# eryxcoop/acvm-backend-plonky2

Measured on AMD Instinct MI355X. Metric: prove latency (ms) + proofs/sec at 2^20 LDE rows, 1 GPU(s): value = proofs/sec, witness resident in HBM, 4 proof(s) in flight per GPU; latency_ms_single_proof = lone resident proof; *_host_witness = p2gpu_prove from host RAM (PCIe inside the call), higher is better.
Workload: dtype u64; 1 GPU; synth(d=17,sha): 131072 gates -> 2^20 LDE rows, 234 wires / 80 routed, KeccakGoldilocksConfig, rate 8, cap 2^4, 28 queries, 16 PoW bits (BASELINE configs[2] shape); degree_bits=17, lde_rows=1048576, mix=sha, public_inputs=0, in_flight_per_gpu=4, proof_bytes=170972

## Files before the change

acvm-backend-plonky2_amd/__init__.py:

```python
from .prover import (
    CircuitData,
    WitnessPlan,
    build_blob,
    VerifierCircuitData,
    ProofWithPublicInputs,
    P2GpuError,
    device_info,
    peer_access,
    init,
    host_array,
    host_free,
    ifft_batch,
    lde_batch,
    commit_values,
    hash_rows,
    field_selftest,
    lib_path,
    load_library,
)
from .synth import make_circuit, synth_lib_path
from . import parallel
from . import translate
from . import acir
```

acvm-backend-plonky2_amd/csrc/gen_keccak_fixed.py:

```python
#!/usr/bin/env python3
import sys

from gen_keccak_sched import RC, Op, ref_keccak_f, round_ops, schedule

NTEMP = 36


def build(base):
    a = [(f"a{i}l", f"a{i}h") for i in range(25)]
    live = [v for p in a for v in p]
    ops = []
    c = []
    for x in range(5):
        halves = []
        for h in range(2):
            p = f"cin{x}{'lh'[h]}p"
            q = f"cin{x}{'lh'[h]}"
            ops.append(Op("X3", p, (a[x][h], a[x + 5][h], a[x + 10][h]), 0x96, len(ops)))
            ops.append(Op("X3", q, (p, a[x + 15][h], a[x + 20][h]), 0x96, len(ops)))
            halves.append(q)
        c.append(tuple(halves))
    cur_a, cur_c = a, c
    for r in range(24):
        rops, cur_a, cur_c = round_ops(r, cur_a, cur_c)
        ops.extend(rops)
    needed = {v for p in cur_a for v in p}
    keep = []
    for o in reversed(ops):
        if o.dst in needed:
            keep.append(o)
            needed.update(o.srcs)
    ops = list(reversed(keep))
    return live, g_schedule(ops, live), cur_a


def g_schedule(ops, live_in, gap=1):
    pos = {v: -gap for v in live_in}
    remaining = list(ops)
    out = []
    slot = 0
    pattern = "BBA"
    while remaining:
        t = len(out)
        avail = [o for o in remaining if all(s in pos and pos[s] + gap <= t for s in o.srcs)]
        if not avail:
            avail = [o for o in remaining if all(s in pos for s in o.srcs)][:1]
        want_a = pattern[slot % 3] == "A"
        pick = None
        for o in avail:
            if (o.kind == "ROT") == want_a:
                pick = o
                break
        if pick is None:
            pick = avail[0]
        else:
            slot += 1
        out.append(pick)
        pos[pick.dst] = t
        remaining.remove(pick)
    return out


def allocate(live, ops, final_a, base):
    alias = {}
    for o in ops:
        if o.kind == "IOTA" and ((RC[int(o.dst[1:].split("_")[0])] >> (32 * o.imm)) & 0xFFFFFFFF) == 0:
            alias[o.dst] = alias.get(o.srcs[0], o.srcs[0])
    if alias:
        ops = [Op(o.kind, o.dst, tuple(alias.get(s_, s_) for s_ in o.srcs), o.imm, o.order) for o in ops if o.dst not in alias]
        final_a = [tuple(alias.get(v, v) for v in p) for p in final_a]
    last_use = {}
    for t, o in enumerate(ops):
        for s in o.srcs:
            last_use[s] = t
    finals = [v for p in final_a for v in p]
    for v in finals:
        last_use[v] = len(ops) + 1
    consumers = {}
    for t, o in enumerate(ops):
        for s in o.srcs:
            consumers.setdefault(s, []).append(o)
    reg = {v: base + i for i, v in enumerate(live)}
    free = list(range(base + 50, base + 50 + NTEMP))
    out = []
    conflicts = 0
    for t, o in enumerate(ops):
        srcs = [reg[s] for s in o.srcs]
        if o.kind in ("X3", "CHI") and len({r % 4 for r in srcs}) == 1:
            conflicts += 1
        for s in set(o.srcs):
            if last_use[s] == t:
                free.append(reg[s])
        avoid_hard, avoid_soft = set(), set()
        for cns in consumers.get(o.dst, []):
            if cns.kind not in ("X3", "CHI"):
                continue
            others = [s for s in cns.srcs if s != o.dst]
            banks = [reg[s] % 4 for s in others if s in reg]
            if len(others) == 2 and len(banks) == 2 and banks[0] == banks[1]:
                avoid_hard.add(banks[0])
            else:
                avoid_soft.update(banks)
        best = None
        for r_ in free:
            b = r_ % 4
            score = (b in avoid_hard) * 100 + (b in avoid_soft) * 1
            if best is None or score < best[0]:
                best = (score, r_)
        if best is None:
            raise SystemExit(f"out of registers at op {t} (NTEMP = {NTEMP})")
        free.remove(best[1])
        reg[o.dst] = best[1]
        out.append((o, best[1], srcs))
    moves = []
    want = {base + i: reg[v] for i, v in enumerate(finals)}
    pending = {d: s for d, s in want.items() if d != s}
    tmp = None
    spare = [r_ for r_ in range(base + 50, base + 50 + NTEMP) if r_ not in set(want.values())]
    while pending:
        progressed = False
        for d, s in list(pending.items()):
            if d not in pending.values():
                moves.append((d, s))
                del pending[d]
                progressed = True
        if not progressed:
            d, s = next(iter(pending.items()))
            tmp = spare[0]
            moves.append((tmp, d))
            for k in pending:
                if pending[k] == d:
                    pending[k] = tmp
    return out, moves, conflicts


def simulate(alloc, moves, st, base):
    M = 0xFFFFFFFF
    regs = {}
    for i in range(25):
        regs[base + 2 * i] = st[i] & M
        regs[base + 2 * i + 1] = st[i] >> 32
    for o, d, srcs in alloc:
        s = [regs[r] for r in srcs]
        if o.kind == "X3":
            v = s[0] ^ s[1] ^ s[2]
        elif o.kind == "CHI":
            v = s[0] ^ (~s[1] & s[2] & M)
        elif o.kind == "ROT":
            v = (((s[0] << 32) | s[1]) >> o.imm) & M
        else:
            rnd = int(o.dst[1:].split("_")[0])
            v = s[0] ^ ((RC[rnd] >> (32 * o.imm)) & M)
        regs[d] = v & M
    for d, s in moves:
        regs[d] = regs[s]
    return [regs[base + 2 * i] | (regs[base + 2 * i + 1] << 32) for i in range(25)]


def main():
    base = 36
    args = [x for x in sys.argv[1:] if not x.startswith("--")]
    if args:
        base = int(args[0])
    live, ops, final_a = build(base)
    alloc, moves, conflicts = allocate(live, ops, final_a, base)
    if "--check" in sys.argv:
        import random
        rng = random.Random(2)
        for _ in range(3):
            st = [rng.getrandbits(64) for _ in range(25)]
            assert simulate(alloc, moves, st, base) == ref_keccak_f(st)
        kinds = "".join("A" if o.kind == "ROT" else "B" for o, _, _ in alloc)
        print(f"ok: {len(alloc)} instructions + {len(moves)} moves, {conflicts} three-source instructions with all sources in one bank;",
              kinds[:60], "...", file=sys.stderr)
        return
    w = sys.stdout.write
    top = base + 50 + NTEMP
    w("// GENERATED by gen_keccak_fixed.py -- do not edit.  Keccak-f[1600], 24 rounds unrolled, explicit VGPRs (see the generator).\n")
    w(f"#define P2_KF_BASE {base}\n#define P2_KF_TOP {top}  /* first register above the block's */\n")
    w("#define P2_KECCAK_FIXED_PERMUTE() P2_KECCAK_FIXED_PERMUTE_PH(1)\n")
    w("#define P2_KECCAK_FIXED_PERMUTE_PH(PH) asm volatile(\".p2align 6\\n .rept \" #PH \"\\n s_nop 0\\n .endr\\n\" \\\n")
    for o, d, srcs in alloc:
        if o.kind in ("X3", "CHI"):
            w(f'  "v_bitop3_b32 v{d}, v{srcs[0]}, v{srcs[1]}, v{srcs[2]} bitop3:{hex(o.imm)}\\n" \\\n')
        elif o.kind == "ROT":
            w(f'  "v_alignbit_b32 v{d}, v{srcs[0]}, v{srcs[1]}, {o.imm}\\n" \\\n')
        else:
            rnd = int(o.dst[1:].split("_")[0])
            k = (RC[rnd] >> (32 * o.imm)) & 0xFFFFFFFF
            if k <= 64:
                w(f'  "v_xor_b32_e64 v{d}, {k}, v{srcs[0]}\\n" \\\n')
            else:
                w(f'  "v_xor_b32 v{d}, {hex(k)}, v{srcs[0]}\\n" \\\n')
    for d, s in moves:
        w(f'  "v_mov_b32 v{d}, v{s}\\n" \\\n')
    w(f'  ::: "v{top - 1}")\n')


if __name__ == "__main__":
    main()
```

acvm-backend-plonky2_amd/csrc/handle.hip:

```cpp
#include "prover_internal.hpp"
#include <functional>

using namespace p2;

namespace {

void release_for_destroy(p2gpu_circuit *c) {
  for (p2gpu_circuit *m : c->group) {
    m->peer = nullptr;
    release_for_destroy(m);
    delete m;
  }
  c->group.clear();
  if (c->peer && c->shard_rank == 0) {
    for (auto e : c->peer->recv_free) if (e) (void)hipEventDestroy(e);
    for (auto e : c->peer->sent) if (e) (void)hipEventDestroy(e);
    delete c->peer;
  }
  c->peer = nullptr;
  (void)hipSetDevice(c->device);
  if (c->stream) (void)hipStreamSynchronize(c->stream);
  if (c->rccl_comm) (void)rccl().CommDestroy((ncclComm_t)c->rccl_comm);
  c->rccl_comm = nullptr;
  circuit_release(c);
}
struct ReleaseHook {
  ReleaseHook() { p2::g_circuit_release = release_for_destroy; }
} g_release_hook;

struct Scratch {
  std::vector<void *> ptrs;
  hipStream_t st = nullptr;
  ~Scratch() {
    for (void *p : ptrs) (void)hipFree(p);
    if (st) (void)hipStreamDestroy(st);
  }
  template <class T> T *alloc(size_t n) {
    void *p = nullptr;
    if (hipMalloc(&p, (n ? n : 1) * sizeof(T)) != hipSuccess) return nullptr;
    ptrs.push_back(p);
    return (T *)p;
  }
};

}

namespace p2 {

int g_device = -1;
std::vector<int> g_peer_access;
std::vector<int> g_devices;

void circuit_release(p2gpu_circuit *c) {
  c->tw_fwd.release(); c->tw_inv.release(); c->scale.release(); c->inv_scale.release(); c->d_kis.release();
  c->d_sigmas.release(); c->fri_scale.release(); c->d_gates.release(); c->qconst.release(); c->l0_lde.release();
  c->d_row_gate.release(); c->d_gconsts.release(); c->d_prc.release(); c->d_prc_hash.release();
  c->hsum.release(); c->htmp_a.release(); c->htmp_b.release();
  c->cs.release(); c->wires.release(); c->zp.release(); c->quot.release();
  c->wires_vals.release(); c->zp_vals.release(); c->cp.release(); c->scan_tmp.release();
  c->apow.release(); c->qvals.release(); c->qtmp.release(); c->pw.release(); c->partial.release();
  c->ext_apow.release(); c->f01.release(); c->f01v.release(); c->fv.release();
  for (auto &b : c->fri_coef) b.release();
  for (auto &b : c->fri_vals) b.release();
  for (auto &b : c->fri_trees) b.release();
  c->hash_state.release();
  c->wire_nz.release();
  c->wire_nzlist.release();
  c->wire_clean.release();
  c->wire_scalar.release(); c->sparse_coeffs.release(); c->sparse_lde.release(); c->sparse_partial.release();
  c->pin.release();
  if (c->sync_event) (void)hipEventDestroy(c->sync_event);
  c->sync_event = nullptr;
  if (c->tail_stage) (void)hipHostFree(c->tail_stage);
  c->tail_stage = nullptr;
  c->pow_result.release(); c->gather_ptrs.release(); c->gather_out.release(); c->xchg_recv.release();
  ntt_plan_destroy(c->plan_inv);
  ntt_plan_destroy(c->plan_fwd);
  for (auto *p : c->fri_plans)
    if (p != c->plan_fwd) ntt_plan_destroy(p);
  c->plan_inv = c->plan_fwd = nullptr;
  c->fri_plans.clear();
  for (auto e : c->event_pool) (void)hipEventDestroy(e);
  for (auto e : c->copy_events) (void)hipEventDestroy(e);
  if (c->copy_stream) (void)hipStreamDestroy(c->copy_stream);
  if (c->stream) (void)hipStreamDestroy(c->stream);
}

int ensure_device() {
  if (g_device >= 0) return 0;
  int cnt = 0;
  hipError_t e = hipGetDeviceCount(&cnt);
  if (e != hipSuccess || cnt == 0) {
    set_err("no HIP device available (%s); libp2gpu has no CPU fallback", e == hipSuccess ? "count=0" : hipGetErrorString(e));
    return P2GPU_E_DEVICE;
  }
  int dev = 0;
  (void)hipGetDevice(&dev);
  g_device = dev;
  g_devices.assign(1, dev);
  g_peer_access.assign(1, -1);
  return 0;
}

}


namespace {

#define CK(e, what)                                       \
  do {                                                    \
    const hipError_t e_ = (e);                            \
    if (e_ != hipSuccess) {                               \
      set_err("%s: %s", what, hipGetErrorString(e_));     \
      return P2GPU_E_DEVICE;                              \
    }                                                     \
  } while (0)

void schedule_gates(p2gpu_circuit *c) {
  c->nterms = c->K + c->K * c->nchunks + c->max_gate_constraints;
  auto cost = [](const GateDesc &g) { return g.kind == G_POSEIDON ? 0u : 4u * g.num_constraints + 8u; };
  const uint32_t perm_cost = (uint32_t)env_uint("P2GPU_PERM_COST", 8u * c->R + 100u);
  uint32_t total = 0;
  for (auto &g : c->gates) total += cost(g);
  c->gate_groups = env_uint("P2GPU_GATE_GROUPS", total > 2 * perm_cost ? 4u : 1u) == 4 ? 4u : 1u;
  uint32_t load[4] = {perm_cost, 0, 0, 0};
  std::vector<uint32_t> order(c->gates.size());
  for (size_t i = 0; i < order.size(); i++) order[i] = (uint32_t)i;
  std::sort(order.begin(), order.end(), [&](uint32_t x, uint32_t y) { return cost(c->gates[x]) > cost(c->gates[y]); });
  for (uint32_t gi : order) {
    uint32_t best = 0;
    for (uint32_t q = 1; q < 4; q++)
      if (load[q] < load[best]) best = q;
    c->gates[gi].pad = c->gate_groups == 4 ? best : 0;
    load[best] += cost(c->gates[gi]);
  }
  uint64_t half_constraints = 0;
  if (env_flag("P2GPU_HALF_GATES", true) && c->d >= 6 && c->rate_bits == 3)
    for (auto &g : c->gates)
      if (g.kind != G_POSEIDON && g.num_constraints >= 48 && gate_degree(g.kind, g.p) <= 4 && c->half_slots < 64) {
        g.pad |= (++c->half_slots) << 16;
        half_constraints += g.num_constraints;
      }
  c->half_auto = (half_constraints << c->d) >= ((uint64_t)12 << 20);
  if (c->half_slots) {
    auto cost_main = [&](const GateDesc &g) { return gate_half_slot(g) ? 8u : cost(g); };
    uint32_t rest = 0;
    for (auto &g : c->gates) rest += cost_main(g);
    c->gate_groups_half = env_uint("P2GPU_GATE_GROUPS_HALF", rest > 2 * perm_cost ? 4u : 1u) == 4 ? 4u : 1u;
    uint32_t lm[4] = {perm_cost, 0, 0, 0}, ls[4] = {0, 0, 0, 0};
    c->sums_groups = env_uint("P2GPU_SUMS_GROUPS", c->half_slots >= 2 ? 4u : 1u) == 4 ? 4u : 1u;
    for (uint32_t gi : order) {
      GateDesc &g = c->gates[gi];
      uint32_t bm = 0, bs = 0;
      for (uint32_t q = 1; q < 4; q++) {
        if (lm[q] < lm[bm]) bm = q;
        if (ls[q] < ls[bs]) bs = q;
      }
      if (c->gate_groups_half == 4) g.pad |= bm << 4;
      lm[bm] += cost_main(g);
      if (gate_half_slot(g)) {
        if (c->sums_groups == 4) g.pad |= bs << 8;
        ls[bs] += cost(g);
      }
    }
  }
}

int make_streams(p2gpu_circuit *c) {
  if (poseidon_upload_constants()) { set_err("uploading Poseidon constants failed"); return P2GPU_E_DEVICE; }
  CK(hipStreamCreateWithFlags(&c->stream, hipStreamNonBlocking), "hipStreamCreate");
  CK(hipStreamCreateWithFlags(&c->copy_stream, hipStreamNonBlocking), "hipStreamCreate");
  return P2GPU_OK;
}

int make_root_tables(p2gpu_circuit *c) {
  hipStream_t st = c->stream;
  const size_t n = c->n;
  const uint32_t d = c->d, K = c->K, C = c->C;
  const size_t half = n >= 2 ? n / 2 : 1;
  CK(c->tw_fwd.alloc(half), "alloc tw");
  CK(c->tw_inv.alloc(half), "alloc tw");
  CK(c->scale.alloc((size_t)C * n), "alloc scale");
  CK(c->inv_scale.alloc((size_t)C * n), "alloc scale");
  CK(c->fri_scale.alloc((size_t)C * n), "alloc scale");
  CK(c->d_kis.alloc(c->R), "alloc kis");
  CK(c->d_sigmas.alloc((size_t)c->R * n), "alloc sigmas");
  CK(c->d_gates.alloc(c->num_gates ? c->num_gates : 1), "alloc gates");
  gl_t wn = gl_root(d), wN = gl_root(d + c->rate_bits);
  c->plan_inv = ntt_plan_create(st, d, NttDir::ToCoeffs);
  c->plan_fwd = ntt_plan_create(st, d, NttDir::ToValues);
  if (!c->plan_inv || !c->plan_fwd) { set_err("ntt plan allocation failed"); return P2GPU_E_DEVICE; }
  fill_powers(st, c->tw_fwd.p, wn, (uint32_t)half);
  fill_powers(st, c->tw_inv.p, gl_inv(wn), (uint32_t)half);
  fill_coset_scale(st, c->scale.p, GL_GEN, wN, d, C, 1);
  fill_coset_scale(st, c->inv_scale.p, gl_inv(GL_GEN), gl_inv(wN), d, C, 1);
  if (c->half_slots) {
    const size_t per = (size_t)4 * c->half_slots * K * n;
    CK(c->hsum.alloc(2 * per), "alloc gate sums");
    CK(c->htmp_a.alloc(per), "alloc gate sums");
    CK(c->htmp_b.alloc(per), "alloc gate sums");
    const gl_t w8 = gl_root(3), quarter = gl_inv(4);
    for (int mo = 0; mo < 4; mo++)
      for (int m = 0; m < 4; m++) {
        const gl_t base = gl_pow(w8, (uint64_t)((2 * mo + 1 - 2 * m + 16) % 8));
        gl_t acc = 0, pw = 1;
        for (int j = 0; j < 4; j++) {
          acc = gl_add(acc, pw);
          pw = gl_mul(pw, base);
        }
        c->half_cross[4 * mo + m] = gl_mul(acc, quarter);
      }
  }
  CK(c->qconst.alloc(24), "alloc qconst");
  {
    gl_t qc[24];
    memset(qc, 0, sizeof qc);
    gl_t wC = gl_root(c->rate_bits), gn = gl_pow(GL_GEN, n);
    for (uint32_t r = 0; r < C; r++) {
      qc[r] = gl_mul(GL_GEN, gl_pow(wN, r));
      qc[8 + r] = gl_sub(gl_mul(gn, gl_pow(wC, r)), 1);
      qc[16 + r] = gl_inv(qc[8 + r]);
    }
    CK(hipMemcpy(c->qconst.p, qc, sizeof qc, hipMemcpyHostToDevice), "copy qconst");
    CK(c->l0_lde.alloc((size_t)C * n), "alloc L0 table");
    fill_l0_table(st, c->qconst.p, c->tw_fwd.p, 0, d, C, gl_inv((gl_t)n), c->l0_lde.p);
  }
  return P2GPU_OK;
}

int tables_from_blob(p2gpu_circuit *c, const gl_t *constants, const gl_t *sigmas) {
  const size_t n = c->n;
  const uint32_t ngc = c->NC - c->num_selectors;
  CK(hipMemcpyAsync(c->d_sigmas.p, sigmas, 8 * (size_t)c->R * n, hipMemcpyHostToDevice, c->stream), "copy sigmas");
  std::vector<uint8_t> rg(n, 0);
  for (size_t row = 0; row < n; row++) {
    uint32_t gi = 0;
    for (uint32_t s = 0; s < c->num_selectors; s++) {
      gl_t v = constants[(size_t)s * n + row];
      if (c->num_selectors == 1 || v != 0xFFFFFFFFULL) gi = (uint32_t)v;
    }
    if (gi >= c->num_gates) { set_err("selector column holds an unknown gate index"); return P2GPU_E_BLOB; }
    rg[row] = (uint8_t)gi;
    if (c->sparse_row == UINT32_MAX && c->gates[gi].kind == G_PUBLIC_INPUT) c->sparse_row = (uint32_t)row;
  }
  c->sparse_rows = SparseRows();
  if (c->sparse_row != UINT32_MAX) {
    c->sparse_rows.row[c->sparse_rows.count++] = c->sparse_row;
    for (size_t row = 0; row < n && c->sparse_rows.count < MAX_SPARSE_ROWS; row++)
      if (c->gates[rg[row]].kind == G_POSEIDON) c->sparse_rows.row[c->sparse_rows.count++] = (uint32_t)row;
  }
  CK(hipMemcpy(c->d_row_gate.p, rg.data(), n, hipMemcpyHostToDevice), "copy row_gate");
  if (ngc)
    CK(hipMemcpy(c->d_gconsts.p, constants + (size_t)c->num_selectors * n, 8 * (size_t)ngc * n, hipMemcpyHostToDevice), "copy gconsts");
  return P2GPU_OK;
}

int alloc_proof_buffers(p2gpu_circuit *c) {
  hipStream_t st = c->stream;
  const size_t n = c->n;
  const uint32_t d = c->d, K = c->K, C = c->C;
  const uint32_t ncs = c->NC + c->R, nzp = K * (1 + c->PP), nq = K * c->QF;
  const uint32_t nall = ncs + c->W + nzp + nq;
  if (batch_alloc(c, c->cs, ncs) || batch_alloc(c, c->wires, c->W) || batch_alloc(c, c->zp, nzp) || batch_alloc(c, c->quot, nq)) return P2GPU_E_DEVICE;
  CK(c->wires_vals.alloc((size_t)c->W * n), "alloc wires");
  CK(c->wire_nz.alloc(c->W), "alloc wire flags");
  CK(c->wire_nzlist.alloc(c->W + 1), "alloc wire flags");
  CK(c->wire_clean.alloc(c->W), "alloc wire flags");
  CK(hipMemsetAsync(c->wire_clean.p, 0, sizeof(uint32_t) * c->W, c->stream), "clear wire flags");
  CK(c->wire_scalar.alloc((size_t)MAX_SPARSE_ROWS * c->W), "alloc wire flags");
  if (c->sparse_row != UINT32_MAX) {
    const uint32_t nr = c->sparse_rows.count;
    CK(c->sparse_coeffs.alloc((size_t)nr * n), "alloc sparse basis");
    CK(c->sparse_lde.alloc((size_t)nr * C * n), "alloc sparse basis");
    CK(c->sparse_partial.alloc(16 * 2 + 2), "alloc sparse basis");
    const gl_t one = 1;
    CK(hipMemsetAsync(c->sparse_coeffs.p, 0, 8 * (size_t)nr * n, st), "sparse basis");
    for (uint32_t s = 0; s < nr; s++)
      CK(hipMemcpyAsync(c->sparse_coeffs.p + (size_t)s * n + c->sparse_rows.row[s], &one, 8, hipMemcpyHostToDevice, st), "sparse basis");
    CK(hipStreamSynchronize(st), "sparse basis");
    ntt_batch(st, c->plan_inv, c->sparse_coeffs.p, c->sparse_coeffs.p, nr, 1, nullptr, gl_inv((gl_t)n), false);
    for (uint32_t s = 0; s < nr; s++)
      ntt_batch(st, c->plan_fwd, c->sparse_coeffs.p + (size_t)s * n, c->sparse_lde.p + (size_t)s * C * n, 1, C, c->scale.p, 1, false);
  }
  CK(c->zp_vals.alloc((size_t)nzp * n), "alloc zp");
  CK(c->cp.alloc((size_t)K * (c->nchunks + 1) * n), "alloc cp");
  CK(c->scan_tmp.alloc((size_t)K * (n + (n + 255) / 256 + 8)), "alloc scan");
  CK(c->apow.alloc((size_t)2 * c->nterms), "alloc apow");
  CK(c->qvals.alloc((size_t)K * C * n), "alloc qvals");
  CK(c->qtmp.alloc((size_t)K * C * n), "alloc qtmp");
  CK(c->pw.alloc((size_t)4 * n), "alloc pw");
  CK(c->partial.alloc(((size_t)(nall + K) + 8) * 16 * 2), "alloc partial");
  CK(c->ext_apow.alloc((size_t)2 * nall), "alloc ext_apow");
  CK(c->f01.alloc((size_t)4 * n), "alloc f01");
  CK(c->f01v.alloc((size_t)4 * n), "alloc f01v");
  CK(c->fv.alloc((size_t)2 * n), "alloc fv");
  c->fri_coef.resize(c->n_steps + 1);
  c->fri_vals.resize(c->n_steps + 1);
  c->fri_trees.resize(c->n_steps);
  size_t gather_words = 0;
  {
    uint32_t ds = d;
    const size_t cap_per = ((size_t)1 << c->cap_h) >> c->rate_bits;
    for (uint32_t s = 0; s <= c->n_steps; s++) {
      c->fri_plans.push_back(s == 0 ? c->plan_fwd : ntt_plan_create(st, ds, NttDir::ToValues));
      if (!c->fri_plans.back()) { set_err("ntt plan allocation failed"); return P2GPU_E_DEVICE; }
      CK(c->fri_coef[s].alloc((size_t)2 << ds), "alloc fri coef");
      if (s < c->n_steps) {
        CK(c->fri_vals[s].alloc((size_t)2 * C << ds), "alloc fri vals");
        uint32_t ab = c->arity[s];
        if (ab < 1 || ab > 4 || ds < ab || (((size_t)1 << ds) >> ab) < cap_per) { set_err("unsupported FRI reduction arity"); return P2GPU_E_BLOB; }
        if (tree_alloc(c->fri_trees[s], C, ((size_t)1 << ds) >> ab, cap_per)) return P2GPU_E_DEVICE;
        gather_words += (2u << ab) + 4 * (size_t)(ds + c->rate_bits);
        ds -= ab;
      }
    }
  }
  gather_words += nall + 4 * 4 * (size_t)(d + c->rate_bits);
  c->gather_cap = gather_words * c->num_queries + 64;
  CK(c->gather_ptrs.alloc(c->gather_cap), "alloc gather");
  CK(c->gather_out.alloc(c->gather_cap), "alloc gather");
  CK(c->pow_result.alloc(1), "alloc pow");
  {
    size_t n_final = n;
    for (uint32_t s = 0; s < c->n_steps; s++) n_final >>= c->arity[s];
    const size_t caps = (size_t)2 * (4 + c->n_steps) * (sizeof(dig_t) << c->cap_h);
    CK(c->pin.alloc(16 * c->gather_cap + 32 * n_final + 16 * (size_t)(nall + K) * 16 + 16 * (size_t)nall + 16 * (size_t)c->nterms +
                    20 * (size_t)c->W + caps + ((size_t)1 << 18)),
       "alloc pinned staging");
  }
  return P2GPU_OK;
}

struct TableSource {
  const gl_t *constants = nullptr, *sigmas = nullptr;
  const BuildInputs *build = nullptr;
};

int commit_constants_sigmas(p2gpu_circuit *c, const TableSource &src) {
  hipStream_t st = c->stream;
  const size_t n = c->n;
  const uint32_t ncs = c->NC + c->R;
  gl_t *stage = c->cs.lde.p;
  if (src.build) {
    build_selector_columns(st, c, stage);
    if (c->NC > c->num_selectors)
      CK(hipMemcpyAsync(stage + (size_t)c->num_selectors * n, c->d_gconsts.p, 8 * (size_t)(c->NC - c->num_selectors) * n, hipMemcpyDeviceToDevice, st),
         "copy constants");
  } else {
    CK(hipMemcpyAsync(stage, src.constants, 8 * (size_t)c->NC * n, hipMemcpyHostToDevice, st), "copy constants");
  }
  CK(hipMemcpyAsync(stage + (size_t)c->NC * n, c->d_sigmas.p, 8 * (size_t)c->R * n, hipMemcpyDeviceToDevice, st), "copy sigmas");
  ntt_batch(st, c->plan_inv, stage, c->cs.coeffs.p, ncs, 1, nullptr, gl_inv((gl_t)n), false);
  return batch_commit_from_coeffs(c, c->cs);
}

int check_cap_and_digest(p2gpu_circuit *c, const uint8_t *cap_in) {
  if (cap_in) {
    for (size_t i = 0; i < c->cs.cap.size(); i++)
      if (memcmp(cap_in + 32 * i, c->cs.cap[i].w, c->hasher ? 32 : 25)) { set_err("constants_sigmas cap mismatch"); return P2GPU_E_CAP_MISMATCH; }
  }
  if (!(c->flags & 1)) {
    std::vector<gl_t> parts;
    for (auto &dg : c->cs.cap) {
      gl_t e[4];
      digest_elems(dg, e);
      parts.insert(parts.end(), e, e + 4);
    }
    std::vector<gl_t> pad(8, 0);
    pad[0] = 1;
    pad[7] = 1;
    dig_t ds = host_hash_no_pad(pad);
    gl_t e[4];
    digest_elems(ds, e);
    parts.insert(parts.end(), e, e + 4);
    parts.push_back(c->d);
    c->circuit_digest = host_hash_no_pad(parts);
  }
  return P2GPU_OK;
}

int circuit_finish(p2gpu_circuit *c, const TableSource &src, const uint8_t *cap_in) {
  schedule_gates(c);
  CK(hipSetDevice(c->device), "hipSetDevice");
  const CreateTrace tr{c, now_ms()};
  if (int rc = make_streams(c)) return rc;
  tr.mark("streams + poseidon constants");
  if (int rc = make_root_tables(c)) return rc;
  tr.mark("root tables + ntt plans");
  const uint32_t ngc = c->NC - c->num_selectors;
  CK(hipMemcpyAsync(c->d_kis.p, c->k_is.data(), 8 * (size_t)c->R, hipMemcpyHostToDevice, c->stream), "copy kis");
  if (c->num_gates)
    CK(hipMemcpyAsync(c->d_gates.p, c->gates.data(), sizeof(GateDesc) * c->num_gates, hipMemcpyHostToDevice, c->stream), "copy gates");
  CK(c->d_row_gate.alloc(c->n), "alloc row_gate");
  CK(c->d_gconsts.alloc((size_t)(ngc ? ngc : 1) * c->n), "alloc gconsts");
  CK(c->d_prc.alloc(360), "alloc prc");
  if (int rc = src.build ? build_device_tables(c, *src.build, tr) : tables_from_blob(c, src.constants, src.sigmas)) return rc;
  CK(hipMemcpy(c->d_prc.p, c->poseidon_rc, sizeof c->poseidon_rc, hipMemcpyHostToDevice), "copy prc");
  gl_t hrc[360];
  poseidon_device_constants(c->poseidon_rc, hrc);
  CK(c->d_prc_hash.alloc(360), "alloc prc (hash form)");
  CK(hipMemcpy(c->d_prc_hash.p, hrc, sizeof hrc, hipMemcpyHostToDevice), "copy prc (hash form)");
  tr.mark("sigma/constant uploads, row->gate");
  if (int rc = alloc_proof_buffers(c)) return rc;
  tr.mark("batch + work buffer allocation");
  if (int rc = commit_constants_sigmas(c, src)) return rc;
  if (int rc = check_cap_and_digest(c, cap_in)) return rc;
  CK(hipStreamSynchronize(c->stream), "sync");
  tr.mark("constants_sigmas commitment");
  return P2GPU_OK;
}
#undef CK

int circuit_create_one(const uint8_t *blob, size_t len, int device, p2gpu_circuit **out_c) try {
  HalfBuilt c(new p2gpu_circuit());
  size_t off = 0;
  const uint8_t *cap_in = nullptr;
  c->device = device;
  if (int rc = circuit_parse(blob, len, c.get(), &off, &cap_in)) return rc;
  c->blob_prefix.assign(blob, blob + off);
  if (len < off + 8 * ((size_t)c->NC * c->n + (size_t)c->R * c->n)) { set_err("blob truncated (tables)"); return P2GPU_E_BLOB; }
  TableSource src;
  src.constants = (const gl_t *)(blob + off);
  src.sigmas = src.constants + (size_t)c->NC * c->n;
  if (int rc = circuit_finish(c.get(), src, cap_in)) return rc;
  *out_c = c.release();
  return P2GPU_OK;
} P2GPU_CATCH

struct BuildCall {
  const p2gpu_build_params *bp;
  const p2gpu_gate_decl *gates;
  uint32_t num_gates;
  BuildInputs in;
  std::vector<uint8_t> prefix;
};
int build_call_prepare(BuildCall &b, const p2gpu_build_params *bp, const p2gpu_gate_decl *gates, uint32_t num_gates, const uint32_t *row_gate,
                       const uint64_t *row_constants, const uint32_t *copies, size_t num_copies, uint32_t hasher, p2gpu_circuit **out_c) {
  if (out_c) *out_c = nullptr;
  if (!bp || !gates || !row_gate || !out_c || (num_copies && !copies)) return P2GPU_E_ARG;
  if (hasher > 1) { set_err("unsupported hasher (0 = KeccakHash<25>, 1 = PoseidonHash)"); return P2GPU_E_ARG; }
  BuildPlan pl;
  if (int rc = build_plan(bp, gates, num_gates, row_constants != nullptr, pl)) return rc;
  b.prefix.resize(pl.prefix_len);
  if (int rc = build_prefix(pl, bp, gates, hasher, b.prefix.data())) return rc;
  b.bp = bp; b.gates = gates; b.num_gates = num_gates;
  b.in = BuildInputs{row_gate, row_constants, copies, num_copies};
  return P2GPU_OK;
}
int circuit_build_one(const BuildCall &b, int device, p2gpu_circuit **out_c) try {
  HalfBuilt c(new p2gpu_circuit());
  c->device = device;
  size_t off = 0;
  const uint8_t *cap_in = nullptr;
  if (int rc = circuit_parse(b.prefix.data(), b.prefix.size(), c.get(), &off, &cap_in))
    return rc == P2GPU_E_BLOB ? P2GPU_E_ARG : rc;
  c->blob_prefix = b.prefix;
  TableSource src;
  src.build = &b.in;
  if (int rc = circuit_finish(c.get(), src, nullptr)) return rc;
  *out_c = c.release();
  return P2GPU_OK;
} P2GPU_CATCH
}

extern "C" {

int p2gpu_init(const int *device_ids, int n_devices) {
  int cnt = 0;
  hipError_t e = hipGetDeviceCount(&cnt);
  if (e != hipSuccess || cnt == 0) {
    set_err("no HIP device available (%s); libp2gpu has no CPU fallback", e == hipSuccess ? "count=0" : hipGetErrorString(e));
    return P2GPU_E_DEVICE;
  }
  if (n_devices > 8) {
    set_err("p2gpu_init: %d device ids (at most 8: one per LDE coset)", n_devices);
    return P2GPU_E_ARG;
  }
  std::vector<int> devs;
  for (int i = 0; i < (device_ids ? n_devices : 0); i++) devs.push_back(device_ids[i]);
  if (devs.empty()) devs.push_back(0);
  for (int dev : devs)
    if (dev < 0 || dev >= cnt) {
      set_err("device id %d out of range (%d devices)", dev, cnt);
      return P2GPU_E_ARG;
    }
  std::vector<int> peer(devs.size() * devs.size(), -1);
  for (size_t a = 0; a < devs.size(); a++)
    for (size_t b = 0; b < devs.size(); b++)
      if (devs[a] != devs[b]) {
        (void)hipSetDevice(devs[a]);
        const hipError_t pe = hipDeviceEnablePeerAccess(devs[b], 0);
        (void)hipGetLastError();
        peer[a * devs.size() + b] = (pe == hipSuccess || pe == hipErrorPeerAccessAlreadyEnabled) ? 1 : 0;
      }
  HIP_TRY(hipSetDevice(devs[0]));
  g_device = devs[0];
  g_devices = devs;
  g_peer_access = peer;
  return P2GPU_OK;
}

int p2gpu_peer_access(int *matrix_out, int cap) {
  if (int rc = ensure_device()) return rc;
  const int n = (int)g_devices.size();
  if (matrix_out) {
    if (cap < n * n) { set_err("p2gpu_peer_access: room for %d entries, %d needed", cap, n * n); return P2GPU_E_BUFFER; }
    for (int i = 0; i < n * n; i++) matrix_out[i] = i < (int)g_peer_access.size() ? g_peer_access[i] : -1;
  }
  return n;
}

void *p2gpu_host_alloc(size_t bytes) {
  if (ensure_device()) return nullptr;
  void *p = nullptr;
  hipError_t e = hipHostMalloc(&p, bytes ? bytes : 1, hipHostMallocPortable);
  if (e != hipSuccess) {
    (void)hipGetLastError();
    set_err("p2gpu_host_alloc: %zu bytes of page-locked memory: %s", bytes, hipGetErrorString(e));
    return nullptr;
  }
  return p;
}
void p2gpu_host_free(void *p) {
  if (p) (void)hipHostFree(p);
}

int p2gpu_device_info(char *name_out, size_t name_cap, int *cu_count, size_t *hbm_bytes) {
  if (int rc = ensure_device()) return rc;
  hipDeviceProp_t prop;
  HIP_TRY(hipGetDeviceProperties(&prop, g_device));
  if (name_out && name_cap) snprintf(name_out, name_cap, "%s (%s)", prop.name, prop.gcnArchName);
  if (cu_count) *cu_count = prop.multiProcessorCount;
  if (hbm_bytes) *hbm_bytes = prop.totalGlobalMem;
  return P2GPU_OK;
}


static int shard_layout(p2gpu_circuit *c, int rank, int world);
static int shard_args_ok(p2gpu_circuit *c, int rank, int world);


int p2gpu_circuit_create_on(const uint8_t *blob, size_t len, int device_id, p2gpu_circuit **out_c) try {
  if (!blob || !out_c) return P2GPU_E_ARG;
  if (int rc = ensure_device()) return rc;
  if (std::find(g_devices.begin(), g_devices.end(), device_id) == g_devices.end()) {
    set_err("p2gpu_circuit_create_on: device %d is not in the list given to p2gpu_init", device_id);
    return P2GPU_E_ARG;
  }
  const int rc = circuit_create_one(blob, len, device_id, out_c);
  (void)hipSetDevice(g_device);
  return rc;
} P2GPU_CATCH

static int circuit_make(const std::function<int(int, p2gpu_circuit **)> &one, p2gpu_circuit **out_c) {
  if (g_devices.size() <= 1) return one(g_device, out_c);
  const int n = (int)g_devices.size();
  std::vector<p2gpu_circuit *> hs(n, nullptr);
  std::vector<int> rcs(n, 0);
  std::vector<std::string> errs(n);
  {
    std::vector<std::thread> th;
    for (int q = 0; q < n; q++)
      th.emplace_back([&, q] {
        rcs[q] = one(g_devices[q], &hs[q]);
        if (rcs[q]) errs[q] = p2gpu_last_error();
      });
    for (auto &t : th) t.join();
  }
  (void)hipSetDevice(g_device);
  auto drop = [&](int rc, const std::string &msg) {
    for (auto *h : hs)
      if (h) {
        h->peer = nullptr;
        p2gpu_circuit_destroy(h);
      }
    set_err("%s", msg.c_str());
    return rc;
  };
  for (int q = 0; q < n; q++)
    if (rcs[q]) return drop(rcs[q], errs[q]);
  for (int q = 0; q < n; q++) {
    if (int rc = shard_args_ok(hs[q], q, n)) return drop(rc, p2gpu_last_error());
    if (int rc = shard_layout(hs[q], q, n)) return drop(rc, p2gpu_last_error());
  }
  PeerGroup *pg = new PeerGroup();
  pg->n = n;
  pg->cs = hs;
  pg->recv_free.assign(n, nullptr);
  pg->sent.assign(n, nullptr);
  pg->proof_scratch.resize(n);
  pg->send_ptr.resize(n);
  pg->recv_ptr.resize(n);
  for (int q = 0; q < n; q++) {
    (void)hipSetDevice(hs[q]->device);
    if (hipEventCreateWithFlags(&pg->recv_free[q], hipEventDisableTiming) != hipSuccess ||
        hipEventCreateWithFlags(&pg->sent[q], hipEventDisableTiming) != hipSuccess) {
      for (int k = 0; k <= q; k++) {
        (void)hipSetDevice(hs[k]->device);
        if (pg->recv_free[k]) (void)hipEventDestroy(pg->recv_free[k]);
        if (pg->sent[k]) (void)hipEventDestroy(pg->sent[k]);
        hs[k]->peer = nullptr;
      }
      (void)hipSetDevice(g_device);
      delete pg;
      return drop(P2GPU_E_DEVICE, "hipEventCreate failed");
    }
    hs[q]->peer = pg;
  }
  (void)hipSetDevice(g_device);
  for (int q = 1; q < n; q++) hs[0]->group.push_back(hs[q]);
  *out_c = hs[0];
  return P2GPU_OK;
}

int p2gpu_circuit_create(const uint8_t *blob, size_t len, p2gpu_circuit **out_c) try {
  if (!blob || !out_c) return P2GPU_E_ARG;
  if (int rc = ensure_device()) return rc;
  return circuit_make([&](int device, p2gpu_circuit **h) { return circuit_create_one(blob, len, device, h); }, out_c);
} P2GPU_CATCH


int p2gpu_circuit_build_on(const p2gpu_build_params *bp, const p2gpu_gate_decl *gates, uint32_t num_gates, const uint32_t *row_gate,
                           const uint64_t *row_constants, const uint32_t *copies, size_t num_copies, uint32_t hasher, int device_id,
                           p2gpu_circuit **out_c) try {
  BuildCall b;
  if (int rc = build_call_prepare(b, bp, gates, num_gates, row_gate, row_constants, copies, num_copies, hasher, out_c)) return rc;
  if (int rc = ensure_device()) return rc;
  if (std::find(g_devices.begin(), g_devices.end(), device_id) == g_devices.end()) {
    set_err("p2gpu_circuit_build_on: device %d is not in the list given to p2gpu_init", device_id);
    return P2GPU_E_ARG;
  }
  const int rc = circuit_build_one(b, device_id, out_c);
  (void)hipSetDevice(g_device);
  return rc;
} P2GPU_CATCH

int p2gpu_circuit_build(const p2gpu_build_params *bp, const p2gpu_gate_decl *gates, uint32_t num_gates, const uint32_t *row_gate,
                        const uint64_t *row_constants, const uint32_t *copies, size_t num_copies, uint32_t hasher, p2gpu_circuit **out_c) try {
  BuildCall b;
  if (int rc = build_call_prepare(b, bp, gates, num_gates, row_gate, row_constants, copies, num_copies, hasher, out_c)) return rc;
  if (int rc = ensure_device()) return rc;
  return circuit_make([&](int device, p2gpu_circuit **h) { return circuit_build_one(b, device, h); }, out_c);
} P2GPU_CATCH

int p2gpu_circuit_export_blob(const p2gpu_circuit *cc, uint8_t *out, size_t *len) try {
  if (!cc || !len) return P2GPU_E_ARG;
  if (int rc = prover_handle(cc)) return rc;
  p2gpu_circuit *c = const_cast<p2gpu_circuit *>(cc);
  const size_t n = c->n, nsel = c->num_selectors, ngc = c->NC - c->num_selectors;
  const size_t need = c->blob_prefix.size() + 8 * ((size_t)c->NC + c->R) * n;
  if (!out || *len < need) {
    const bool probe = out == nullptr;
    *len = need;
    if (probe) return P2GPU_OK;
    set_err("blob buffer too small: need %zu bytes", need);
    return P2GPU_E_BUFFER;
  }
  HIP_TRY(hipSetDevice(c->device));
  Scratch S;
  gl_t *sel = S.alloc<gl_t>(nsel * n);
  if (!sel) { set_err("hipMalloc failed"); (void)hipSetDevice(g_device); return P2GPU_E_DEVICE; }
  build_selector_columns(c->stream, c, sel);
  memcpy(out, c->blob_prefix.data(), c->blob_prefix.size());
  uint8_t *q = out + c->blob_prefix.size();
  hipError_t e = hipMemcpyAsync(q, sel, 8 * nsel * n, hipMemcpyDeviceToHost, c->stream);
  if (e == hipSuccess && ngc) e = hipMemcpyAsync(q + 8 * nsel * n, c->d_gconsts.p, 8 * ngc * n, hipMemcpyDeviceToHost, c->stream);
  if (e == hipSuccess) e = hipMemcpyAsync(q + 8 * (size_t)c->NC * n, c->d_sigmas.p, 8 * (size_t)c->R * n, hipMemcpyDeviceToHost, c->stream);
  const hipError_t e2 = hipStreamSynchronize(c->stream);
  (void)hipSetDevice(g_device);
  HIP_TRY(e);
  HIP_TRY(e2);
  *len = need;
  return P2GPU_OK;
} P2GPU_CATCH




int p2gpu_circuit_set(p2gpu_circuit *c, const char *key, uint64_t value) try {
  if (!c || !key) return P2GPU_E_ARG;
  if (int rc = prover_handle(c)) return rc;
  for (p2gpu_circuit *m : c->group)
    if (int rc = p2gpu_circuit_set(m, key, value)) return rc;
  HIP_TRY(hipSetDevice(c->device));
  std::string k(key);
  if (k == "pow_hint") c->pow_hint = value;
  else if (k == "self_check") c->self_check = (int)value;
  else if (k == "shard_exercise") c->shard_exercise = (int)value;
  else if (k == "shard_intt") c->shard_intt = (int)value;
  else if (k == "shard_reduce") c->shard_reduce = (int)value;
  else if (k == "shard_zs") c->shard_zs = (int)value;
  else if (k == "half_gates") c->half_gates = (int)value;
  else if (k == "blocking_sync") c->blocking_sync = (int)value;
  else if (k == "virtual_columns") {
    c->virtual_columns = (int)value;
    if (c->wire_clean.p) HIP_TRY(hipMemsetAsync(c->wire_clean.p, 0, sizeof(uint32_t) * c->W, c->stream));
  }
  else if (k == "zero_columns") {
    c->zero_columns = (int)value;
    c->structured_off = false;
    if (c->wire_clean.p) HIP_TRY(hipMemsetAsync(c->wire_clean.p, 0, sizeof(uint32_t) * c->W, c->stream));
  }
  else if (k == "profile") {
    flush_kstats(c);
    c->profile = (int)value;
    c->kstats.clear();
  } else {
    set_err("unknown knob %s", key);
    return P2GPU_E_ARG;
  }
  return P2GPU_OK;
} P2GPU_CATCH

static int shard_layout(p2gpu_circuit *c, int rank, int world) {
  HIP_TRY(hipSetDevice(c->device));
  if (c->stream) HIP_TRY(hipStreamSynchronize(c->stream));
  if (c->rccl_comm) {
    (void)rccl().CommDestroy((ncclComm_t)c->rccl_comm);
    c->rccl_comm = nullptr;
  }
  c->shard_rank = rank;
  c->shard_world = world;
  c->shard_fn = nullptr;
  c->shard_ctx = nullptr;
  const uint32_t ncl = c->C / (uint32_t)world;
  const size_t cap_per = ((size_t)1 << c->cap_h) >> c->rate_bits;
  CosetMap cm;
  cm.first = (uint32_t)rank;
  cm.stride = (uint32_t)world;
  Batch *bs[3] = {&c->wires, &c->zp, &c->quot};
  for (Batch *b : bs) {
    b->ncl = ncl;
    b->cm = cm;
    tree_layout(*b, ncl, c->n, cap_per);
  }
  if (c->n_steps > 0) {
    Batch &t0 = c->fri_trees[0];
    t0.ncl = ncl;
    t0.cm = cm;
    tree_layout(t0, ncl, c->n >> c->arity[0], cap_per);
  }
  if (c->wire_clean.p) HIP_TRY(hipMemsetAsync(c->wire_clean.p, 0, sizeof(uint32_t) * c->W, c->stream));
  c->xchg_recv.release();
  HIP_TRY(c->xchg_recv.alloc(std::max({(size_t)world * c->gather_cap, (size_t)c->K * c->C * c->n, (size_t)2 * world * c->n}) + 64));
  return P2GPU_OK;
}
static int shard_args_ok(p2gpu_circuit *c, int rank, int world) {
  if (!c || world < 1 || rank < 0 || rank >= world || (c->C % (uint32_t)world) != 0) {
    set_err("bad shard configuration: rank %d of %d (cosets %u)", rank, world, c ? c->C : 0u);
    return P2GPU_E_ARG;
  }
  if (int rc = prover_handle(c)) return rc;
  return P2GPU_OK;
}

static int not_a_group(const p2gpu_circuit *c) {
  if (c && c->peer) { set_err("this handle is a device group of one process (p2gpu_init with several ids): its sharding is fixed"); return P2GPU_E_ARG; }
  return P2GPU_OK;
}
int p2gpu_circuit_set_shard(p2gpu_circuit *c, int rank, int world, p2gpu_allgather_fn fn, void *ctx) try {
  if (int rc = not_a_group(c)) return rc;
  if (int rc = shard_args_ok(c, rank, world)) return rc;
  if (world > 1 && !fn) { set_err("a host all-gather callback is needed for world > 1 (or use p2gpu_circuit_set_shard_rccl)"); return P2GPU_E_ARG; }
  if (int rc = shard_layout(c, rank, world)) return rc;
  c->shard_fn = fn;
  c->shard_ctx = ctx;
  return P2GPU_OK;
} P2GPU_CATCH

int p2gpu_shard_unique_id(uint8_t id_out[128]) try {
  if (!id_out) return P2GPU_E_ARG;
  if (int rc = ensure_device()) return rc;
  if (!rccl().ok) { set_err("librccl.so.1 could not be loaded"); return P2GPU_E_DEVICE; }
  ncclUniqueId id;
  static_assert(sizeof id == 128, "ncclUniqueId is 128 bytes");
  RCCL_TRY(rccl().GetUniqueId(&id));
  memcpy(id_out, &id, sizeof id);
  return P2GPU_OK;
} P2GPU_CATCH

int p2gpu_circuit_set_shard_rccl(p2gpu_circuit *c, int rank, int world, const uint8_t id_in[128]) try {
  if (int rc = not_a_group(c)) return rc;
  if (int rc = shard_args_ok(c, rank, world)) return rc;
  if (!id_in) return P2GPU_E_ARG;
  if (!rccl().ok) { set_err("librccl.so.1 could not be loaded"); return P2GPU_E_DEVICE; }
  if (int rc = shard_layout(c, rank, world)) return rc;
  ncclUniqueId id;
  memcpy(&id, id_in, sizeof id);
  ncclComm_t comm = nullptr;
  RCCL_TRY(rccl().CommInitRank(&comm, world, id, rank));
  c->rccl_comm = (void *)comm;
  return P2GPU_OK;
} P2GPU_CATCH

int p2gpu_kernel_stats(p2gpu_circuit *c, char *names, double *ms, double *bytes, uint64_t *launches, int cap) try {
  if (!c) return P2GPU_E_ARG;
  if (int rc = prover_handle(c)) return rc;
  (void)hipSetDevice(c->device);
  (void)hipStreamSynchronize(c->stream);
  flush_kstats(c);
  int i = 0;
  for (auto &kv : c->kstats) {
    if (i >= cap) break;
    snprintf(names + 64 * i, 64, "%s", kv.first.c_str());
    ms[i] = kv.second.ms;
    bytes[i] = kv.second.bytes;
    launches[i] = kv.second.launches;
    i++;
  }
  return i;
} P2GPU_CATCH

int p2gpu_ifft_batch(const uint64_t *vals, size_t ncols, unsigned d, uint64_t *coeffs_out) try {
  if (int rc = ensure_device()) return rc;
  if (!vals || !coeffs_out || d > 24) return P2GPU_E_ARG;
  Scratch S;
  HIP_TRY(hipStreamCreate(&S.st));
  size_t n = (size_t)1 << d, half = n >= 2 ? n / 2 : 1;
  gl_t *a = S.alloc<gl_t>(ncols * n), *b = S.alloc<gl_t>(ncols * n), *tw = S.alloc<gl_t>(half);
  if (!a || !b || !tw) { set_err("hipMalloc failed"); return P2GPU_E_DEVICE; }
  HIP_TRY(hipMemcpyAsync(a, vals, 8 * ncols * n, hipMemcpyHostToDevice, S.st));
  NttPlan *plan = ntt_plan_create(S.st, d, NttDir::ToCoeffs);
  if (!plan) { set_err("hipMalloc failed"); return P2GPU_E_DEVICE; }
  ntt_batch(S.st, plan, a, b, (uint32_t)ncols, 1, nullptr, gl_inv((gl_t)n), false);
  bitrev_cols(S.st, b, a, d, (uint32_t)ncols);
  hipError_t e1 = hipMemcpyAsync(coeffs_out, a, 8 * ncols * n, hipMemcpyDeviceToHost, S.st);
  hipError_t e2 = hipStreamSynchronize(S.st);
  ntt_plan_destroy(plan);
  HIP_TRY(e1);
  HIP_TRY(e2);
  return P2GPU_OK;
} P2GPU_CATCH

int p2gpu_lde_batch(const uint64_t *coeffs, size_t ncols, unsigned d, unsigned rate_bits, uint64_t *lde_out) try {
  if (int rc = ensure_device()) return rc;
  if (!coeffs || !lde_out || d > 24 || rate_bits > 3) return P2GPU_E_ARG;
  Scratch S;
  HIP_TRY(hipStreamCreate(&S.st));
  size_t n = (size_t)1 << d, half = n >= 2 ? n / 2 : 1;
  uint32_t C = 1u << rate_bits;
  gl_t *a = S.alloc<gl_t>(ncols * n), *b = S.alloc<gl_t>(ncols * n), *tw = S.alloc<gl_t>(half);
  gl_t *scale = S.alloc<gl_t>(C * n), *lde = S.alloc<gl_t>(C * ncols * n);
  if (!a || !b || !tw || !scale || !lde) { set_err("hipMalloc failed"); return P2GPU_E_DEVICE; }
  HIP_TRY(hipMemcpyAsync(a, coeffs, 8 * ncols * n, hipMemcpyHostToDevice, S.st));
  bitrev_cols(S.st, a, b, d, (uint32_t)ncols);
  NttPlan *plan = ntt_plan_create(S.st, d, NttDir::ToValues);
  if (!plan) { set_err("hipMalloc failed"); return P2GPU_E_DEVICE; }
  fill_coset_scale(S.st, scale, GL_GEN, gl_root(d + rate_bits), d, C, 1);
  ntt_batch(S.st, plan, b, lde, (uint32_t)ncols, C, scale, 1, false);
  std::vector<gl_t> tmp(C * ncols * n);
  hipError_t e1 = hipMemcpyAsync(tmp.data(), lde, 8 * tmp.size(), hipMemcpyDeviceToHost, S.st);
  hipError_t e2 = hipStreamSynchronize(S.st);
  ntt_plan_destroy(plan);
  HIP_TRY(e1);
  HIP_TRY(e2);
  for (uint32_t r = 0; r < C; r++)
    for (size_t col = 0; col < ncols; col++)
      for (size_t k = 0; k < n; k++) lde_out[col * C * n + C * k + r] = tmp[((size_t)r * ncols + col) * n + k];
  return P2GPU_OK;
} P2GPU_CATCH

static int field_selftest_words(const uint64_t *a, const uint64_t *b, size_t n, uint64_t *bad_out, size_t words);
int p2gpu_field_selftest(const uint64_t *a, const uint64_t *b, size_t n, uint64_t bad_out[8]) { return field_selftest_words(a, b, n, bad_out, 8); }
int p2gpu_field_selftest16(const uint64_t *a, const uint64_t *b, size_t n, uint64_t bad_out[16]) { return field_selftest_words(a, b, n, bad_out, 16); }
static int field_selftest_words(const uint64_t *a, const uint64_t *b, size_t n, uint64_t *bad_out, size_t words) try {
  if (int rc = ensure_device()) return rc;
  if (!a || !b || !bad_out || n == 0 || n > ((size_t)1 << 28)) return P2GPU_E_ARG;
  Scratch S;
  HIP_TRY(hipStreamCreate(&S.st));
  uint64_t *da = S.alloc<uint64_t>(n), *db = S.alloc<uint64_t>(n);
  unsigned long long *bad = S.alloc<unsigned long long>(16);
  if (!da || !db || !bad) { set_err("hipMalloc failed"); return P2GPU_E_DEVICE; }
  HIP_TRY(hipMemcpyAsync(da, a, 8 * n, hipMemcpyHostToDevice, S.st));
  HIP_TRY(hipMemcpyAsync(db, b, 8 * n, hipMemcpyHostToDevice, S.st));
  HIP_TRY(hipMemsetAsync(bad, 0, 128, S.st));
  field_selftest(S.st, da, db, (uint32_t)n, bad);
  HIP_TRY(hipMemcpyAsync(bad_out, bad, 8 * words, hipMemcpyDeviceToHost, S.st));
  HIP_TRY(hipStreamSynchronize(S.st));
  return P2GPU_OK;
} P2GPU_CATCH

int p2gpu_hash_rows(const uint64_t *rows, size_t n_rows, size_t row_len, uint8_t *digests_out) try {
  if (int rc = ensure_device()) return rc;
  if (!rows || !digests_out) return P2GPU_E_ARG;
  Scratch S;
  HIP_TRY(hipStreamCreate(&S.st));
  gl_t *a = S.alloc<gl_t>(n_rows * row_len);
  dig_t *dg = S.alloc<dig_t>(n_rows);
  if (!a || !dg) { set_err("hipMalloc failed"); return P2GPU_E_DEVICE; }
  HIP_TRY(hipMemcpyAsync(a, rows, 8 * n_rows * row_len, hipMemcpyHostToDevice, S.st));
  hash_rows(S.st, a, n_rows, (uint32_t)row_len, dg);
  std::vector<dig_t> h(n_rows);
  HIP_TRY(hipMemcpyAsync(h.data(), dg, sizeof(dig_t) * n_rows, hipMemcpyDeviceToHost, S.st));
  HIP_TRY(hipStreamSynchronize(S.st));
  for (size_t i = 0; i < n_rows; i++) memcpy(digests_out + 25 * i, h[i].w, 25);
  return P2GPU_OK;
} P2GPU_CATCH

int p2gpu_commit_values(const uint64_t *vals, size_t ncols, unsigned d, unsigned rate_bits, unsigned cap_h,
                        uint8_t *cap_out) try {
  if (int rc = ensure_device()) return rc;
  if (!vals || !cap_out || d > 24 || rate_bits > 3 || cap_h < rate_bits || cap_h > rate_bits + d) return P2GPU_E_ARG;
  HalfBuilt own(new p2gpu_circuit());
  p2gpu_circuit *c = own.get();
  c->d = d; c->rate_bits = rate_bits; c->cap_h = cap_h; c->n = (size_t)1 << d; c->N = c->n << rate_bits;
  c->C = 1u << rate_bits; c->device = g_device; c->n_steps = 0;
  int rc = P2GPU_OK;
  size_t n = c->n, half = n >= 2 ? n / 2 : 1;
  do {
    if (hipStreamCreate(&c->stream) != hipSuccess || c->tw_fwd.alloc(half) != hipSuccess ||
        c->tw_inv.alloc(half) != hipSuccess || c->scale.alloc((size_t)c->C * n) != hipSuccess ||
        c->wires_vals.alloc(ncols * n) != hipSuccess || c->pin.alloc(((size_t)1 << 16) + 2 * (sizeof(dig_t) << cap_h)) != hipSuccess) {
      set_err("hipMalloc failed");
      rc = P2GPU_E_DEVICE;
      break;
    }
    if ((rc = batch_alloc(c, c->wires, (uint32_t)ncols))) break;
    c->plan_inv = ntt_plan_create(c->stream, d, NttDir::ToCoeffs);
    c->plan_fwd = ntt_plan_create(c->stream, d, NttDir::ToValues);
    if (!c->plan_inv || !c->plan_fwd) {
      set_err("hipMalloc failed");
      rc = P2GPU_E_DEVICE;
      break;
    }
    fill_coset_scale(c->stream, c->scale.p, GL_GEN, gl_root(d + rate_bits), d, c->C, 1);
    if (hipMemcpyAsync(c->wires_vals.p, vals, 8 * ncols * n, hipMemcpyHostToDevice, c->stream) != hipSuccess) {
      set_err("copy failed");
      rc = P2GPU_E_DEVICE;
      break;
    }
    if ((rc = batch_commit_from_values(c, c->wires, c->wires_vals.p))) break;
    for (size_t i = 0; i < c->wires.cap.size(); i++) memcpy(cap_out + 25 * i, c->wires.cap[i].w, 25);
  } while (0);
  return rc;
} P2GPU_CATCH

}
```

acvm-backend-plonky2_amd/csrc/internal.hpp:

```cpp
#pragma once
#include <hip/hip_runtime.h>
#include <cstdlib>
#include <vector>
#include "gl.hpp"
#include "keccak.hpp"
#include "gates.hpp"

namespace p2 {

constexpr int MAX_GATES = 64;
constexpr uint32_t MAX_GATE_CONSTRAINTS = 4096;
constexpr uint32_t MAX_ARITY_BITS = 4;
constexpr int MAX_CHALLENGES = 2;
constexpr int MAX_ROUTED = 128;

inline bool env_flag(const char *name, bool dflt) {
  const char *e = getenv(name);
  return e && *e ? *e != '0' : dflt;
}
inline uint64_t env_uint(const char *name, uint64_t dflt) {
  const char *e = getenv(name);
  return e ? strtoull(e, nullptr, 10) : dflt;
}

struct Prof {
  virtual void begin(const char *kernel, double algorithmic_bytes) = 0;
  virtual void end() = 0;
  virtual ~Prof() {}
};
extern thread_local Prof *g_prof;
struct ProfScope {
  ProfScope(const char *k, double bytes) { if (g_prof) g_prof->begin(k, bytes); }
  ~ProfScope() { if (g_prof) g_prof->end(); }
};

constexpr uint32_t MAX_SPARSE_ROWS = 4;
struct SparseRows {
  uint32_t row[MAX_SPARSE_ROWS] = {UINT32_MAX, UINT32_MAX, UINT32_MAX, UINT32_MAX};
  uint32_t count = 0;
};
struct ColHints {
  const uint32_t *cls = nullptr;
  const uint32_t *clean = nullptr;
  const gl_t *val = nullptr;
  const gl_t *basis = nullptr;
  bool basis_per_coset = false;
  uint32_t nrows = 1, val_stride = 0;
  size_t basis_stride = 0;
  uint32_t virt_first = UINT32_MAX;
  uint32_t dense_hint = 0;
  bool fill_only = false;
};
void column_clean_update(hipStream_t st, const uint32_t *cls, uint32_t cols, uint32_t *clean, bool after);
void column_flags(hipStream_t st, const gl_t *vals, uint32_t cols, uint32_t d, const SparseRows &rows, uint32_t *flags,
                  gl_t *scalar, uint32_t sstride);

constexpr int NTT_MAX_ROUNDS = 6;
enum class NttDir { ToCoeffs, ToValues };
struct NttPass {
  uint32_t s, a, tb, nrounds;
  uint32_t r[NTT_MAX_ROUNDS], tw_off[NTT_MAX_ROUNDS];
  bool direct = false;
  uint32_t rm = 0, rl = 0, fold_r = 0, fold_s0 = 0;
  uint32_t ftw_off = 0;
};
struct NttPlan {
  uint32_t d = 0;
  NttDir dir = NttDir::ToCoeffs;
  std::vector<NttPass> passes;
  gl_t *ptw = nullptr;
  size_t table_len = 0;
};
struct CosetMap {
  uint32_t first = 0, stride = 1;
};
NttPlan *ntt_plan_create(hipStream_t st, uint32_t d, NttDir dir);
void ntt_plan_destroy(NttPlan *p);
void ntt_batch(hipStream_t st, const NttPlan *plan, const gl_t *src, gl_t *dst, uint32_t cols, uint32_t cosets,
               const gl_t *scale, gl_t post, bool src_per_coset, CosetMap cm = CosetMap(), uint32_t stride_cols = 0,
               const ColHints *hints = nullptr);

void fill_powers(hipStream_t st, gl_t *out, gl_t root, uint32_t count);
void fill_coset_scale(hipStream_t st, gl_t *out, gl_t shift, gl_t wN, uint32_t d, uint32_t cosets, gl_t mult);

void bitrev_cols(hipStream_t st, const gl_t *in, gl_t *out, uint32_t d, uint32_t cols);
void field_selftest(hipStream_t st, const uint64_t *a, const uint64_t *b, uint32_t n, unsigned long long *bad);

struct VirtCols {
  const uint32_t *cls = nullptr;
  const gl_t *val = nullptr;
  const gl_t *basis = nullptr;
  uint32_t first = UINT32_MAX;
  uint32_t coset_first = 0, coset_stride = 1;
};
uint32_t hash_lde_leaves(hipStream_t st, const gl_t *lde, uint32_t cols, uint32_t d, uint32_t cosets, dig_t *dig, const gl_t *prc = nullptr,
                         const VirtCols *virt = nullptr, dig_t *lvl1 = nullptr, dig_t *lvl2 = nullptr);
void hash_lde_absorb(hipStream_t st, const gl_t *lde, uint32_t cols, uint32_t d, uint32_t cosets, uint32_t blk0,
                     uint32_t nblk, bool first, bool last, uint64_t *state, dig_t *dig, const VirtCols *virt = nullptr);
void hash_rows(hipStream_t st, const gl_t *rows, size_t n_rows, uint32_t row_len, dig_t *dig);
void hash_fri_leaves(hipStream_t st, const gl_t *vals, uint32_t lg_npc, uint32_t cosets, uint32_t arity_bits,
                     dig_t *dig, const gl_t *prc = nullptr);
bool tree_levels(hipStream_t st, dig_t *lvl, uint32_t cosets, uint32_t m, uint32_t cap_per, const gl_t *prc = nullptr,
                 dig_t *host_mirror = nullptr);

struct ZsArgs {
  const gl_t *wires;
  const gl_t *sigmas;
  const gl_t *k_is;
  const gl_t *sub_tw;
  uint32_t tw_shift;
  uint32_t d, R, QF, nchunks, K;
  gl_t betas[MAX_CHALLENGES], gammas[MAX_CHALLENGES];
  gl_t *cp;
  uint32_t sb;
  uint32_t row0, rows;
  gl_t *zp;
};
void zs_partial_products(hipStream_t st, const ZsArgs &a, gl_t *scan_tmp);
void zs_chunks(hipStream_t st, const ZsArgs &a);
void zs_scan_finish(hipStream_t st, const ZsArgs &a, gl_t *scan_tmp);

struct QuotArgs {
  const gl_t *cs_lde;
  const gl_t *wires_lde;
  const gl_t *zp_lde;
  const gl_t *k_is;
  const gl_t *tw;
  const gl_t *apow;
  const GateDesc *gates;
  const GateDesc *host_gates;
  gl_t *out;
  uint32_t tw_shift, d, rate_bits, W, R, NC, num_selectors, K, QF, nchunks, PP, num_gates, nterms, has_poseidon;
  uint32_t gate_groups;
  uint32_t gate_groups_half;
  uint32_t use_half;
  uint32_t nsk;
  gl_t *hsum;
  uint32_t coset_first, coset_stride, ncosets;
  gl_t betas[MAX_CHALLENGES], gammas[MAX_CHALLENGES];
  gl_t pi_hash[4];
  const gl_t *qconst;
  gl_t n_inv;
  const gl_t *l0;
};
void quotient_eval(hipStream_t st, const QuotArgs &a);
void gate_sums_eval(hipStream_t st, const QuotArgs &a, uint32_t groups);
void gate_sums_cross(hipStream_t st, const gl_t *in, const gl_t *inv_scale, gl_t *out, uint32_t d, uint32_t cols, const gl_t F[16]);
void fill_l0_table(hipStream_t st, const gl_t *qconst, const gl_t *tw, uint32_t tw_shift, uint32_t d, uint32_t cosets, gl_t n_inv, gl_t *out);
int poseidon_upload_constants();
void quotient_chunks(hipStream_t st, const gl_t *in, const gl_t *inv_scale, gl_t *out, uint32_t d, uint32_t K,
                     uint32_t rate_bits, gl_t w_inv, gl_t gn_inv, gl_t rate_inv, uint32_t world = 1);

void fill_witness(hipStream_t st, gl_t *wires, const uint8_t *row_gate, const GateDesc *gates, const gl_t *gconsts,
                  const gl_t *prc, uint32_t d, uint32_t ngc, uint32_t num_wires);

void ext_powers_bitrev2(hipStream_t st, ext_t base0, ext_t base1, uint32_t d, gl_t *out0, gl_t *out1);
void eval_columns(hipStream_t st, const gl_t *coeffs, uint32_t cols, uint32_t d, const gl_t *pw, uint32_t parts,
                  gl_t *partial , const ColHints *hints = nullptr, const gl_t *basis_partial = nullptr);
struct EvalSegs {
  struct Seg {
    const gl_t *coeffs;
    const gl_t *pw;
    gl_t *partial;
    uint32_t cols;
  } seg[6];
  uint32_t count = 0, hinted = UINT32_MAX;
  const uint32_t *cls = nullptr;
  const gl_t *val = nullptr, *basis_partial = nullptr;
};
void eval_columns_multi(hipStream_t st, const EvalSegs &S, uint32_t d, uint32_t parts, uint32_t col0 = 0, uint32_t ncols = UINT32_MAX);
void reduce_columns(hipStream_t st, const gl_t *coeffs, uint32_t cols, uint32_t d, const gl_t *apow ,
                    uint32_t j0, gl_t *acc, bool accumulate, const uint32_t *nzlist = nullptr, const gl_t *basis = nullptr,
                    const gl_t *fold = nullptr);
void compact_nonzero(hipStream_t st, const uint32_t *flags, uint32_t cols, uint32_t *list);
void sum_parts(hipStream_t st, const gl_t *parts, uint32_t nparts, size_t len, gl_t *out);
void class1_fold(hipStream_t st, const ColHints &h, uint32_t cols, const gl_t *apow, uint32_t j0, gl_t *fold);
void fri_quotient_values(hipStream_t st, const gl_t *F0, const gl_t *F1, uint32_t d, const gl_t *tw, uint32_t tw_shift,
                         ext_t zeta, ext_t gzeta, ext_t f0z, ext_t f1z, ext_t aK, gl_t *out );
void fri_fold(hipStream_t st, const gl_t *in , uint32_t d, uint32_t arity_bits, ext_t beta, gl_t *out);
void pow_search(hipStream_t st, const gl_t state[12], uint32_t pos, uint32_t pow_bits, uint64_t base, uint64_t count,
                unsigned long long *result, const gl_t *prc = nullptr);
void gather_u64(hipStream_t st, const uint64_t *addr, uint32_t count, gl_t *out);

}
```

acvm-backend-plonky2_amd/csrc/keccak.hpp:

```cpp
#pragma once
#include "gl.hpp"

namespace p2 {

struct alignas(32) dig_t {
  uint64_t w[4];
};

P2_HD uint64_t rotl64(uint64_t x, int n) { return (x << n) | (x >> (64 - n)); }

#if defined(__HIP_DEVICE_COMPILE__)
__device__ __forceinline__ uint64_t kx3(uint64_t a, uint64_t b, uint64_t c) {
  uint32_t lo = __builtin_amdgcn_bitop3_b32((uint32_t)a, (uint32_t)b, (uint32_t)c, 0x96);
  uint32_t hi = __builtin_amdgcn_bitop3_b32((uint32_t)(a >> 32), (uint32_t)(b >> 32), (uint32_t)(c >> 32), 0x96);
  return ((uint64_t)hi << 32) | lo;
}
__device__ __forceinline__ uint64_t kchi(uint64_t a, uint64_t b, uint64_t c) {
  uint32_t lo = __builtin_amdgcn_bitop3_b32((uint32_t)a, (uint32_t)b, (uint32_t)c, 0xD2);
  uint32_t hi = __builtin_amdgcn_bitop3_b32((uint32_t)(a >> 32), (uint32_t)(b >> 32), (uint32_t)(c >> 32), 0xD2);
  return ((uint64_t)hi << 32) | lo;
}
template <int N>
__device__ __forceinline__ uint64_t krot(uint64_t x) {
  const uint32_t lo = (uint32_t)x, hi = (uint32_t)(x >> 32);
  if constexpr (N == 0) {
    return x;
  } else if constexpr (N == 32) {
    return ((uint64_t)lo << 32) | hi;
  } else if constexpr (N < 32) {
    uint32_t nh = __builtin_amdgcn_alignbit(hi, lo, 32 - N), nl = __builtin_amdgcn_alignbit(lo, hi, 32 - N);
    return ((uint64_t)nh << 32) | nl;
  } else {
    uint32_t nh = __builtin_amdgcn_alignbit(lo, hi, 64 - N), nl = __builtin_amdgcn_alignbit(hi, lo, 64 - N);
    return ((uint64_t)nh << 32) | nl;
  }
}
#define P2_KX3(a, b, c) kx3(a, b, c)
#define P2_KCHI(a, b, c) kchi(a, b, c)
#define P2_KROT(x, n) krot<n>(x)
#else
#define P2_KX3(a, b, c) ((a) ^ (b) ^ (c))
#define P2_KCHI(a, b, c) ((a) ^ (~(b) & (c)))
#define P2_KROT(x, n) rotl64(x, n)
#endif

#define P2_KECCAK_ROUND(RC)                                                                                            \
  {                                                                                                                    \
    uint64_t c0 = P2_KX3(P2_KX3(a00, a05, a10), a15, a20), c1 = P2_KX3(P2_KX3(a01, a06, a11), a16, a21),               \
             c2 = P2_KX3(P2_KX3(a02, a07, a12), a17, a22), c3 = P2_KX3(P2_KX3(a03, a08, a13), a18, a23),               \
             c4 = P2_KX3(P2_KX3(a04, a09, a14), a19, a24);                                                             \
    uint64_t r0 = P2_KROT(c0, 1), r1 = P2_KROT(c1, 1), r2 = P2_KROT(c2, 1), r3 = P2_KROT(c3, 1), r4 = P2_KROT(c4, 1);  \
                                                                        \
    a00 = P2_KX3(a00, c4, r1); a05 = P2_KX3(a05, c4, r1); a10 = P2_KX3(a10, c4, r1); a15 = P2_KX3(a15, c4, r1);        \
    a20 = P2_KX3(a20, c4, r1);                                                                                         \
    a01 = P2_KX3(a01, c0, r2); a06 = P2_KX3(a06, c0, r2); a11 = P2_KX3(a11, c0, r2); a16 = P2_KX3(a16, c0, r2);        \
    a21 = P2_KX3(a21, c0, r2);                                                                                         \
    a02 = P2_KX3(a02, c1, r3); a07 = P2_KX3(a07, c1, r3); a12 = P2_KX3(a12, c1, r3); a17 = P2_KX3(a17, c1, r3);        \
    a22 = P2_KX3(a22, c1, r3);                                                                                         \
    a03 = P2_KX3(a03, c2, r4); a08 = P2_KX3(a08, c2, r4); a13 = P2_KX3(a13, c2, r4); a18 = P2_KX3(a18, c2, r4);        \
    a23 = P2_KX3(a23, c2, r4);                                                                                         \
    a04 = P2_KX3(a04, c3, r0); a09 = P2_KX3(a09, c3, r0); a14 = P2_KX3(a14, c3, r0); a19 = P2_KX3(a19, c3, r0);        \
    a24 = P2_KX3(a24, c3, r0);                                                                                         \
                                                                             \
    uint64_t b00 = a00, b10 = P2_KROT(a01, 1), b20 = P2_KROT(a02, 62), b05 = P2_KROT(a03, 28), b15 = P2_KROT(a04, 27); \
    uint64_t b16 = P2_KROT(a05, 36), b01 = P2_KROT(a06, 44), b11 = P2_KROT(a07, 6), b21 = P2_KROT(a08, 55),            \
             b06 = P2_KROT(a09, 20);                                                                                   \
    uint64_t b07 = P2_KROT(a10, 3), b17 = P2_KROT(a11, 10), b02 = P2_KROT(a12, 43), b12 = P2_KROT(a13, 25),            \
             b22 = P2_KROT(a14, 39);                                                                                   \
    uint64_t b23 = P2_KROT(a15, 41), b08 = P2_KROT(a16, 45), b18 = P2_KROT(a17, 15), b03 = P2_KROT(a18, 21),           \
             b13 = P2_KROT(a19, 8);                                                                                    \
    uint64_t b14 = P2_KROT(a20, 18), b24 = P2_KROT(a21, 2), b09 = P2_KROT(a22, 61), b19 = P2_KROT(a23, 56),            \
             b04 = P2_KROT(a24, 14);                                                                                   \
                                                                                                              \
    a00 = P2_KCHI(b00, b01, b02); a01 = P2_KCHI(b01, b02, b03); a02 = P2_KCHI(b02, b03, b04);                          \
    a03 = P2_KCHI(b03, b04, b00); a04 = P2_KCHI(b04, b00, b01);                                                        \
    a05 = P2_KCHI(b05, b06, b07); a06 = P2_KCHI(b06, b07, b08); a07 = P2_KCHI(b07, b08, b09);                          \
    a08 = P2_KCHI(b08, b09, b05); a09 = P2_KCHI(b09, b05, b06);                                                        \
    a10 = P2_KCHI(b10, b11, b12); a11 = P2_KCHI(b11, b12, b13); a12 = P2_KCHI(b12, b13, b14);                          \
    a13 = P2_KCHI(b13, b14, b10); a14 = P2_KCHI(b14, b10, b11);                                                        \
    a15 = P2_KCHI(b15, b16, b17); a16 = P2_KCHI(b16, b17, b18); a17 = P2_KCHI(b17, b18, b19);                          \
    a18 = P2_KCHI(b18, b19, b15); a19 = P2_KCHI(b19, b15, b16);                                                        \
    a20 = P2_KCHI(b20, b21, b22); a21 = P2_KCHI(b21, b22, b23); a22 = P2_KCHI(b22, b23, b24);                          \
    a23 = P2_KCHI(b23, b24, b20); a24 = P2_KCHI(b24, b20, b21);                                                        \
    a00 ^= (RC);                                                                                                       \
  }

#if defined(__HIP_DEVICE_COMPILE__)
#include "keccak_fixed.inc"
#define P2_KF_SET(i, lo, hi)                                                                                     \
  asm volatile("v_mov_b32 v%c2, %0\n v_mov_b32 v%c3, %1" ::"v"(lo), "v"(hi), "n"(P2_KF_BASE + 2 * (i)), "n"(P2_KF_BASE + 2 * (i) + 1))
#define P2_KF_XOR(i, lo, hi)                                                                                     \
  asm volatile("v_xor_b32 v%c2, v%c2, %0\n v_xor_b32 v%c3, v%c3, %1" ::"v"(lo), "v"(hi), "n"(P2_KF_BASE + 2 * (i)), "n"(P2_KF_BASE + 2 * (i) + 1))
#define P2_KF_GET(i, lo, hi)                                                                                     \
  asm volatile("v_mov_b32 %0, v%c2\n v_mov_b32 %1, v%c3" : "=v"(lo), "=v"(hi) : "n"(P2_KF_BASE + 2 * (i)), "n"(P2_KF_BASE + 2 * (i) + 1))
#define P2_KF_KERNEL_ATTR __attribute__((amdgpu_num_vgpr(P2_KF_BASE / 2)))
#else
#define P2_KF_KERNEL_ATTR
#define P2_KF_SET(i, lo, hi) ((void)(lo), (void)(hi))
#define P2_KF_XOR(i, lo, hi) ((void)(lo), (void)(hi))
#define P2_KF_GET(i, lo, hi) ((lo) = 0, (hi) = 0)
#define P2_KECCAK_FIXED_PERMUTE() ((void)0)
#define P2_KECCAK_FIXED_PERMUTE_PH(PH) ((void)0)
#endif

P2_HD void keccak_f1600(uint64_t st[25]) {
  const uint64_t RC[24] = {
      0x0000000000000001ULL, 0x0000000000008082ULL, 0x800000000000808aULL, 0x8000000080008000ULL,
      0x000000000000808bULL, 0x0000000080000001ULL, 0x8000000080008081ULL, 0x8000000000008009ULL,
      0x000000000000008aULL, 0x0000000000000088ULL, 0x0000000080008009ULL, 0x000000008000000aULL,
      0x000000008000808bULL, 0x800000000000008bULL, 0x8000000000008089ULL, 0x8000000000008003ULL,
      0x8000000000008002ULL, 0x8000000000000080ULL, 0x000000000000800aULL, 0x800000008000000aULL,
      0x8000000080008081ULL, 0x8000000000008080ULL, 0x0000000080000001ULL, 0x8000000080008008ULL};
  uint64_t a00 = st[0], a01 = st[1], a02 = st[2], a03 = st[3], a04 = st[4], a05 = st[5], a06 = st[6], a07 = st[7],
           a08 = st[8], a09 = st[9], a10 = st[10], a11 = st[11], a12 = st[12], a13 = st[13], a14 = st[14],
           a15 = st[15], a16 = st[16], a17 = st[17], a18 = st[18], a19 = st[19], a20 = st[20], a21 = st[21],
           a22 = st[22], a23 = st[23], a24 = st[24];
#if defined(__HIP_DEVICE_COMPILE__)
#pragma unroll 2
#endif
  for (int r = 0; r < 24; r++) P2_KECCAK_ROUND(RC[r])
  st[0] = a00; st[1] = a01; st[2] = a02; st[3] = a03; st[4] = a04; st[5] = a05; st[6] = a06; st[7] = a07;
  st[8] = a08; st[9] = a09; st[10] = a10; st[11] = a11; st[12] = a12; st[13] = a13; st[14] = a14; st[15] = a15;
  st[16] = a16; st[17] = a17; st[18] = a18; st[19] = a19; st[20] = a20; st[21] = a21; st[22] = a22; st[23] = a23;
  st[24] = a24;
}

P2_HD void keccak256_words(const uint64_t *in, size_t nwords, uint64_t out[4]) {
  uint64_t st[25];
  for (int i = 0; i < 25; i++) st[i] = 0;
  size_t off = 0;
  while (nwords - off >= 17) {
    for (int i = 0; i < 17; i++) st[i] ^= in[off + i];
    keccak_f1600(st);
    off += 17;
  }
  size_t rem = nwords - off;
  for (size_t i = 0; i < rem; i++) st[i] ^= in[off + i];
  st[rem] ^= 0x01ULL;
  st[16] ^= 0x8000000000000000ULL;
  keccak_f1600(st);
  for (int i = 0; i < 4; i++) out[i] = st[i];
}

P2_HD dig_t dig_from_state(const uint64_t st[4]) {
  dig_t d;
  d.w[0] = st[0];
  d.w[1] = st[1];
  d.w[2] = st[2];
  d.w[3] = st[3] & 0xFFULL;
  return d;
}

P2_HD dig_t keccak_two_to_one(const dig_t &l, const dig_t &r) {
  uint64_t st[25];
  for (int i = 0; i < 25; i++) st[i] = 0;
  st[0] = l.w[0];
  st[1] = l.w[1];
  st[2] = l.w[2];
  st[3] = (l.w[3] & 0xFFULL) | (r.w[0] << 8);
  st[4] = (r.w[0] >> 56) | (r.w[1] << 8);
  st[5] = (r.w[1] >> 56) | (r.w[2] << 8);
  st[6] = (r.w[2] >> 56) | ((r.w[3] & 0xFFULL) << 8) | (0x01ULL << 16);
  st[16] = 0x8000000000000000ULL;
  keccak_f1600(st);
  return dig_from_state(st);
}

struct KeccakCoopLane {
  uint32_t col[4];
  uint32_t rm, rp;
  uint32_t b0, b1, b2;
  uint32_t s, swap;
  uint32_t m0;
};
P2_HD KeccakCoopLane keccak_coop_lane(uint32_t lane) {
  const int rot[25] = {0, 1, 62, 28, 27, 36, 44, 6, 55, 20, 3, 10, 43, 25, 39, 41, 45, 15, 21, 8, 18, 2, 61, 56, 14};
  const uint32_t base = lane & 32u, L0 = lane & 31u, L = L0 < 25 ? L0 : 0;
  const int x = L % 5, y = L / 5;
  KeccakCoopLane c;
  for (int i = 0; i < 4; i++) c.col[i] = (base + (L + 5 * (i + 1)) % 25) * 4;
  c.rm = (base + (x + 4) % 5 + 5 * y) * 4;
  c.rp = (base + (x + 1) % 5 + 5 * y) * 4;
  auto src = [&](int X, int Y) { return (uint32_t)((((Y - 3 * X) % 5 + 5) % 5) * 3 % 5 + 5 * X); };
  c.b0 = (base + src(x, y)) * 4;
  c.b1 = (base + src((x + 1) % 5, y)) * 4;
  c.b2 = (base + src((x + 2) % 5, y)) * 4;
  const int r = rot[L];
  c.swap = (r == 0 || r >= 32) ? 1u : 0u;
  c.s = (uint32_t)(32 - (r & 31)) & 31u;
  c.m0 = L0 == 0 ? 0xFFFFFFFFu : 0u;
  return c;
}
__device__ __forceinline__ void keccak_f1600_coop(uint32_t &lo, uint32_t &hi, const KeccakCoopLane &c) {
#if defined(__HIP_DEVICE_COMPILE__)
  constexpr uint64_t RC[24] = {
      0x0000000000000001ULL, 0x0000000000008082ULL, 0x800000000000808aULL, 0x8000000080008000ULL,
      0x000000000000808bULL, 0x0000000080000001ULL, 0x8000000080008081ULL, 0x8000000000008009ULL,
      0x000000000000008aULL, 0x0000000000000088ULL, 0x0000000080008009ULL, 0x000000008000000aULL,
      0x000000008000808bULL, 0x800000000000008bULL, 0x8000000000008089ULL, 0x8000000000008003ULL,
      0x8000000000008002ULL, 0x8000000000000080ULL, 0x000000000000800aULL, 0x800000008000000aULL,
      0x8000000080008081ULL, 0x8000000000008080ULL, 0x0000000080000001ULL, 0x8000000080008008ULL};
  auto bp = [](uint32_t addr, uint32_t v) { return (uint32_t)__builtin_amdgcn_ds_bpermute((int)addr, (int)v); };
  auto x3 = [](uint32_t a, uint32_t b, uint32_t d) { return __builtin_amdgcn_bitop3_b32(a, b, d, 0x96); };
#pragma unroll
  for (int r = 0; r < 24; r++) {
    const uint32_t t0 = bp(c.col[0], lo), t1 = bp(c.col[1], lo), t2 = bp(c.col[2], lo), t3 = bp(c.col[3], lo);
    const uint32_t u0 = bp(c.col[0], hi), u1 = bp(c.col[1], hi), u2 = bp(c.col[2], hi), u3 = bp(c.col[3], hi);
    const uint32_t cl = x3(x3(lo, t0, t1), t2, t3), ch = x3(x3(hi, u0, u1), u2, u3);
    const uint32_t ml = bp(c.rm, cl), mh = bp(c.rm, ch), pl = bp(c.rp, cl), ph = bp(c.rp, ch);
    lo = x3(lo, ml, __builtin_amdgcn_alignbit(pl, ph, 31));
    hi = x3(hi, mh, __builtin_amdgcn_alignbit(ph, pl, 31));
    const uint32_t L_ = c.swap ? hi : lo, H_ = c.swap ? lo : hi;
    const uint32_t rl = __builtin_amdgcn_alignbit(L_, H_, c.s), rh = __builtin_amdgcn_alignbit(H_, L_, c.s);
    const uint32_t a0 = bp(c.b0, rl), a1 = bp(c.b1, rl), a2 = bp(c.b2, rl);
    const uint32_t h0 = bp(c.b0, rh), h1 = bp(c.b1, rh), h2 = bp(c.b2, rh);
    lo = __builtin_amdgcn_bitop3_b32(a0, a1, a2, 0xD2) ^ ((uint32_t)RC[r] & c.m0);
    hi = __builtin_amdgcn_bitop3_b32(h0, h1, h2, 0xD2) ^ ((uint32_t)(RC[r] >> 32) & c.m0);
  }
#else
  (void)lo, (void)hi, (void)c;
#endif
}

P2_HD void dig_to_elems(const dig_t &d, gl_t out[4]) {
  const uint64_t M56 = 0x00FFFFFFFFFFFFFFULL;
  out[0] = d.w[0] & M56;
  out[1] = ((d.w[0] >> 56) | (d.w[1] << 8)) & M56;
  out[2] = ((d.w[1] >> 48) | (d.w[2] << 16)) & M56;
  out[3] = ((d.w[2] >> 40) | ((d.w[3] & 0xFF) << 24)) & 0xFFFFFFFFULL;
}

template <int NEED = 12>
P2_HD void keccak_permutation12(gl_t st[12]) {
  uint64_t h[4];
  keccak256_words(st, 12, h);
  int got = 0;
  for (;;) {
    for (int i = 0; i < 4 && got < NEED; i++)
      if (h[i] < GL_P) st[got++] = h[i];
    if (got >= NEED) break;
    uint64_t h2[4];
    keccak256_words(h, 4, h2);
    for (int i = 0; i < 4; i++) h[i] = h2[i];
  }
}

}
```

acvm-backend-plonky2_amd/csrc/kf_check.py:

```python
#!/usr/bin/env python3
import os
import re
import subprocess
import sys
import tempfile

here = os.path.dirname(os.path.abspath(__file__))
inc = open(os.path.join(here, "keccak_fixed.inc")).read()
base = int(re.search(r"#define P2_KF_BASE (\d+)", inc).group(1))
top = int(re.search(r"#define P2_KF_TOP (\d+)", inc).group(1))
hipcc = sys.argv[1] if len(sys.argv) > 1 else "hipcc"
arch = sys.argv[2] if len(sys.argv) > 2 else "gfx950"
flags = [f for f in sys.argv[3:] if f not in ("-fPIC", "-c") and not f.startswith("--offload-arch")] or ["-O3", "-std=c++17", "-Wno-pass-failed", "-Wno-inline-asm"]
with tempfile.NamedTemporaryFile(suffix=".s") as f:
    subprocess.run([hipcc] + flags + [f"--offload-arch={arch}", "--cuda-device-only", "-S", os.path.join(here, "merkle.hip"), "-o", f.name],
                   check=True, capture_output=True)
    lines = [l.strip() for l in open(f.name)]
bad = 0
names = [l[:-1].split(":")[0] for l in lines if re.match(r"^_Z\w*kf_kernel\w*:", l)]
assert names, "no *_kf_kernel found"
for name in names:
    i = [k for k, l in enumerate(lines) if l.startswith(name + ":")][0]
    ends = [k for k in range(i, len(lines)) if re.match(r"^\.Lfunc_end\d+:", lines[k]) or lines[k].startswith(".size\t" + name + ",") or lines[k].startswith(".size " + name + ",")]
    assert ends, f"no end marker for {name}"
    inasm, mx, endpgm, barriers = False, 0, 0, 0
    for l in lines[i:ends[0]]:
        if l.startswith("s_endpgm"):
            endpgm += 1
        if l.startswith("s_barrier"):
            barriers += 1
        if "ASMSTART" in l:
            inasm = True
        elif "ASMEND" in l:
            inasm = False
        elif not inasm and l and not l.startswith((";", ".")) and not l.endswith(":"):
            regs = [int(x) for x in re.findall(r"\bv(\d+)\b", l)] + [int(b) for _, b in re.findall(r"v\[(\d+):(\d+)\]", l)]
            if regs:
                mx = max(mx, max(regs))
    scratch = [int(m.group(1)) for l in lines if (m := re.match(r"\.set " + re.escape(name) + r"\.private_seg_size, (\d+)", l))]
    nfree = None
    k0 = [k for k, l in enumerate(lines) if l.startswith(".amdhsa_kernel " + name)]
    if k0:
        for l in lines[k0[0]:k0[0] + 80]:
            m = re.match(r"\.amdhsa_next_free_vgpr\s+(\S+)", l)
            if m:
                try:
                    nfree = int(m.group(1))
                except ValueError:
                    sym = [int(mm.group(1)) for ll in lines if (mm := re.match(r"\.set " + re.escape(name) + r"\.num_vgpr, (\d+)", ll))]
                    nfree = sym[0] if sym else None
                break
    want_barriers = 2 if re.search(r"hash_lde_leaves_kf_kernelILb[01]ELi2E", name) else None
    ok = mx < base and (not scratch or scratch[0] == 0) and endpgm >= 1 and nfree is not None and nfree >= top and \
        (want_barriers is None or barriers == want_barriers)
    print(f"{name[:60]:60s} compiler registers up to v{mx} (state v{base}..v{top - 1}), scratch {scratch[0] if scratch else '?'} B, "
          f"next_free_vgpr {nfree}, s_endpgm x{endpgm}, s_barrier x{barriers}: {'ok' if ok else 'VIOLATION'}")
    bad += not ok
sys.exit(1 if bad else 0)
```

acvm-backend-plonky2_amd/csrc/merkle.hip:

```cpp
#include "internal.hpp"
#include "treeplan.hpp"

namespace p2 {

__device__ __forceinline__ dig_t poseidon_digest(const gl_t *st) {
  dig_t d;
  d.w[0] = st[0]; d.w[1] = st[1]; d.w[2] = st[2]; d.w[3] = st[3];
  return d;
}
template <class F>
__device__ __forceinline__ dig_t poseidon_sponge(uint32_t nwords, F get, const gl_t *prc) {
  gl_t st[12];
#pragma unroll
  for (int i = 0; i < 12; i++) st[i] = 0;
  for (uint32_t off = 0; off < nwords; off += 8) {
#pragma unroll
    for (int w = 0; w < 8; w++)
      if (off + w < nwords) st[w] = get(off + w);
    poseidon_permute_dev(st, prc);
  }
  return poseidon_digest(st);
}
__device__ __forceinline__ dig_t poseidon_two_to_one(const dig_t &l, const dig_t &r, const gl_t *prc) {
  gl_t st[12] = {l.w[0], l.w[1], l.w[2], l.w[3], r.w[0], r.w[1], r.w[2], r.w[3], 0, 0, 0, 0};
  poseidon_permute_dev(st, prc);
  return poseidon_digest(st);
}

template <bool PREFETCH = true, class F>
__device__ __forceinline__ dig_t sponge_hash(uint32_t nwords, F get) {
  uint64_t st[25];
#pragma unroll
  for (int i = 0; i < 25; i++) st[i] = 0;
  uint32_t off = 0;
  if constexpr (PREFETCH) {
    uint64_t nxt[17];
    const bool first_full = nwords >= 17;
    if (first_full) {
#pragma unroll
      for (int w = 0; w < 17; w++) nxt[w] = get(w);
    }
    while (nwords - off >= 17) {
#pragma unroll
      for (int w = 0; w < 17; w++) st[w] ^= nxt[w];
      off += 17;
      if (nwords - off >= 17) {
#pragma unroll
        for (int w = 0; w < 17; w++) nxt[w] = get(off + w);
      }
      keccak_f1600(st);
    }
  } else {
    while (nwords - off >= 17) {
#pragma unroll
      for (int w = 0; w < 17; w++) st[w] ^= get(off + w);
      off += 17;
      keccak_f1600(st);
    }
  }
  const uint32_t rem = nwords - off;
#pragma unroll
  for (int w = 0; w < 17; w++) {
    if ((uint32_t)w < rem) st[w] ^= get(off + w);
    if ((uint32_t)w == rem) st[w] ^= 0x01ULL;
  }
  st[16] ^= 0x8000000000000000ULL;
  keccak_f1600(st);
  return dig_from_state(st);
}

template <int H = 0, bool PREFETCH = true, class F>
__device__ __forceinline__ dig_t hash_or_noop(uint32_t nwords, F get, const gl_t *prc = nullptr) {
  constexpr uint32_t COPIED = H == 1 ? 4 : 3;
  if (H == 1 ? nwords <= 4 : nwords * 8 <= 25) {
    dig_t d;
#pragma unroll
    for (uint32_t j = 0; j < 4; j++) d.w[j] = j < COPIED && j < nwords ? get(j) : 0;
    return d;
  }
  if constexpr (H == 1) return poseidon_sponge(nwords, get, prc);
  else return sponge_hash<PREFETCH>(nwords, get);
}

__device__ __forceinline__ gl_t virt_get(const VirtCols &v, uint32_t i, gl_t Lk, const gl_t *base, size_t n) {
  if (i >= v.first) {
    const uint32_t cl = ld_uniform(v.cls + i);
    if (cl < 2u) return cl == 1u ? gl_mul(ld_uniform(v.val + i), Lk) : (gl_t)0;
  }
  return base[(size_t)i * n];
}
template <bool V>
struct LeafRow {
  const size_t &n;
  const gl_t *base;
  const VirtCols &v;
  gl_t Lk = 0;
  __device__ __forceinline__ LeafRow(const gl_t *lde, uint32_t cols, const size_t &n_, uint32_t c, size_t k, const VirtCols &v_)
      : n(n_), base(lde + (size_t)c * cols * n + k), v(v_) {
    if constexpr (V) Lk = v.basis ? v.basis[(size_t)(v.coset_first + c * v.coset_stride) * n + k] : (gl_t)0;
  }
  __device__ __forceinline__ gl_t operator()(uint32_t i) const {
    if constexpr (V) return virt_get(v, i, Lk, base, n);
    else return base[(size_t)i * n];
  }
};
template <int H, bool V>
__global__ __launch_bounds__(256, V ? 4 : 1) void hash_lde_leaves_kernel(const gl_t *__restrict__ lde, uint32_t cols, uint32_t d,
                                                              dig_t *__restrict__ dig, const gl_t *__restrict__ prc, const VirtCols v) {
  const size_t n = (size_t)1 << d;
  const size_t k = (size_t)blockIdx.x * blockDim.x + threadIdx.x;
  const uint32_t c = blockIdx.y;
  if (k >= n) return;
  const LeafRow<V> row(lde, cols, n, c, k, v);
  dig[(size_t)c * n + k] = hash_or_noop<H, !V>(cols, row, prc);
}

__device__ __forceinline__ void kf_zero() {
  static_for<0, 25>([&](auto ic) { P2_KF_SET(decltype(ic)::value, 0u, 0u); });
}
template <int W0, int W1, class F>
__device__ __forceinline__ void kf_absorb_group(uint32_t off, F get) {
  uint64_t x[W1 - W0];
#pragma unroll
  for (int w = W0; w < W1; w++) x[w - W0] = get(off + w);
  static_for<W0, W1>([&](auto wc) {
    constexpr int w = decltype(wc)::value;
    const uint64_t xw = x[w - W0];
    const uint32_t lo = (uint32_t)xw, hi = (uint32_t)(xw >> 32);
    P2_KF_XOR(w, lo, hi);
  });
}
template <bool SPLIT, class F>
__device__ __forceinline__ void kf_absorb(uint32_t off, uint32_t rem, F get) {
  if (rem >= 17) {
    if constexpr (SPLIT) {
      kf_absorb_group<0, 6>(off, get);
      kf_absorb_group<6, 12>(off, get);
      kf_absorb_group<12, 17>(off, get);
    } else {
      kf_absorb_group<0, 17>(off, get);
    }
  } else {
    static_for<0, 17>([&](auto wc) {
      constexpr int w = decltype(wc)::value;
      if ((uint32_t)w <= rem) {
        const uint64_t xw = (uint32_t)w < rem ? get(off + w) : (uint64_t)1;
        const uint32_t lo = (uint32_t)xw, hi = (uint32_t)(xw >> 32);
        P2_KF_XOR(w, lo, hi);
      }
    });
    P2_KF_XOR(16, 0u, 0x80000000u);
  }
}
__device__ __forceinline__ dig_t kf_digest() {
  uint32_t l0, h0, l1, h1, l2, h2, l3, h3;
  P2_KF_GET(0, l0, h0);
  P2_KF_GET(1, l1, h1);
  P2_KF_GET(2, l2, h2);
  P2_KF_GET(3, l3, h3);
  dig_t dg;
  dg.w[0] = ((uint64_t)h0 << 32) | l0;
  dg.w[1] = ((uint64_t)h1 << 32) | l1;
  dg.w[2] = ((uint64_t)h2 << 32) | l2;
  dg.w[3] = l3 & 0xFFu;
  (void)h3;
  return dg;
}
__device__ __forceinline__ void kf_set_two_to_one(const dig_t &l, const dig_t &r) {
  uint64_t w[7];
  w[0] = l.w[0];
  w[1] = l.w[1];
  w[2] = l.w[2];
  w[3] = (l.w[3] & 0xFFULL) | (r.w[0] << 8);
  w[4] = (r.w[0] >> 56) | (r.w[1] << 8);
  w[5] = (r.w[1] >> 56) | (r.w[2] << 8);
  w[6] = (r.w[2] >> 56) | ((r.w[3] & 0xFFULL) << 8) | (0x01ULL << 16);
  static_for<0, 7>([&](auto ic) {
    constexpr int i = decltype(ic)::value;
    const uint64_t x = w[i];
    const uint32_t lo = (uint32_t)x, hi = (uint32_t)(x >> 32);
    P2_KF_SET(i, lo, hi);
  });
  static_for<7, 25>([&](auto ic) {
    constexpr int i = decltype(ic)::value;
    P2_KF_SET(i, 0u, (i == 16 ? 0x80000000u : 0u));
  });
}
template <bool V, int LV>
__global__ __launch_bounds__(256) P2_KF_KERNEL_ATTR void hash_lde_leaves_kf_kernel(const gl_t *__restrict__ lde, uint32_t cols, uint32_t d,
                                                                                   dig_t *__restrict__ dig, dig_t *__restrict__ lvl1,
                                                                                   dig_t *__restrict__ lvl2, const VirtCols v) {
  __shared__ dig_t xch1[LV ? 2 : 1][64], xch2[64];
  const size_t n = (size_t)1 << d;
  const uint32_t g = threadIdx.x >> 6, t = threadIdx.x & 63u;
  const size_t k = LV ? (size_t)blockIdx.x * 64 + t + (size_t)g * (n >> 2) : (size_t)blockIdx.x * blockDim.x + threadIdx.x;
  const uint32_t c = blockIdx.y;
  if (!LV && k >= n) return;
  const LeafRow<V> row(lde, cols, n, c, k, v);
  kf_zero();
  uint64_t x[V ? 1 : 17];
  auto load_block = [&](uint32_t off) {
    if constexpr (!V) {
      const uint32_t rem = cols - off;
#pragma unroll
      for (int w = 0; w < 17; w++) x[w] = (uint32_t)w < rem ? row(off + w) : ((uint32_t)w == rem ? (uint64_t)1 : (uint64_t)0);
    }
  };
  load_block(0);
  uint32_t off = 0, stage = 0;
  for (;;) {
    bool complete = true;
    off = __builtin_amdgcn_readfirstlane(off);
    if (stage == 0) {
      const uint32_t rem = cols - off;
      complete = rem < 17;
      if constexpr (!V) {
        static_for<0, 17>([&](auto wc) {
          constexpr int w = decltype(wc)::value;
          const uint64_t xw = x[w];
          const uint32_t lo = (uint32_t)xw, hi = (uint32_t)(xw >> 32);
          P2_KF_XOR(w, lo, hi);
        });
        if (complete) P2_KF_XOR(16, 0u, 0x80000000u);
        off += 17;
        if (!complete) load_block(off);
      } else {
        kf_absorb<true>(off, rem, row);
        off += 17;
      }
    }
    P2_KECCAK_FIXED_PERMUTE();
    if (!complete) continue;
    const dig_t dg = kf_digest();
    if (stage == 0) dig[(size_t)c * n + k] = dg;
    else if (stage == 1) lvl1[(size_t)c * (n >> 1) + k] = dg;
    else lvl2[(size_t)c * (n >> 2) + k] = dg;
    if (stage == (uint32_t)LV) break;
    dig_t r;
    if (stage == 0) {
      if (g >= 2) xch1[g & 1][t] = dg;
      __syncthreads();
      if (g >= 2) break;
      r = xch1[g & 1][t];
    } else {
      if (g == 1) xch2[t] = dg;
      __syncthreads();
      if (g == 1) break;
      r = xch2[t];
    }
    kf_set_two_to_one(dg, r);
    if constexpr (!V) {
#pragma unroll
      for (int w = 0; w < 17; w++) x[w] = 0;
    }
    stage++;
  }
}
template <int PH>
__device__ __forceinline__ dig_t kf_two_to_one(const dig_t &l, const dig_t &r) {
  kf_set_two_to_one(l, r);
  if constexpr (PH == 0) P2_KECCAK_FIXED_PERMUTE_PH(0);
  else P2_KECCAK_FIXED_PERMUTE_PH(1);
  return kf_digest();
}
template <int PH>
__global__ __launch_bounds__(256) P2_KF_KERNEL_ATTR void merkle_level_kf_kernel(const dig_t *__restrict__ in, dig_t *__restrict__ out, uint32_t m) {
  const uint32_t half = m >> 1;
  const uint32_t k = blockIdx.x * blockDim.x + threadIdx.x;
  const uint32_t c = blockIdx.y;
  if (k >= half) return;
  const dig_t l = in[(size_t)c * m + k], r = in[(size_t)c * m + k + half];
  out[(size_t)c * half + k] = kf_two_to_one<PH>(l, r);
}
__global__ __launch_bounds__(256) P2_KF_KERNEL_ATTR void merkle_levels_kf_kernel(dig_t *lvl, uint32_t cosets, uint32_t m, uint32_t levels) {
  __shared__ dig_t nodes[4][64];
  const uint32_t mf = m >> levels, bpc = mf >> 6;
  const uint32_t c = blockIdx.x / bpc, t = threadIdx.x & 63u, g = threadIdx.x >> 6;
  const uint32_t k = (blockIdx.x % bpc) * 64 + t;
  uint32_t cnt = 1u << levels;
#pragma unroll 1
  for (uint32_t lv = 0; lv < levels; lv++) {
    const uint32_t half = cnt >> 1;
    if (g < half) {
      dig_t l, r;
      if (lv == 0) {
        const dig_t *in = lvl + (size_t)c * m;
        l = in[k + (size_t)g * mf];
        r = in[k + (size_t)(g + half) * mf];
      } else {
        l = nodes[g][t];
        r = nodes[g + half][t];
      }
      const dig_t o = kf_two_to_one<0>(l, r);
      lvl[(size_t)cosets * m + (size_t)c * (m >> 1) + k + (size_t)g * mf] = o;
      nodes[g][t] = o;
    }
    __syncthreads();
    lvl += (size_t)cosets * m;
    m >>= 1;
    cnt = half;
  }
}
__global__ __launch_bounds__(256) void merkle_coop_kernel(dig_t *lvl, uint32_t cosets, uint32_t m, uint32_t levels, dig_t *mirror,
                                                          uint32_t cap_per) {
  __shared__ uint64_t nodes[16][4];
  const uint32_t mf = m >> levels;
  const uint32_t c = blockIdx.x / mf, k0 = blockIdx.x % mf;
  const uint32_t lane = threadIdx.x & 63u, L = lane & 31u, slot = (threadIdx.x >> 6) * 2 + (lane >> 5);
  const KeccakCoopLane cl = keccak_coop_lane(lane);
  uint32_t cnt = 1u << levels;
  for (uint32_t lv = 0; lv < levels; lv++) {
    const uint32_t half = cnt >> 1;
    if (slot < half) {
      uint64_t p = 0, q = 0;
      if (L < 7) {
        if (lv == 0) {
          const dig_t *in = lvl + (size_t)c * m;
          const dig_t *l = in + k0 + (size_t)slot * mf, *r = in + k0 + (size_t)(slot + half) * mf;
          p = L < 4 ? l->w[L] : r->w[L - 4];
          if (L >= 3) q = r->w[L - 3];
        } else {
          p = L < 4 ? nodes[slot][L] : nodes[slot + half][L - 4];
          if (L >= 3) q = nodes[slot + half][L - 3];
        }
      }
      uint64_t w = L < 3 ? p : (L == 3 ? (p & 0xFFULL) : (p >> 56));
      if (L >= 3 && L < 7) w |= (L == 6 ? ((q & 0xFFULL) << 8) | (1ULL << 16) : (q << 8));
      if (L >= 7) w = L == 16 ? 0x8000000000000000ULL : 0ULL;
      uint32_t lo = (uint32_t)w, hi = (uint32_t)(w >> 32);
      keccak_f1600_coop(lo, hi, cl);
      if (L < 4) {
        const uint64_t o = L == 3 ? (uint64_t)(lo & 0xFFu) : (((uint64_t)hi << 32) | lo);
        lvl[(size_t)cosets * m + (size_t)c * (m >> 1) + k0 + (size_t)slot * mf].w[L] = o;
        if (mirror != nullptr && (m >> 1) == cap_per) mirror[(size_t)c * cap_per + k0 + (size_t)slot * mf].w[L] = o;
        nodes[slot][L] = o;
      }
    }
    __syncthreads();
    lvl += (size_t)cosets * m;
    m >>= 1;
    cnt = half;
  }
}

template <bool V>
__global__ __launch_bounds__(256) P2_KF_KERNEL_ATTR void hash_lde_absorb_kf_kernel(const gl_t *__restrict__ lde, uint32_t cols, uint32_t d,
                                                                                   uint32_t blk0, uint32_t nblk, int first, int last,
                                                                                   uint64_t *__restrict__ state, dig_t *__restrict__ dig, const VirtCols v) {
  const size_t n = (size_t)1 << d;
  const size_t k = (size_t)blockIdx.x * blockDim.x + threadIdx.x;
  const uint32_t c = blockIdx.y;
  if (k >= n) return;
  const LeafRow<V> row(lde, cols, n, c, k, v);
  uint64_t *sp = state + (size_t)c * 25 * n + k;
  if (first) kf_zero();
  else
    static_for<0, 25>([&](auto ic) {
      constexpr int i = decltype(ic)::value;
      const uint64_t x = sp[(size_t)i * n];
      P2_KF_SET(i, (uint32_t)x, (uint32_t)(x >> 32));
    });
  const uint32_t steps = nblk + (last ? 1u : 0u);
  for (uint32_t b = 0; b < steps; b++) {
    const uint32_t off = 17 * (blk0 + b);
    kf_absorb<true>(off, b < nblk ? 17u : cols - off, row);
    P2_KECCAK_FIXED_PERMUTE();
  }
  if (last) {
    dig[(size_t)c * n + k] = kf_digest();
  } else {
    static_for<0, 25>([&](auto ic) {
      constexpr int i = decltype(ic)::value;
      uint32_t lo, hi;
      P2_KF_GET(i, lo, hi);
      sp[(size_t)i * n] = ((uint64_t)hi << 32) | lo;
    });
  }
}

template <bool V>
__global__ __launch_bounds__(256) void hash_lde_absorb_kernel(const gl_t *__restrict__ lde, uint32_t cols, uint32_t d,
                                                              uint32_t blk0, uint32_t nblk, int first, int last,
                                                              uint64_t *__restrict__ state, dig_t *__restrict__ dig, const VirtCols v) {
  const size_t n = (size_t)1 << d;
  const size_t k = (size_t)blockIdx.x * blockDim.x + threadIdx.x;
  const uint32_t c = blockIdx.y;
  if (k >= n) return;
  const LeafRow<V> row(lde, cols, n, c, k, v);
  uint64_t *sp = state + (size_t)c * 25 * n + k;
  uint64_t st[25];
#pragma unroll
  for (int i = 0; i < 25; i++) st[i] = first ? 0 : sp[(size_t)i * n];
  for (uint32_t b = 0; b < nblk; b++) {
    const uint32_t i0 = 17 * (blk0 + b);
#pragma unroll
    for (int w = 0; w < 17; w++) st[w] ^= row(i0 + w);
    keccak_f1600(st);
  }
  if (last) {
    const uint32_t off = 17 * (blk0 + nblk), rem = cols - off;
#pragma unroll
    for (int w = 0; w < 17; w++) {
      if ((uint32_t)w < rem) st[w] ^= row(off + w);
      if ((uint32_t)w == rem) st[w] ^= 0x01ULL;
    }
    st[16] ^= 0x8000000000000000ULL;
    keccak_f1600(st);
    dig[(size_t)c * n + k] = dig_from_state(st);
  } else {
#pragma unroll
    for (int i = 0; i < 25; i++) sp[(size_t)i * n] = st[i];
  }
}

__global__ __launch_bounds__(256) void hash_rows_kernel(const gl_t *__restrict__ rows, size_t n_rows, uint32_t row_len,
                                                        dig_t *__restrict__ dig) {
  const size_t r = (size_t)blockIdx.x * blockDim.x + threadIdx.x;
  if (r >= n_rows) return;
  const gl_t *base = rows + r * row_len;
  dig[r] = hash_or_noop(row_len, [&](uint32_t i) { return base[i]; });
}

template <int H>
__global__ __launch_bounds__(256) void hash_fri_leaves_kernel(const gl_t *__restrict__ vals, uint32_t lg_npc,
                                                              uint32_t ab, dig_t *__restrict__ dig, const gl_t *__restrict__ prc) {
  const uint32_t npc = 1u << lg_npc, per = npc >> ab;
  const uint32_t kl = blockIdx.x * blockDim.x + threadIdx.x;
  const uint32_t r = blockIdx.y;
  if (kl >= per) return;
  const gl_t *c0 = vals + (size_t)r * 2 * npc, *c1 = c0 + npc;
  dig[(size_t)r * per + kl] = hash_or_noop<H>(2u << ab, [&](uint32_t w) {
    uint32_t t = w >> 1;
    uint32_t k = bitrev32(t, ab) * per + kl;
    return (w & 1) ? c1[k] : c0[k];
  }, prc);
}

__global__ __launch_bounds__(256) void hash_fri_leaves_coop_poseidon_kernel(const gl_t *__restrict__ vals, uint32_t lg_npc, uint32_t ab,
                                                                            uint32_t cosets, dig_t *__restrict__ dig,
                                                                            const gl_t *__restrict__ prc) {
  const uint32_t npc = 1u << lg_npc, per = npc >> ab;
  const uint32_t lane = threadIdx.x & 63u, i = lane & 15u;
  const uint32_t slot = blockIdx.x * 16 + (threadIdx.x >> 6) * 4 + (lane >> 4);
  if (slot >= cosets * per) return;
  const uint32_t r = slot / per, kl = slot % per;
  const gl_t *c0 = vals + (size_t)r * 2 * npc, *c1 = c0 + npc;
  const PoseidonCoopLane cl = poseidon_coop_lane(lane);
  gl_t x = 0;
  for (uint32_t b = 0; b < (2u << ab) / 8; b++) {
    if (i < 8) {
      const uint32_t w = 8 * b + i, k = bitrev32(w >> 1, ab) * per + kl;
      x = (w & 1) ? c1[k] : c0[k];
    }
    x = poseidon_permute_coop(x, prc, cl);
  }
  if (i < 4) dig[(size_t)r * per + kl].w[i] = x;
}

template <int H>
__global__ __launch_bounds__(256) void merkle_level_kernel(const dig_t *__restrict__ in, dig_t *__restrict__ out,
                                                           uint32_t m, const gl_t *__restrict__ prc) {
  const uint32_t half = m >> 1;
  const uint32_t k = blockIdx.x * blockDim.x + threadIdx.x;
  const uint32_t c = blockIdx.y;
  if (k >= half) return;
  const dig_t l = in[(size_t)c * m + k], r = in[(size_t)c * m + k + half];
  static_assert(H == 1, "Keccak levels: merkle_level_kf_kernel");
  out[(size_t)c * half + k] = poseidon_two_to_one(l, r, prc);
}

__global__ __launch_bounds__(256) void merkle_coop_poseidon_kernel(dig_t *lvl, uint32_t cosets, uint32_t m, uint32_t levels,
                                                                   const gl_t *__restrict__ prc) {
  __shared__ uint64_t nodes[32][4];
  const uint32_t mf = m >> levels;
  const uint32_t c = blockIdx.x / mf, k0 = blockIdx.x % mf;
  const uint32_t lane = threadIdx.x & 63u, i = lane & 15u, slot = (threadIdx.x >> 6) * 4 + (lane >> 4);
  const PoseidonCoopLane cl = poseidon_coop_lane(lane);
  uint32_t cnt = 1u << levels;
  for (uint32_t lv = 0; lv < levels; lv++) {
    const uint32_t half = cnt >> 1;
    if (slot < half) {
      gl_t x = 0;
      if (i < 8) {
        const uint32_t j = slot + (i < 4 ? 0u : half), w = i & 3u;
        x = lv == 0 ? lvl[(size_t)c * m + k0 + (size_t)j * mf].w[w] : nodes[j][w];
      }
      x = poseidon_permute_coop(x, prc, cl);
      if (i < 4) {
        lvl[(size_t)cosets * m + (size_t)c * (m >> 1) + k0 + (size_t)slot * mf].w[i] = x;
        nodes[slot][i] = x;
      }
    }
    __syncthreads();
    lvl += (size_t)cosets * m;
    m >>= 1;
    cnt = half;
  }
}

bool tree_levels(hipStream_t st, dig_t *lvl, uint32_t cosets, uint32_t m, uint32_t cap_per, const gl_t *prc, dig_t *host_mirror) {
  const TreePlan plan = tree_plan(prc ? 1 : 0, cosets, m, cap_per);
  for (uint32_t i = 0; i < plan.count; i++) {
    const TreeStep &s = plan.step[i];
    const dim3 grid(s.grid_x, s.grid_y), block(s.block);
    dig_t *out = lvl + (size_t)cosets * s.m;
    ProfScope ps(tree_kernel_name(s.kernel), s.bytes(cosets));
    switch (s.kernel) {
      case TreeKernel::LevelPoseidon: hipLaunchKernelGGL(merkle_level_kernel<1>, grid, block, 0, st, lvl, out, s.m, prc); break;
      case TreeKernel::LevelKfMany: hipLaunchKernelGGL(merkle_level_kf_kernel<1>, grid, block, 0, st, lvl, out, s.m); break;
      case TreeKernel::LevelKfLone: hipLaunchKernelGGL(merkle_level_kf_kernel<0>, grid, block, 0, st, lvl, out, s.m); break;
      case TreeKernel::LevelsKf: hipLaunchKernelGGL(merkle_levels_kf_kernel, grid, block, 0, st, lvl, cosets, s.m, s.levels); break;
      case TreeKernel::CoopKeccak: hipLaunchKernelGGL(merkle_coop_kernel, grid, block, 0, st, lvl, cosets, s.m, s.levels, host_mirror, cap_per); break;
      case TreeKernel::CoopPoseidon: hipLaunchKernelGGL(merkle_coop_poseidon_kernel, grid, block, 0, st, lvl, cosets, s.m, s.levels, prc); break;
    }
    for (uint32_t q = 0; q < s.levels; q++) lvl += (size_t)cosets * (s.m >> q);
  }
  return host_mirror != nullptr && plan.cap_from_coop_keccak();
}

static bool leaf_levels_on() {
  static const bool on = env_flag("P2GPU_LEAF_LEVELS", true);
  return on;
}
static bool has_virtual(const VirtCols *virt, uint32_t cols) { return virt && virt->cls && virt->first < cols; }

struct LeafVariant {
  const char *name;
  void (*plain)(const gl_t *, uint32_t, uint32_t, dig_t *, const gl_t *, VirtCols);
  void (*fixed)(const gl_t *, uint32_t, uint32_t, dig_t *, dig_t *, dig_t *, VirtCols);
  uint32_t levels;
};
#define P2_LEAF_PLAIN(...) LeafVariant{#__VA_ARGS__, __VA_ARGS__, nullptr, 0}
#define P2_LEAF_FIXED(LV, ...) LeafVariant{#__VA_ARGS__, nullptr, __VA_ARGS__, LV}
uint32_t hash_lde_leaves(hipStream_t st, const gl_t *lde, uint32_t cols, uint32_t d, uint32_t cosets, dig_t *dig, const gl_t *prc,
                         const VirtCols *virt, dig_t *lvl1, dig_t *lvl2) {
  size_t n = (size_t)1 << d;
  uint32_t threads = n >= 256 ? 256 : 64;
  const bool kf = !prc && cols * 8 > 25 && n >= 256;
  const bool virt_on = has_virtual(virt, cols);
  const bool lv2 = kf && virt_on && lvl1 != nullptr && lvl2 != nullptr && cols > 3 * 17 && leaf_levels_on();
  const LeafVariant k = prc   ? (virt_on ? P2_LEAF_PLAIN(hash_lde_leaves_kernel<1, true>) : P2_LEAF_PLAIN(hash_lde_leaves_kernel<1, false>))
                        : !kf ? (virt_on ? P2_LEAF_PLAIN(hash_lde_leaves_kernel<0, true>) : P2_LEAF_PLAIN(hash_lde_leaves_kernel<0, false>))
                        : !virt_on ? P2_LEAF_FIXED(0, hash_lde_leaves_kf_kernel<false, 0>)
                        : lv2      ? P2_LEAF_FIXED(2, hash_lde_leaves_kf_kernel<true, 2>)
                                   : P2_LEAF_FIXED(0, hash_lde_leaves_kf_kernel<true, 0>);
  const double node_bytes = k.levels ? 96.0 * cosets * (double)(n / 2 + n / 4) : 0.0;
  const dim3 grid((uint32_t)((n + threads - 1) / threads), cosets);
  const VirtCols vc = virt_on ? *virt : VirtCols();
  ProfScope ps(k.name, (8.0 * cols + 32.0) * cosets * (double)n + node_bytes);
  if (k.fixed) hipLaunchKernelGGL(k.fixed, grid, dim3(threads), 0, st, lde, cols, d, dig, lvl1, lvl2, vc);
  else hipLaunchKernelGGL(k.plain, grid, dim3(threads), 0, st, lde, cols, d, dig, prc, vc);
  return k.levels;
}
#undef P2_LEAF_PLAIN
#undef P2_LEAF_FIXED
void hash_lde_absorb(hipStream_t st, const gl_t *lde, uint32_t cols, uint32_t d, uint32_t cosets, uint32_t blk0,
                     uint32_t nblk, bool first, bool last, uint64_t *state, dig_t *dig, const VirtCols *virt) {
  size_t n = (size_t)1 << d;
  uint32_t threads = n >= 256 ? 256 : 64;
  const bool virt_on = has_virtual(virt, cols), kf = n >= 256;
  ProfScope ps("hash_lde_absorb_kernel", (8.0 * 17 * nblk + (first ? 0 : 200) + (last ? 32 + 8.0 * (cols - 17 * (blk0 + nblk)) : 200)) *
                                             cosets * (double)n);
  hipLaunchKernelGGL(kf ? (virt_on ? hash_lde_absorb_kf_kernel<true> : hash_lde_absorb_kf_kernel<false>)
                        : (virt_on ? hash_lde_absorb_kernel<true> : hash_lde_absorb_kernel<false>),
                     dim3((n + threads - 1) / threads, cosets), dim3(threads), 0, st, lde, cols, d, blk0, nblk, first ? 1 : 0, last ? 1 : 0,
                     state, dig, virt_on ? *virt : VirtCols());
}
void hash_rows(hipStream_t st, const gl_t *rows, size_t n_rows, uint32_t row_len, dig_t *dig) {
  hipLaunchKernelGGL(hash_rows_kernel, dim3((n_rows + 255) / 256), dim3(256), 0, st, rows, n_rows, row_len, dig);
}
void hash_fri_leaves(hipStream_t st, const gl_t *vals, uint32_t lg_npc, uint32_t cosets, uint32_t ab, dig_t *dig, const gl_t *prc) {
  uint32_t per = (1u << lg_npc) >> ab;
  uint32_t threads = per >= 256 ? 256 : 64;
  ProfScope ps(prc ? "hash_fri_leaves_kernel<1>" : "hash_fri_leaves_kernel<0>", (16.0 * (1u << ab) + 32.0) * cosets * (double)per);
  if (prc && (2u << ab) >= 8 && (size_t)cosets * per <= 4096)
    hipLaunchKernelGGL(hash_fri_leaves_coop_poseidon_kernel, dim3((cosets * per + 15) / 16), dim3(256), 0, st, vals, lg_npc, ab, cosets, dig, prc);
  else
    hipLaunchKernelGGL(prc ? hash_fri_leaves_kernel<1> : hash_fri_leaves_kernel<0>, dim3((per + threads - 1) / threads, cosets), dim3(threads), 0,
                       st, vals, lg_npc, ab, dig, prc);
}

}
```

acvm-backend-plonky2_amd/prover.py:

```python
import ctypes
import os

import numpy as np

_HERE = os.path.dirname(os.path.abspath(__file__))
_LIB = None

UINT64_MAX = (1 << 64) - 1


class P2GpuError(RuntimeError):
    def __init__(self, code, msg):
        super().__init__(f"p2gpu error {code}: {msg}")
        self.code = code


class _Timings(ctypes.Structure):
    _fields_ = [
        ("wires_commit_ms", ctypes.c_double),
        ("zs_commit_ms", ctypes.c_double),
        ("quotient_ms", ctypes.c_double),
        ("openings_ms", ctypes.c_double),
        ("fri_ms", ctypes.c_double),
        ("total_ms", ctypes.c_double),
        ("h2d_ms", ctypes.c_double),
        ("pow_witness", ctypes.c_uint64),
    ]


_ALLGATHER_FN = ctypes.CFUNCTYPE(ctypes.c_int, ctypes.c_void_p, ctypes.c_uint64, ctypes.c_uint64, ctypes.c_uint64)


class _DevBytes:

    def __init__(self, ptr, nbytes):
        self.__cuda_array_interface__ = {"shape": (int(nbytes),), "typestr": "|u1", "data": (int(ptr), False),
                                         "version": 2}


def lib_path():
    return os.environ.get("P2GPU_LIBRARY") or os.path.join(_HERE, "libp2gpu.so")


def load_library():
    global _LIB
    if _LIB is not None:
        return _LIB
    path = lib_path()
    if not os.path.exists(path):
        raise P2GpuError(-8, f"{path} is missing: build it with __graft_entry__.build() (hipcc, gfx950)")
    try:
        import torch
    except Exception:
        pass
    lib = ctypes.CDLL(path)
    vp, sz, u8p = ctypes.c_void_p, ctypes.c_size_t, ctypes.c_void_p
    lib.p2gpu_last_error.restype = ctypes.c_char_p
    lib.p2gpu_init.argtypes = [ctypes.POINTER(ctypes.c_int), ctypes.c_int]
    lib.p2gpu_circuit_create.argtypes = [u8p, sz, ctypes.POINTER(vp)]
    lib.p2gpu_circuit_destroy.argtypes = [vp]
    lib.p2gpu_circuit_destroy.restype = None
    lib.p2gpu_circuit_cap.argtypes = [vp, u8p]
    lib.p2gpu_circuit_digest.argtypes = [vp, u8p]
    lib.p2gpu_proof_size_bound.argtypes = [vp]
    lib.p2gpu_proof_size_bound.restype = sz
    lib.p2gpu_circuit_device.argtypes = [vp]
    lib.p2gpu_circuit_hash_bytes.argtypes = [vp]
    lib.p2gpu_prove.argtypes = [vp, vp, vp, ctypes.c_uint32, u8p, ctypes.POINTER(sz), ctypes.POINTER(_Timings)]
    lib.p2gpu_prove_dev.argtypes = lib.p2gpu_prove.argtypes
    lib.p2gpu_prove_routed.argtypes = lib.p2gpu_prove.argtypes
    a = lib.p2gpu_prove.argtypes
    lib.p2gpu_prove_sparse.argtypes = [a[0], a[1], ctypes.c_uint32, ctypes.c_void_p, ctypes.c_uint32] + list(a[2:])
    lib.p2gpu_fill_witness.argtypes = [vp, vp]
    lib.p2gpu_witness_plan_create.argtypes = [vp, vp, sz, ctypes.POINTER(vp)]
    lib.p2gpu_witness_plan_build.argtypes = [vp, vp, sz, ctypes.POINTER(vp)]
    lib.p2gpu_witness_plan_export.argtypes = [vp, vp, vp, vp, vp]
    lib.p2gpu_witness_plan_create_gen.argtypes = [vp, vp, sz, vp, sz, ctypes.POINTER(vp)]
    lib.p2gpu_witness_plan_build_gen.argtypes = [vp, vp, sz, vp, sz, ctypes.POINTER(vp)]
    lib.p2gpu_witness_plan_export_generators.argtypes = [vp, vp, ctypes.POINTER(sz)]
    lib.p2gpu_witness_plan_destroy.argtypes = [vp]
    lib.p2gpu_witness_plan_destroy.restype = None
    lib.p2gpu_witness_plan_info.argtypes = [vp, vp, vp]
    lib.p2gpu_generate_witness.argtypes = [vp, vp, vp]
    lib.p2gpu_generate_witness_batch.argtypes = [vp, vp, sz, vp, vp, vp]
    lib.p2gpu_prove_seeds.argtypes = [vp, vp, vp, ctypes.c_uint32, u8p, ctypes.POINTER(sz), ctypes.POINTER(_Timings)]
    lib.p2gpu_verify.argtypes = [vp, u8p, sz]
    lib.p2gpu_circuit_export_vk.argtypes = [vp, u8p, ctypes.POINTER(sz)]
    lib.p2gpu_circuit_export_vk_plonky2.argtypes = [vp, u8p, ctypes.POINTER(sz)]
    lib.p2gpu_verifier_create_plonky2.argtypes = [u8p, sz, ctypes.c_int, ctypes.POINTER(vp)]
    lib.p2gpu_verifier_create.argtypes = [u8p, sz, ctypes.POINTER(vp)]
    lib.p2gpu_proof_compress.argtypes = [vp, u8p, sz, u8p, ctypes.POINTER(sz)]
    lib.p2gpu_proof_decompress.argtypes = [vp, u8p, sz, u8p, ctypes.POINTER(sz)]
    lib.p2gpu_verify_compressed.argtypes = [vp, u8p, sz]
    lib.p2gpu_circuit_set.argtypes = [vp, ctypes.c_char_p, ctypes.c_uint64]
    lib.p2gpu_circuit_set_shard.argtypes = [vp, ctypes.c_int, ctypes.c_int, _ALLGATHER_FN, vp]
    lib.p2gpu_shard_unique_id.argtypes = [vp]
    lib.p2gpu_circuit_set_shard_rccl.argtypes = [vp, ctypes.c_int, ctypes.c_int, vp]
    lib.p2gpu_kernel_stats.argtypes = [vp, ctypes.c_char_p, vp, vp, vp, ctypes.c_int]
    lib.p2gpu_ifft_batch.argtypes = [vp, sz, ctypes.c_uint, vp]
    lib.p2gpu_lde_batch.argtypes = [vp, sz, ctypes.c_uint, ctypes.c_uint, vp]
    lib.p2gpu_commit_values.argtypes = [vp, sz, ctypes.c_uint, ctypes.c_uint, ctypes.c_uint, u8p]
    lib.p2gpu_hash_rows.argtypes = [vp, sz, sz, u8p]
    lib.p2gpu_field_selftest.argtypes = [vp, vp, sz, vp]
    lib.p2gpu_field_selftest16.argtypes = [vp, vp, sz, vp]
    lib.p2gpu_device_info.argtypes = [ctypes.c_char_p, sz, ctypes.POINTER(ctypes.c_int), ctypes.POINTER(sz)]
    lib.p2gpu_peer_access.argtypes = [ctypes.POINTER(ctypes.c_int), ctypes.c_int]
    lib.p2gpu_circuit_create_on.argtypes = [u8p, sz, ctypes.c_int, ctypes.POINTER(vp)]
    lib.p2gpu_circuit_build.argtypes = [vp, vp, ctypes.c_uint32, vp, vp, vp, sz, ctypes.c_uint32, ctypes.POINTER(vp)]
    lib.p2gpu_circuit_build_on.argtypes = [vp, vp, ctypes.c_uint32, vp, vp, vp, sz, ctypes.c_uint32, ctypes.c_int, ctypes.POINTER(vp)]
    lib.p2gpu_circuit_export_blob.argtypes = [vp, u8p, ctypes.POINTER(sz)]
    lib.p2gpu_peer_access.restype = ctypes.c_int
    lib.p2gpu_host_alloc.argtypes = [sz]
    lib.p2gpu_host_alloc.restype = vp
    lib.p2gpu_host_free.argtypes = [vp]
    lib.p2gpu_host_free.restype = None
    _LIB = lib
    return lib


def _check(rc):
    if rc != 0:
        raise P2GpuError(rc, load_library().p2gpu_last_error().decode(errors="replace"))


def _u64(a):
    a = np.ascontiguousarray(a, dtype=np.uint64)
    return a


def init(devices=(0,)):
    lib = load_library()
    devs = (ctypes.c_int * len(devices))(*[int(d) for d in devices])
    _check(lib.p2gpu_init(devs, len(devices)))


class _HostBlock:

    def __init__(self, nbytes):
        self._lib = load_library()
        self.ptr = self._lib.p2gpu_host_alloc(nbytes)
        if not self.ptr:
            raise P2GpuError(-3, self._lib.p2gpu_last_error().decode(errors="replace"))
        self.buf = (ctypes.c_uint8 * max(1, nbytes)).from_address(self.ptr)

    def __del__(self):
        if getattr(self, "ptr", None):
            self.buf = None
            self._lib.p2gpu_host_free(self.ptr)
            self.ptr = None


def host_array(shape, dtype=np.uint64):
    shape = (shape,) if isinstance(shape, int) else tuple(shape)
    nbytes = int(np.prod(shape, dtype=np.int64)) * np.dtype(dtype).itemsize
    blk = _HostBlock(nbytes)
    arr = np.frombuffer(blk.buf, dtype=dtype, count=nbytes // np.dtype(dtype).itemsize).reshape(shape)
    _HOST_BLOCKS[id(blk)] = blk
    arr.flags.writeable = True
    return arr


_HOST_BLOCKS = {}


def host_free(arr):
    addr = arr.ctypes.data
    for k, blk in list(_HOST_BLOCKS.items()):
        if blk.ptr == addr:
            del _HOST_BLOCKS[k]
            blk.__del__()
            return
    raise P2GpuError(-1, "host_free: not an array from host_array")


def device_info():
    lib = load_library()
    name = ctypes.create_string_buffer(256)
    cu = ctypes.c_int()
    mem = ctypes.c_size_t()
    _check(lib.p2gpu_device_info(name, 256, ctypes.byref(cu), ctypes.byref(mem)))
    return {"name": name.value.decode(), "cu_count": cu.value, "hbm_bytes": mem.value}


def peer_access():
    lib = load_library()
    n = lib.p2gpu_peer_access(None, 0)
    if n < 0:
        _check(n)
    m = (ctypes.c_int * (n * n))()
    _check(min(0, lib.p2gpu_peer_access(m, n * n)))
    return [[int(m[a * n + b]) for b in range(n)] for a in range(n)]


class ProofWithPublicInputs:

    def __init__(self, data, timings=None):
        self._data = bytes(data)
        self.timings = timings or {}

    def to_bytes(self):
        return self._data

    def __len__(self):
        return len(self._data)

    def __eq__(self, other):
        return isinstance(other, ProofWithPublicInputs) and self._data == other._data


class CircuitData:

    def __init__(self, blob, device=None):
        lib = load_library()
        self._lib = lib
        self._blob = np.ascontiguousarray(np.frombuffer(blob, dtype=np.uint8) if not isinstance(blob, np.ndarray) else blob)
        hdr = self._blob[:256].view(np.uint32)
        self.degree_bits = int(hdr[2])
        self.num_wires = int(hdr[3])
        self.num_routed_wires = int(hdr[4])
        self.rate_bits = int(hdr[9])
        self.cap_height = int(hdr[10])
        self.num_public_inputs = int(hdr[24])
        self._h = ctypes.c_void_p()
        if device is None:
            _check(lib.p2gpu_circuit_create(self._blob.ctypes.data, self._blob.nbytes, ctypes.byref(self._h)))
        else:
            _check(lib.p2gpu_circuit_create_on(self._blob.ctypes.data, self._blob.nbytes, int(device), ctypes.byref(self._h)))
        self._bound = lib.p2gpu_proof_size_bound(self._h)

    @classmethod
    def from_blob(cls, blob):
        return cls(blob)

    @classmethod
    def build(cls, degree_bits, gates, row_gate, row_constants, copies, num_public_inputs=0, num_wires=234, num_routed_wires=80,
              num_challenges=2, quotient_degree_factor=8, rate_bits=3, cap_height=4, proof_of_work_bits=16, num_query_rounds=28,
              hasher=0, device=None):
        lib = load_library()
        bp, gd, rg, rc, cp = _build_args(degree_bits, gates, row_gate, row_constants, copies, num_public_inputs, num_wires, num_routed_wires,
                                         num_challenges, quotient_degree_factor, rate_bits, cap_height, proof_of_work_bits, num_query_rounds)
        self = cls.__new__(cls)
        self._lib = lib
        self._blob = None
        self.degree_bits, self.num_wires, self.num_routed_wires = int(degree_bits), int(num_wires), int(num_routed_wires)
        self.rate_bits, self.cap_height, self.num_public_inputs = int(rate_bits), int(cap_height), int(num_public_inputs)
        self._h = ctypes.c_void_p()
        args = [ctypes.byref(bp), gd, len(gates), rg.ctypes.data, rc.ctypes.data if rc.size else None, cp.ctypes.data if cp.size else None,
                len(cp), int(hasher)]
        if device is None:
            _check(lib.p2gpu_circuit_build(*args, ctypes.byref(self._h)))
        else:
            _check(lib.p2gpu_circuit_build_on(*args, int(device), ctypes.byref(self._h)))
        self._bound = lib.p2gpu_proof_size_bound(self._h)
        return self

    def to_blob(self):
        ln = ctypes.c_size_t(0)
        _check(self._lib.p2gpu_circuit_export_blob(self._h, None, ctypes.byref(ln)))
        out = np.zeros(ln.value, dtype=np.uint8)
        _check(self._lib.p2gpu_circuit_export_blob(self._h, out.ctypes.data, ctypes.byref(ln)))
        return out[:ln.value]

    @property
    def degree(self):
        return 1 << self.degree_bits

    def constants_sigmas_cap(self):
        out = np.zeros(self.hash_bytes() << self.cap_height, dtype=np.uint8)
        _check(self._lib.p2gpu_circuit_cap(self._h, out.ctypes.data))
        return out.tobytes()

    def circuit_digest(self):
        out = np.zeros(self.hash_bytes(), dtype=np.uint8)
        _check(self._lib.p2gpu_circuit_digest(self._h, out.ctypes.data))
        return out.tobytes()

    def hash_bytes(self):
        return int(self._lib.p2gpu_circuit_hash_bytes(self._h))

    def device_index(self):
        return int(self._lib.p2gpu_circuit_device(self._h))

    def set(self, key, value):
        _check(self._lib.p2gpu_circuit_set(self._h, key.encode(), ctypes.c_uint64(value)))

    def set_shard(self, rank, world, group=None, transport=None):
        import torch
        import torch.distributed as dist

        backend = dist.get_backend(group) if (world > 1 or (dist.is_available() and dist.is_initialized())) else None
        if transport is None:
            transport = "rccl" if backend == "nccl" else "callback"
        if transport == "rccl":
            idbuf = np.zeros(128, dtype=np.uint8)
            if rank == 0:
                _check(self._lib.p2gpu_shard_unique_id(idbuf.ctypes.data))
            if world > 1:
                if backend == "nccl":
                    t = torch.from_numpy(idbuf).cuda()
                    dist.broadcast(t, src=dist.get_global_rank(group, 0) if group is not None else 0, group=group)
                    idbuf = t.cpu().numpy()
                else:
                    t = torch.from_numpy(idbuf)
                    dist.broadcast(t, src=dist.get_global_rank(group, 0) if group is not None else 0, group=group)
                    idbuf = t.numpy()
            idbuf = np.ascontiguousarray(idbuf)
            _check(self._lib.p2gpu_circuit_set_shard_rccl(self._h, rank, world, idbuf.ctypes.data))
            self._shard_cb = None
            self.shard = (rank, world)
            return
        if world > 1:

            def _allgather(_ctx, send, recv, nbytes):
                try:
                    s = torch.as_tensor(_DevBytes(send, nbytes), device="cuda")
                    r = torch.as_tensor(_DevBytes(recv, nbytes * world), device="cuda")
                    if backend == "nccl":
                        dist.all_gather_into_tensor(r, s, group=group)
                    else:
                        out = torch.empty(nbytes * world, dtype=torch.uint8)
                        dist.all_gather_into_tensor(out, s.cpu(), group=group)
                        r.copy_(out)
                    torch.cuda.synchronize()
                    return 0
                except Exception as e:
                    self._shard_error = e
                    return -1

            self._shard_cb = _ALLGATHER_FN(_allgather)
        else:
            self._shard_cb = _ALLGATHER_FN(0)
        _check(self._lib.p2gpu_circuit_set_shard(self._h, rank, world, self._shard_cb, None))
        self.shard = (rank, world)

    def kernel_stats(self):
        cap = 64
        names = ctypes.create_string_buffer(64 * cap)
        ms = np.zeros(cap, dtype=np.float64)
        by = np.zeros(cap, dtype=np.float64)
        ln = np.zeros(cap, dtype=np.uint64)
        k = self._lib.p2gpu_kernel_stats(self._h, names, ms.ctypes.data, by.ctypes.data, ln.ctypes.data, cap)
        out = {}
        for i in range(max(k, 0)):
            nm = names.raw[64 * i:64 * (i + 1)].split(b"\0", 1)[0].decode()
            out[nm] = {"ms": float(ms[i]), "bytes": float(by[i]), "launches": int(ln[i])}
        return out

    def prove(self, wires, public_inputs=()):
        pis = _u64(np.array(list(public_inputs), dtype=np.uint64))
        out = np.zeros(self._bound, dtype=np.uint8)
        plen = ctypes.c_size_t(out.nbytes)
        tm = _Timings()
        expect = self.num_wires * self.degree
        if hasattr(wires, "data_ptr") and getattr(wires, "is_cuda", False):
            if wires.numel() != expect or wires.element_size() != 8 or not wires.is_contiguous():
                raise P2GpuError(-7, "wires tensor must be contiguous int64/uint64 [num_wires][degree]")
            if wires.device.index != self.device_index():
                raise P2GpuError(-7, f"wires tensor lives on cuda:{wires.device.index}, the circuit on cuda:{self.device_index()}")
            rc = self._lib.p2gpu_prove_dev(self._h, ctypes.c_void_p(wires.data_ptr()), pis.ctypes.data, len(pis),
                                           out.ctypes.data, ctypes.byref(plen), ctypes.byref(tm))
        else:
            w = _u64(wires)
            if w.size != expect:
                raise P2GpuError(-7, f"wires must be [num_wires={self.num_wires}][degree={self.degree}]")
            rc = self._lib.p2gpu_prove(self._h, w.ctypes.data, pis.ctypes.data, len(pis), out.ctypes.data,
                                       ctypes.byref(plen), ctypes.byref(tm))
        _check(rc)
        t = {f: getattr(tm, f) for f, _ in _Timings._fields_}
        return ProofWithPublicInputs(out[:plen.value].tobytes(), t)

    def fill_witness(self, wires_dev):
        if not (hasattr(wires_dev, "data_ptr") and getattr(wires_dev, "is_cuda", False)):
            raise P2GpuError(-7, "fill_witness needs a torch tensor on the GPU")
        if wires_dev.numel() != self.num_wires * self.degree or not wires_dev.is_contiguous():
            raise P2GpuError(-7, "wires tensor must be contiguous [num_wires][degree]")
        _check(self._lib.p2gpu_fill_witness(self._h, ctypes.c_void_p(wires_dev.data_ptr())))
        return wires_dev

    def witness_plan(self, seed_cells, compile="host", generators=None):
        return WitnessPlan(self, seed_cells, compile=compile, generators=generators)

    def prove_routed(self, routed, public_inputs=()):
        pis = _u64(np.array(list(public_inputs), dtype=np.uint64))
        r = _u64(routed)
        if r.size != self.num_routed_wires * self.degree:
            raise P2GpuError(-7, f"routed must be [num_routed_wires={self.num_routed_wires}][degree={self.degree}]")
        out = np.zeros(self._bound, dtype=np.uint8)
        plen = ctypes.c_size_t(out.nbytes)
        tm = _Timings()
        _check(self._lib.p2gpu_prove_routed(self._h, r.ctypes.data, pis.ctypes.data, len(pis), out.ctypes.data,
                                            ctypes.byref(plen), ctypes.byref(tm)))
        return ProofWithPublicInputs(out[:plen.value].tobytes(), {f: getattr(tm, f) for f, _ in _Timings._fields_})

    def prove_sparse(self, wires, ncols, row, public_inputs=(), tail=None):
        pis = _u64(np.array(list(public_inputs), dtype=np.uint64))
        W, n = self.num_wires, self.degree
        w = _u64(wires)
        if not (0 <= ncols <= W and 0 <= row < n):
            raise P2GpuError(-7, f"prove_sparse: ncols {ncols} of {W} wires, row {row} of {n}")
        if tail is None:
            if w.size != W * n:
                raise P2GpuError(-7, f"wires must be [num_wires={W}][degree={n}] when no tail is given")
            full = w.reshape(W, n)
            tail = np.ascontiguousarray(full[ncols:, row])
            w = np.ascontiguousarray(full[:ncols]).reshape(-1)
        else:
            tail = _u64(np.asarray(tail, dtype=np.uint64))
        if ncols > W or w.size != ncols * n or tail.size != W - ncols:
            raise P2GpuError(-7, f"prove_sparse: [{ncols}][{n}] dense columns and {W - ncols} tail values expected")
        out = np.zeros(self._bound, dtype=np.uint8)
        plen = ctypes.c_size_t(out.nbytes)
        tm = _Timings()
        _check(self._lib.p2gpu_prove_sparse(self._h, w.ctypes.data if w.size else None, ncols,
                                            tail.ctypes.data if tail.size else None, row,
                                            pis.ctypes.data, len(pis), out.ctypes.data, ctypes.byref(plen), ctypes.byref(tm)))
        return ProofWithPublicInputs(out[:plen.value].tobytes(), {f: getattr(tm, f) for f, _ in _Timings._fields_})

    def verify(self, proof):
        _verify(self._lib, self._h, proof)

    def verifier_data(self):
        return VerifierCircuitData(self.verifier_blob())

    def verifier_blob(self):
        n = ctypes.c_size_t(0)
        _check(self._lib.p2gpu_circuit_export_vk(self._h, None, ctypes.byref(n)))
        out = np.zeros(n.value, dtype=np.uint8)
        _check(self._lib.p2gpu_circuit_export_vk(self._h, out.ctypes.data, ctypes.byref(n)))
        return out[:n.value].tobytes()

    def close(self):
        if getattr(self, "_h", None) and self._h.value:
            self._lib.p2gpu_circuit_destroy(self._h)
            self._h = ctypes.c_void_p()

    def __del__(self):
        try:
            self.close()
        except Exception:
            pass


class WitnessPlan:

    GENERATOR_KINDS = {"equality": 0}

    def __init__(self, circuit, seed_cells, compile="host", generators=None):
        if compile not in ("host", "device"):
            raise P2GpuError(-7, f'compile must be "host" or "device", not {compile!r}')
        self._cd, self._lib = circuit, circuit._lib
        cells = np.ascontiguousarray(np.array(list(seed_cells), dtype=np.int64).reshape(-1, 2))
        if cells.size and (cells.min() < 0 or cells.max() >= 1 << 32):
            raise P2GpuError(-7, "seed cells are (row, col) pairs of unsigned 32-bit numbers")
        cells = cells.astype(np.uint32)
        self.num_seeds = len(cells)
        self._h = ctypes.c_void_p()
        if generators is None:
            make = self._lib.p2gpu_witness_plan_build if compile == "device" else self._lib.p2gpu_witness_plan_create
            _check(make(circuit._h, cells.ctypes.data if cells.size else None, len(cells), ctypes.byref(self._h)))
            return
        recs = np.zeros((len(generators), 9), dtype=np.int64)
        for i, (kind, gcells) in enumerate(generators):
            recs[i, 0] = self.GENERATOR_KINDS.get(kind, kind) if isinstance(kind, str) else kind
            recs[i, 1:] = np.array(list(gcells), dtype=np.int64).reshape(8)
        if recs.size and (recs.min() < 0 or recs.max() >= 1 << 32):
            raise P2GpuError(-7, "a generator is a kind and four (row, col) cells of unsigned 32-bit numbers")
        recs = np.ascontiguousarray(recs.astype(np.uint32))
        make = self._lib.p2gpu_witness_plan_build_gen if compile == "device" else self._lib.p2gpu_witness_plan_create_gen
        _check(make(circuit._h, cells.ctypes.data if cells.size else None, len(cells), recs.ctypes.data if recs.size else None, len(recs),
                    ctypes.byref(self._h)))

    def _values(self, values):
        v = _u64(np.array([int(x) for x in values], dtype=np.uint64))
        if v.size != self.num_seeds:
            raise P2GpuError(-7, f"{self.num_seeds} seed values expected, {v.size} given")
        return v

    def info(self):
        counts, ms = np.zeros(5, dtype=np.uint64), np.zeros(2, dtype=np.float64)
        _check(self._lib.p2gpu_witness_plan_info(self._h, counts.ctypes.data, ms.ctypes.data))
        out = dict(zip(("ops", "levels", "widest_level", "slots", "seeds"), (int(x) for x in counts)))
        out.update(compile_ms=float(ms[0]), walk_ms=float(ms[1]))
        return out

    def export(self):
        sizes = (ctypes.c_size_t * 3)()
        _check(self._lib.p2gpu_witness_plan_export(self._h, None, None, None, sizes))
        cell_slot = np.zeros(sizes[0], dtype=np.uint32)
        ops = np.zeros(max(1, sizes[1]), dtype=np.uint64)
        level_off = np.zeros(sizes[2], dtype=np.uint32)
        _check(self._lib.p2gpu_witness_plan_export(self._h, cell_slot.ctypes.data, ops.ctypes.data, level_off.ctypes.data, sizes))
        return cell_slot.reshape(self._cd.num_routed_wires, self._cd.degree), ops[:sizes[1]], level_off

    def export_generators(self):
        count = ctypes.c_size_t()
        _check(self._lib.p2gpu_witness_plan_export_generators(self._h, None, ctypes.byref(count)))
        table = np.zeros((count.value, 4), dtype=np.uint32)
        if count.value:
            _check(self._lib.p2gpu_witness_plan_export_generators(self._h, table.ctypes.data, ctypes.byref(count)))
        return table

    def generate(self, values):
        import torch

        v = self._values(values)
        cd = self._cd
        out = torch.empty((cd.num_wires, cd.degree), dtype=torch.int64, device=f"cuda:{cd.device_index()}")
        _check(self._lib.p2gpu_generate_witness(self._h, v.ctypes.data if v.size else None, ctypes.c_void_p(out.data_ptr())))
        return out

    def generate_batch(self, values_list):
        import torch

        rows = [self._values(v) for v in values_list]
        if not rows:
            raise P2GpuError(-7, "generate_batch needs at least one set of values")
        v = np.ascontiguousarray(np.stack(rows))
        cd = self._cd
        out = torch.empty((len(rows), cd.num_wires, cd.degree), dtype=torch.int64, device=f"cuda:{cd.device_index()}")
        status = np.zeros(len(rows), dtype=np.intc)
        bad = np.zeros((len(rows), 2), dtype=np.uint32)
        rc = self._lib.p2gpu_generate_witness_batch(self._h, v.ctypes.data if v.size else None, len(rows), ctypes.c_void_p(out.data_ptr()),
                                                    status.ctypes.data, bad.ctypes.data)
        if rc != -5:
            _check(rc)
        return out, [int(s) for s in status], [(int(r), int(c)) if s else None for s, (r, c) in zip(status, bad)]

    def prove_batch(self, values_list, public_inputs=None):
        wires, status, bad = self.generate_batch(values_list)
        out = []
        for b, st in enumerate(status):
            if st:
                out.append(P2GpuError(st, "unsatisfiable: witness %d of the batch contradicts itself at cell (row %d, column %d)" % (b, *bad[b])))
                continue
            try:
                out.append(self._cd.prove(wires[b], public_inputs[b] if public_inputs is not None else ()))
            except P2GpuError as e:
                out.append(e)
        return out

    def prove(self, values, public_inputs=()):
        v = self._values(values)
        pis = _u64(np.array(list(public_inputs), dtype=np.uint64))
        out = np.zeros(self._cd._bound, dtype=np.uint8)
        plen = ctypes.c_size_t(out.nbytes)
        tm = _Timings()
        _check(self._lib.p2gpu_prove_seeds(self._h, v.ctypes.data if v.size else None, pis.ctypes.data, len(pis), out.ctypes.data,
                                           ctypes.byref(plen), ctypes.byref(tm)))
        return ProofWithPublicInputs(out[:plen.value].tobytes(), {f: getattr(tm, f) for f, _ in _Timings._fields_})

    def close(self):
        if getattr(self, "_h", None) and self._h.value:
            self._lib.p2gpu_witness_plan_destroy(self._h)
            self._h = ctypes.c_void_p()

    def __del__(self):
        try:
            self.close()
        except Exception:
            pass


def _verify(lib, handle, proof):
    data = proof.to_bytes() if hasattr(proof, "to_bytes") else bytes(proof)
    buf = np.frombuffer(data, dtype=np.uint8)
    _check(lib.p2gpu_verify(handle, buf.ctypes.data if buf.size else None, buf.size))


def _convert(fn, handle, data):
    buf = np.frombuffer(bytes(data), dtype=np.uint8)
    n = ctypes.c_size_t(0)
    _check(fn(handle, buf.ctypes.data if buf.size else None, buf.size, None, ctypes.byref(n)))
    out = np.zeros(max(n.value, 1), dtype=np.uint8)
    _check(fn(handle, buf.ctypes.data if buf.size else None, buf.size, out.ctypes.data, ctypes.byref(n)))
    return out[:n.value].tobytes()


class _ProofFormats:

    def compress(self, proof):
        data = proof.to_bytes() if hasattr(proof, "to_bytes") else bytes(proof)
        return _convert(self._lib.p2gpu_proof_compress, self._h, data)

    def decompress(self, compressed):
        return ProofWithPublicInputs(_convert(self._lib.p2gpu_proof_decompress, self._h, compressed))

    def verify_compressed(self, compressed):
        buf = np.frombuffer(bytes(compressed), dtype=np.uint8)
        _check(self._lib.p2gpu_verify_compressed(self._h, buf.ctypes.data if buf.size else None, buf.size))

    def to_plonky2_bytes(self):
        n = ctypes.c_size_t(0)
        _check(self._lib.p2gpu_circuit_export_vk_plonky2(self._h, None, ctypes.byref(n)))
        out = np.zeros(n.value, dtype=np.uint8)
        _check(self._lib.p2gpu_circuit_export_vk_plonky2(self._h, out.ctypes.data, ctypes.byref(n)))
        return out[:n.value].tobytes()


CircuitData.compress = _ProofFormats.compress
CircuitData.decompress = _ProofFormats.decompress
CircuitData.verify_compressed = _ProofFormats.verify_compressed
CircuitData.to_plonky2_vk_bytes = _ProofFormats.to_plonky2_bytes


class VerifierCircuitData(_ProofFormats):

    def __init__(self, blob):
        lib = load_library()
        self._lib = lib
        self._blob = np.ascontiguousarray(np.frombuffer(blob, dtype=np.uint8))
        self._h = ctypes.c_void_p()
        _check(lib.p2gpu_verifier_create(self._blob.ctypes.data, self._blob.nbytes, ctypes.byref(self._h)))
        self._read_header()

    @classmethod
    def from_plonky2_bytes(cls, vk, hasher=0):
        self = cls.__new__(cls)
        lib = load_library()
        self._lib = lib
        buf = np.ascontiguousarray(np.frombuffer(bytes(vk), dtype=np.uint8))
        self._h = ctypes.c_void_p()
        _check(lib.p2gpu_verifier_create_plonky2(buf.ctypes.data if buf.size else None, buf.size, int(hasher), ctypes.byref(self._h)))
        n = ctypes.c_size_t(0)
        _check(lib.p2gpu_circuit_export_vk(self._h, None, ctypes.byref(n)))
        self._blob = np.zeros(n.value, dtype=np.uint8)
        _check(lib.p2gpu_circuit_export_vk(self._h, self._blob.ctypes.data, ctypes.byref(n)))
        self._read_header()
        return self

    def _read_header(self):
        hdr = self._blob[:256].view(np.uint32)
        self.degree_bits = int(hdr[2])
        self.cap_height = int(hdr[10])
        self.num_public_inputs = int(hdr[24])

    def to_bytes(self):
        return self._blob.tobytes()

    def hash_bytes(self):
        return int(self._lib.p2gpu_circuit_hash_bytes(self._h))

    def circuit_digest(self):
        out = np.zeros(self.hash_bytes(), dtype=np.uint8)
        _check(self._lib.p2gpu_circuit_digest(self._h, out.ctypes.data))
        return out.tobytes()

    def constants_sigmas_cap(self):
        out = np.zeros(self.hash_bytes() << self.cap_height, dtype=np.uint8)
        _check(self._lib.p2gpu_circuit_cap(self._h, out.ctypes.data))
        return out.tobytes()

    def verify(self, proof):
        _verify(self._lib, self._h, proof)

    def close(self):
        if getattr(self, "_h", None) and self._h.value:
            self._lib.p2gpu_circuit_destroy(self._h)
            self._h = ctypes.c_void_p()

    def __del__(self):
        try:
            self.close()
        except Exception:
            pass


class _BuildParams(ctypes.Structure):
    _fields_ = [(k, ctypes.c_uint32) for k in ("degree_bits", "num_wires", "num_routed_wires", "num_challenges", "quotient_degree_factor",
                                                "rate_bits", "cap_height", "proof_of_work_bits", "num_query_rounds", "num_public_inputs")]


class _GateDecl(ctypes.Structure):
    _fields_ = [("kind", ctypes.c_uint32), ("p", ctypes.c_uint32 * 4), ("degree", ctypes.c_uint32), ("num_constants", ctypes.c_uint32)]


def _build_args(degree_bits, gates, row_gate, row_constants, copies, num_public_inputs, num_wires, num_routed_wires, num_challenges,
                quotient_degree_factor, rate_bits, cap_height, proof_of_work_bits, num_query_rounds):
    bp = _BuildParams(degree_bits, num_wires, num_routed_wires, num_challenges, quotient_degree_factor, rate_bits, cap_height,
                      proof_of_work_bits, num_query_rounds, num_public_inputs)
    gd = (_GateDecl * len(gates))()
    for i, (kind, ps, deg, nk) in enumerate(gates):
        gd[i].kind, gd[i].degree, gd[i].num_constants = kind, deg, nk
        for j, v in enumerate(tuple(ps) + (0,) * (4 - len(ps))):
            gd[i].p[j] = v
    rg = np.ascontiguousarray(row_gate, dtype=np.uint32)
    rc = np.ascontiguousarray(row_constants, dtype=np.uint64)
    cp = np.ascontiguousarray(copies, dtype=np.uint32).reshape(-1, 4)
    if rg.size != 1 << degree_bits:
        raise P2GpuError(-7, "row_gate must have 2^degree_bits entries")
    return bp, gd, rg, rc, cp


def build_blob(degree_bits, gates, row_gate, row_constants, copies, num_public_inputs=0, num_wires=234, num_routed_wires=80,
               num_challenges=2, quotient_degree_factor=8, rate_bits=3, cap_height=4, proof_of_work_bits=16, num_query_rounds=28):
    lib = load_library()
    lib.p2gpu_build_blob.argtypes = [ctypes.c_void_p, ctypes.c_void_p, ctypes.c_uint32, ctypes.c_void_p, ctypes.c_void_p, ctypes.c_void_p,
                                     ctypes.c_size_t, ctypes.c_void_p, ctypes.POINTER(ctypes.c_size_t)]
    bp, gd, rg, rc, cp = _build_args(degree_bits, gates, row_gate, row_constants, copies, num_public_inputs, num_wires, num_routed_wires,
                                     num_challenges, quotient_degree_factor, rate_bits, cap_height, proof_of_work_bits, num_query_rounds)
    ln = ctypes.c_size_t(0)
    args = [ctypes.byref(bp), gd, len(gates), rg.ctypes.data, rc.ctypes.data if rc.size else None, cp.ctypes.data if cp.size else None, len(cp)]
    _check(lib.p2gpu_build_blob(*args, None, ctypes.byref(ln)))
    out = np.zeros(ln.value, dtype=np.uint8)
    _check(lib.p2gpu_build_blob(*args, out.ctypes.data, ctypes.byref(ln)))
    return out[:ln.value]


def ifft_batch(vals):
    lib = load_library()
    v = _u64(vals)
    ncols, n = v.shape
    d = n.bit_length() - 1
    out = np.zeros_like(v)
    _check(lib.p2gpu_ifft_batch(v.ctypes.data, ncols, d, out.ctypes.data))
    return out


def lde_batch(coeffs, rate_bits=3):
    lib = load_library()
    c = _u64(coeffs)
    ncols, n = c.shape
    d = n.bit_length() - 1
    out = np.zeros((ncols, n << rate_bits), dtype=np.uint64)
    _check(lib.p2gpu_lde_batch(c.ctypes.data, ncols, d, rate_bits, out.ctypes.data))
    return out


def commit_values(vals, rate_bits=3, cap_height=4):
    lib = load_library()
    v = _u64(vals)
    ncols, n = v.shape
    d = n.bit_length() - 1
    out = np.zeros(25 << cap_height, dtype=np.uint8)
    _check(lib.p2gpu_commit_values(v.ctypes.data, ncols, d, rate_bits, cap_height, out.ctypes.data))
    return out.tobytes()


def field_selftest(a, b):
    lib = load_library()
    x = np.ascontiguousarray(a, dtype=np.uint64)
    y = np.ascontiguousarray(b, dtype=np.uint64)
    assert x.shape == y.shape and x.ndim == 1
    bad = np.zeros(16, dtype=np.uint64)
    _check(lib.p2gpu_field_selftest16(x.ctypes.data, y.ctypes.data, x.size, bad.ctypes.data))
    return bad


def hash_rows(rows):
    lib = load_library()
    r = _u64(rows)
    n_rows, row_len = r.shape
    out = np.zeros(25 * n_rows, dtype=np.uint8)
    _check(lib.p2gpu_hash_rows(r.ctypes.data, n_rows, row_len, out.ctypes.data))
    return out.reshape(n_rows, 25)
```

include/p2gpu.h:

```cpp
#ifndef P2GPU_H
#define P2GPU_H
#include <stddef.h>
#include <stdint.h>

#ifdef __cplusplus
extern "C" {
#endif

#define P2GPU_OK 0
#define P2GPU_E_BLOB -1
#define P2GPU_E_BUFFER -2
#define P2GPU_E_DEVICE -3
#define P2GPU_E_OPENING_IN_SUBGROUP -4
#define P2GPU_E_UNSATISFIED -5
#define P2GPU_E_CAP_MISMATCH -6
#define P2GPU_E_ARG -7
#define P2GPU_E_NOT_INIT -8
#define P2GPU_E_VERIFY -9

typedef struct p2gpu_circuit p2gpu_circuit;

typedef struct {
  double wires_commit_ms;
  double zs_commit_ms;
  double quotient_ms;
  double openings_ms;
  double fri_ms;
  double total_ms;
  double h2d_ms;
  uint64_t pow_witness;
} p2gpu_timings;

int p2gpu_init(const int *device_ids, int n_devices);
void *p2gpu_host_alloc(size_t bytes);
void p2gpu_host_free(void *p);

int p2gpu_circuit_create(const uint8_t *blob, size_t len, p2gpu_circuit **out);
int p2gpu_circuit_create_on(const uint8_t *blob, size_t len, int device_id, p2gpu_circuit **out);
void p2gpu_circuit_destroy(p2gpu_circuit *c);
int p2gpu_circuit_hash_bytes(const p2gpu_circuit *c);
int p2gpu_circuit_cap(const p2gpu_circuit *c, uint8_t *out);
int p2gpu_circuit_digest(const p2gpu_circuit *c, uint8_t *out);
int p2gpu_circuit_device(const p2gpu_circuit *c);
size_t p2gpu_proof_size_bound(const p2gpu_circuit *c);

int p2gpu_prove(p2gpu_circuit *c, const uint64_t *wires, const uint64_t *public_inputs, uint32_t n_pi,
                uint8_t *proof_out, size_t *proof_len, p2gpu_timings *opt_timings);
int p2gpu_prove_dev(p2gpu_circuit *c, const uint64_t *wires_dev, const uint64_t *public_inputs, uint32_t n_pi,
                    uint8_t *proof_out, size_t *proof_len, p2gpu_timings *opt_timings);
int p2gpu_fill_witness(p2gpu_circuit *c, uint64_t *wires_dev);
int p2gpu_prove_routed(p2gpu_circuit *c, const uint64_t *routed, const uint64_t *public_inputs, uint32_t n_pi,
                       uint8_t *proof_out, size_t *proof_len, p2gpu_timings *opt_timings);
int p2gpu_prove_sparse(p2gpu_circuit *c, const uint64_t *wires, uint32_t ncols, const uint64_t *tail, uint32_t row,
                       const uint64_t *public_inputs, uint32_t n_pi, uint8_t *proof_out, size_t *proof_len,
                       p2gpu_timings *opt_timings);

typedef struct p2gpu_witness_plan p2gpu_witness_plan;
int p2gpu_witness_plan_create(p2gpu_circuit *c, const uint32_t *seed_cells , size_t n_seeds,
                              p2gpu_witness_plan **out);
int p2gpu_witness_plan_build(p2gpu_circuit *c, const uint32_t *seed_cells , size_t n_seeds,
                             p2gpu_witness_plan **out);
#define P2GPU_GEN_EQUALITY 0
typedef struct { uint32_t kind; uint32_t cells[4][2];  } p2gpu_generator;
int p2gpu_witness_plan_create_gen(p2gpu_circuit *c, const uint32_t *seed_cells, size_t n_seeds,
                                  const p2gpu_generator *generators, size_t n_generators, p2gpu_witness_plan **out);
int p2gpu_witness_plan_build_gen(p2gpu_circuit *c, const uint32_t *seed_cells, size_t n_seeds,
                                 const p2gpu_generator *generators, size_t n_generators, p2gpu_witness_plan **out);
int p2gpu_witness_plan_export_generators(const p2gpu_witness_plan *p, uint32_t *table, size_t *n_generators);
int p2gpu_witness_plan_export(const p2gpu_witness_plan *p, uint32_t *cell_slot, uint64_t *ops, uint32_t *level_off, size_t sizes[3]);
void p2gpu_witness_plan_destroy(p2gpu_witness_plan *p);
int p2gpu_witness_plan_info(const p2gpu_witness_plan *p, uint64_t counts[5], double ms[2]);
int p2gpu_generate_witness(p2gpu_witness_plan *p, const uint64_t *seed_values, uint64_t *wires_dev_out);
int p2gpu_generate_witness_batch(p2gpu_witness_plan *p, const uint64_t *seed_values , size_t batch,
                                 uint64_t *wires_dev_out ,
                                 int *status ,
                                 uint32_t *bad_cells );
int p2gpu_prove_seeds(p2gpu_witness_plan *p, const uint64_t *seed_values, const uint64_t *public_inputs, uint32_t n_pi,
                      uint8_t *proof_out, size_t *proof_len, p2gpu_timings *opt_timings);

typedef struct {
  uint32_t degree_bits, num_wires, num_routed_wires, num_challenges, quotient_degree_factor, rate_bits, cap_height,
      proof_of_work_bits, num_query_rounds, num_public_inputs;
} p2gpu_build_params;
typedef struct {
  uint32_t kind, p[4], degree, num_constants;
} p2gpu_gate_decl;
int p2gpu_build_blob(const p2gpu_build_params *params, const p2gpu_gate_decl *gates, uint32_t num_gates, const uint32_t *row_gate,
                     const uint64_t *row_constants, const uint32_t *copies, size_t num_copies, uint8_t *blob_out,
                     size_t *blob_len);

int p2gpu_circuit_build(const p2gpu_build_params *params, const p2gpu_gate_decl *gates, uint32_t num_gates, const uint32_t *row_gate,
                        const uint64_t *row_constants, const uint32_t *copies, size_t num_copies, uint32_t hasher, p2gpu_circuit **out);
int p2gpu_circuit_build_on(const p2gpu_build_params *params, const p2gpu_gate_decl *gates, uint32_t num_gates, const uint32_t *row_gate,
                           const uint64_t *row_constants, const uint32_t *copies, size_t num_copies, uint32_t hasher, int device_id,
                           p2gpu_circuit **out);
int p2gpu_circuit_export_blob(const p2gpu_circuit *c, uint8_t *out, size_t *len);

int p2gpu_verify(const p2gpu_circuit *c, const uint8_t *proof, size_t len);
int p2gpu_circuit_export_vk(const p2gpu_circuit *c, uint8_t *out, size_t *len);
int p2gpu_verifier_create(const uint8_t *blob, size_t len, p2gpu_circuit **out);
int p2gpu_circuit_export_vk_plonky2(const p2gpu_circuit *c, uint8_t *out, size_t *len);
int p2gpu_verifier_create_plonky2(const uint8_t *vk, size_t len, int hasher, p2gpu_circuit **out);

int p2gpu_proof_compress(const p2gpu_circuit *c, const uint8_t *proof, size_t len, uint8_t *out, size_t *out_len);
int p2gpu_proof_decompress(const p2gpu_circuit *c, const uint8_t *cproof, size_t len, uint8_t *out, size_t *out_len);
int p2gpu_verify_compressed(const p2gpu_circuit *c, const uint8_t *cproof, size_t len);

int p2gpu_circuit_set(p2gpu_circuit *c, const char *key, uint64_t value);
int p2gpu_kernel_stats(p2gpu_circuit *c, char *names, double *ms, double *bytes, uint64_t *launches, int cap);

typedef int (*p2gpu_allgather_fn)(void *ctx, uint64_t send_dev, uint64_t recv_dev, uint64_t bytes_per_rank);
int p2gpu_circuit_set_shard(p2gpu_circuit *c, int rank, int world, p2gpu_allgather_fn fn, void *ctx);
int p2gpu_shard_unique_id(uint8_t id_out[128]);
int p2gpu_shard_assemble_cap(int world, unsigned rate_bits, unsigned cap_h, const uint8_t *gathered, uint8_t *cap_out);
int p2gpu_circuit_set_shard_rccl(p2gpu_circuit *c, int rank, int world, const uint8_t id[128]);

int p2gpu_ifft_batch(const uint64_t *vals, size_t ncols, unsigned d, uint64_t *coeffs_out);
int p2gpu_lde_batch(const uint64_t *coeffs, size_t ncols, unsigned d, unsigned rate_bits, uint64_t *lde_out);
int p2gpu_commit_values(const uint64_t *vals, size_t ncols, unsigned d, unsigned rate_bits, unsigned cap_h,
                        uint8_t *cap_out);
int p2gpu_hash_rows(const uint64_t *rows, size_t n_rows, size_t row_len, uint8_t *digests_out);
int p2gpu_field_selftest(const uint64_t *a, const uint64_t *b, size_t n, uint64_t bad_out[8]);
int p2gpu_field_selftest16(const uint64_t *a, const uint64_t *b, size_t n, uint64_t bad_out[16]);

const char *p2gpu_last_error(void);
int p2gpu_device_info(char *name_out, size_t name_cap, int *cu_count, size_t *hbm_bytes);
int p2gpu_peer_access(int *matrix_out, int cap);

#ifdef __cplusplus
}
#endif
#endif
```

Before: 233.4 proofs/sec.

## Specialize fixed-register Keccak permutation for node inputs and digest-only outputs

```diff
diff --git a/acvm-backend-plonky2_amd/__init__.py b/acvm-backend-plonky2_amd/__init__.py
--- a/acvm-backend-plonky2_amd/__init__.py
+++ b/acvm-backend-plonky2_amd/__init__.py
@@ -14,6 +14,10 @@
     lde_batch,
     commit_values,
     hash_rows,
+    keccak_nodes,
+    leaf_digests,
+    fri_leaves,
+    pow_min,
     field_selftest,
     lib_path,
     load_library,
diff --git a/acvm-backend-plonky2_amd/csrc/gen_keccak_fixed.py b/acvm-backend-plonky2_amd/csrc/gen_keccak_fixed.py
--- a/acvm-backend-plonky2_amd/csrc/gen_keccak_fixed.py
+++ b/acvm-backend-plonky2_amd/csrc/gen_keccak_fixed.py
@@ -4,6 +4,7 @@
 from gen_keccak_sched import RC, Op, ref_keccak_f, round_ops, schedule
 
 NTEMP = 36
+DIGEST_HALVES = 7
 
 
 def build(base):
@@ -31,7 +32,14 @@
             keep.append(o)
             needed.update(o.srcs)
     ops = list(reversed(keep))
-    return live, g_schedule(ops, live), cur_a
+    needed = set([v for p in cur_a for v in p][:DIGEST_HALVES])
+    for o in reversed(ops):
+        if o.dst in needed:
+            needed.update(o.srcs)
+    main, tail = [o for o in ops if o.dst in needed], [o for o in ops if o.dst not in needed]
+    assert all(o.dst.startswith("r23_") for o in tail)
+    main = g_schedule(main, live)
+    return live, main + g_schedule(tail, live + [o.dst for o in main]), cur_a, len(main)
 
 
 def g_schedule(ops, live_in, gap=1):
@@ -84,11 +92,12 @@
     free = list(range(base + 50, base + 50 + NTEMP))
     out = []
     conflicts = 0
+    homes_left = {base + i for i in range(50)}
     for t, o in enumerate(ops):
         srcs = [reg[s] for s in o.srcs]
         if o.kind in ("X3", "CHI") and len({r % 4 for r in srcs}) == 1:
             conflicts += 1
-        for s in set(o.srcs):
+        for s in dict.fromkeys(o.srcs):
             if last_use[s] == t:
                 free.append(reg[s])
         avoid_hard, avoid_soft = set(), set()
@@ -101,22 +110,29 @@
                 avoid_hard.add(banks[0])
             else:
                 avoid_soft.update(banks)
+        home = base + finals.index(o.dst) if o.dst in finals else -1
+        late = o.dst.startswith(("r22_", "r23_"))
         best = None
         for r_ in free:
             b = r_ % 4
-            score = (b in avoid_hard) * 100 + (b in avoid_soft) * 1
+            score = (b in avoid_hard) * 100 + (b in avoid_soft) * 1 - (r_ == home) * 50 + (late and r_ != home and r_ in homes_left) * 2
             if best is None or score < best[0]:
                 best = (score, r_)
         if best is None:
             raise SystemExit(f"out of registers at op {t} (NTEMP = {NTEMP})")
         free.remove(best[1])
+        homes_left.discard(home)
         reg[o.dst] = best[1]
         out.append((o, best[1], srcs))
+    want = {base + i: reg[v] for i, v in enumerate(finals)}
+    spare = [r_ for r_ in range(base + 50, base + 50 + NTEMP) if r_ not in set(want.values())]
+    return concrete(out), [reg[v] for v in finals], reg, parallel_moves(want, spare), \
+        parallel_moves(dict(list(want.items())[:DIGEST_HALVES]), spare), conflicts
+
+
+def parallel_moves(want, spare):
     moves = []
-    want = {base + i: reg[v] for i, v in enumerate(finals)}
     pending = {d: s for d, s in want.items() if d != s}
-    tmp = None
-    spare = [r_ for r_ in range(base + 50, base + 50 + NTEMP) if r_ not in set(want.values())]
     while pending:
         progressed = False
         for d, s in list(pending.items()):
@@ -131,30 +147,120 @@
             for k in pending:
                 if pending[k] == d:
                     pending[k] = tmp
-    return out, moves, conflicts
-
-
-def simulate(alloc, moves, st, base):
+    return moves
+
+
+def concrete(alloc):
+    out = []
+    for o, d, srcs in alloc:
+        if o.kind == "IOTA":
+            out.append(("XK", d, srcs, (RC[int(o.dst[1:].split("_")[0])] >> (32 * o.imm)) & 0xFFFFFFFF, o.dst))
+        else:
+            out.append((o.kind, d, srcs, o.imm, o.dst))
+    return out
+
+
+NODE_ZERO = range(7, 25)
+NODE_PAD = (16, "h", 0x80000000)
+
+
+def node_region(ins, reg):
+    zero = {f"a{i}{h}": (i, h) for i in NODE_ZERO for h in "lh"}
+    name_of = {r: v for v, r in reg.items() if v[0] == "a" and v[1:-1].isdigit()}
+    tz = {}
+    last_read = {}
+    E = 0
+    for t, (kind, d, srcs, imm, name) in enumerate(ins):
+        if name.startswith("r1_"):
+            break
+        if name.startswith("cin"):
+            E = t + 1
+        elif kind == "X3" and name.startswith("r0_t") and name_of.get(srcs[0]) in zero:
+            tz[name] = zero[name_of[srcs[0]]]
+        elif kind == "ROT" and name_of.get(srcs[0]) in tz:
+            assert name_of.get(srcs[1]) in tz
+            E = t + 1
+            last_read[name_of[srcs[0]]] = last_read[name_of[srcs[1]]] = t
+        name_of[d] = name
+    assert len(tz) == 2 * len(NODE_ZERO) and set(last_read) == set(tz)
+    last_of = {}
+    for name, (i, h) in tz.items():
+        last_of[(i % 5, h)] = name
+    a = lambda i, h: reg[f"a{i}{h}"]
+    alt, seen_c, holder, at = [], False, {}, {}
+    name_of = {r: v for v, r in reg.items() if v[0] == "a" and v[1:-1].isdigit()}
+    for t, (kind, d, srcs, imm, name) in enumerate(ins[:E]):
+        if name.startswith("cin"):
+            if not seen_c:
+                seen_c = True
+                for h in "lh":
+                    alt.append(("XOR", reg[f"cin0{h}"], [a(0, h), a(5, h)], 0, ""))
+                    alt.append(("XOR", reg[f"cin1{h}"], [a(1, h), a(6, h)], 0, ""))
+                    if NODE_PAD[1] == h:
+                        alt.append(("XK", reg[f"cin1{h}"], [reg[f"cin1{h}"]], NODE_PAD[2], ""))
+                    for x in (2, 3, 4):
+                        alt.append(("MOV", reg[f"cin{x}{h}"], [a(x, h)], 0, ""))
+        elif name in tz:
+            i, h = tz[name]
+            col = (i % 5, h)
+            home = reg[f"a{tz[last_of[col]][0]}{h}"]
+            if name == last_of[col] or any(ins[u][1] == home for u in range(last_read[name])):
+                alt.append(("XOR", d, [srcs[1], srcs[2]], 0, ""))
+                at[name] = d
+            else:
+                if col not in holder:
+                    holder[col] = home
+                    alt.append(("XOR", home, [srcs[1], srcs[2]], 0, ""))
+                at[name] = home
+            if (i, h) == NODE_PAD[:2]:
+                alt.append(("XK", d, [at[name]], NODE_PAD[2], ""))
+                at[name] = d
+        elif kind == "ROT" and name_of.get(srcs[0]) in tz:
+            alt.append((kind, d, [at[name_of[srcs[0]]], at[name_of[srcs[1]]]], imm, name))
+        else:
+            alt.append((kind, d, srcs, imm, name))
+        name_of[d] = name
+    return E, alt
+
+
+def simulate(ins, moves, regs, base):
     M = 0xFFFFFFFF
-    regs = {}
-    for i in range(25):
-        regs[base + 2 * i] = st[i] & M
-        regs[base + 2 * i + 1] = st[i] >> 32
-    for o, d, srcs in alloc:
+    regs = dict(regs)
+    for kind, d, srcs, imm, name in ins:
         s = [regs[r] for r in srcs]
-        if o.kind == "X3":
+        if kind == "X3":
             v = s[0] ^ s[1] ^ s[2]
-        elif o.kind == "CHI":
+        elif kind == "CHI":
             v = s[0] ^ (~s[1] & s[2] & M)
-        elif o.kind == "ROT":
-            v = (((s[0] << 32) | s[1]) >> o.imm) & M
+        elif kind == "ROT":
+            v = (((s[0] << 32) | s[1]) >> imm) & M
+        elif kind == "XK":
+            v = s[0] ^ imm
+        elif kind == "XOR":
+            v = s[0] ^ s[1]
         else:
-            rnd = int(o.dst[1:].split("_")[0])
-            v = s[0] ^ ((RC[rnd] >> (32 * o.imm)) & M)
+            v = s[0]
         regs[d] = v & M
     for d, s in moves:
         regs[d] = regs[s]
     return [regs[base + 2 * i] | (regs[base + 2 * i + 1] << 32) for i in range(25)]
+
+
+def state_regs(st, base):
+    return {base + 2 * i + h: (st[i] >> (32 * h)) & 0xFFFFFFFF for i in range(25) for h in range(2)}
+
+
+def text(ins):
+    kind, d, srcs, imm, name = ins
+    if kind in ("X3", "CHI"):
+        return f"v_bitop3_b32 v{d}, v{srcs[0]}, v{srcs[1]}, v{srcs[2]} bitop3:{hex(imm)}"
+    if kind == "ROT":
+        return f"v_alignbit_b32 v{d}, v{srcs[0]}, v{srcs[1]}, {imm}"
+    if kind == "XK":
+        return f"v_xor_b32_e64 v{d}, {imm}, v{srcs[0]}" if imm <= 64 else f"v_xor_b32 v{d}, {hex(imm)}, v{srcs[0]}"
+    if kind == "XOR":
+        return f"v_xor_b32_e64 v{d}, v{srcs[0]}, v{srcs[1]}"
+    return f"v_mov_b32_e64 v{d}, v{srcs[0]}"
 
 
 def main():
@@ -162,39 +268,66 @@
     args = [x for x in sys.argv[1:] if not x.startswith("--")]
     if args:
         base = int(args[0])
-    live, ops, final_a = build(base)
-    alloc, moves, conflicts = allocate(live, ops, final_a, base)
+    live, ops, final_a, nmain = build(base)
+    ins, final_regs, reg, moves, dmoves, conflicts = allocate(live, ops, final_a, base)
+    E, alt = node_region(ins, reg)
     if "--check" in sys.argv:
         import random
         rng = random.Random(2)
-        for _ in range(3):
+        mask = [(1 << 64) - 1] * 3 + [(1 << 32) - 1]
+        digest = lambda st: [w & m for w, m in zip(st, mask)]
+        for _ in range(8):
             st = [rng.getrandbits(64) for _ in range(25)]
-            assert simulate(alloc, moves, st, base) == ref_keccak_f(st)
-        kinds = "".join("A" if o.kind == "ROT" else "B" for o, _, _ in alloc)
-        print(f"ok: {len(alloc)} instructions + {len(moves)} moves, {conflicts} three-source instructions with all sources in one bank;",
-              kinds[:60], "...", file=sys.stderr)
+            ref = ref_keccak_f(st)
+            assert simulate(ins, moves, state_regs(st, base), base) == ref
+            assert digest(simulate(ins[:nmain], dmoves, state_regs(st, base), base)) == digest(ref)
+            node = st[:7] + [0] * 18
+            node[NODE_PAD[0]] = NODE_PAD[2] << 32
+            ref = ref_keccak_f(node)
+            regs = state_regs(st, base)
+            assert simulate(alt + ins[E:], moves, regs, base) == ref
+            assert digest(simulate(alt + ins[E:nmain], dmoves, regs, base)) == digest(ref)
+        kinds = "".join("A" if i[0] == "ROT" else "B" for i in ins)
+        print(f"ok: {nmain} + {len(ins) - nmain} (tail) instructions + {len(moves)} moves (digest only: {len(dmoves)}); node state: "
+              f"{len(alt)} for the first {E}; {conflicts} three-source instructions with all sources in one bank;", kinds[:60], "...",
+              file=sys.stderr)
         return
     w = sys.stdout.write
     top = base + 50 + NTEMP
     w("// GENERATED by gen_keccak_fixed.py -- do not edit.  Keccak-f[1600], 24 rounds unrolled, explicit VGPRs (see the generator).\n")
     w(f"#define P2_KF_BASE {base}\n#define P2_KF_TOP {top}  /* first register above the block's */\n")
-    w("#define P2_KECCAK_FIXED_PERMUTE() P2_KECCAK_FIXED_PERMUTE_PH(1)\n")
-    w("#define P2_KECCAK_FIXED_PERMUTE_PH(PH) asm volatile(\".p2align 6\\n .rept \" #PH \"\\n s_nop 0\\n .endr\\n\" \\\n")
-    for o, d, srcs in alloc:
-        if o.kind in ("X3", "CHI"):
-            w(f'  "v_bitop3_b32 v{d}, v{srcs[0]}, v{srcs[1]}, v{srcs[2]} bitop3:{hex(o.imm)}\\n" \\\n')
-        elif o.kind == "ROT":
-            w(f'  "v_alignbit_b32 v{d}, v{srcs[0]}, v{srcs[1]}, {o.imm}\\n" \\\n')
-        else:
-            rnd = int(o.dst[1:].split("_")[0])
-            k = (RC[rnd] >> (32 * o.imm)) & 0xFFFFFFFF
-            if k <= 64:
-                w(f'  "v_xor_b32_e64 v{d}, {k}, v{srcs[0]}\\n" \\\n')
-            else:
-                w(f'  "v_xor_b32 v{d}, {hex(k)}, v{srcs[0]}\\n" \\\n')
+    w("#define P2_KECCAK_FIXED_PERMUTE(NODE, DIGEST) P2_KECCAK_FIXED_PERMUTE_PH(1, NODE, DIGEST)\n")
+    w("#define P2_KECCAK_FIXED_PERMUTE_PH(PH, NODE, DIGEST) asm volatile(\".p2align 6\\n .rept \" #PH \"\\n s_nop 0\\n .endr\\n\" \\\n")
+    size = [0]
+
+    def line(txt, nbytes):
+        w(f'  "{txt}\\n" \\\n')
+        size[0] += nbytes
+
+    line("s_cmp_lg_u32 %0, 0", 4)
+    line("s_cbranch_scc1 .Lkf_node%=", 4)
+    for t, i in enumerate(ins):
+        if t == E:
+            line(".Lkf_join%=:", 0)
+        if t == nmain:
+            line("s_cmp_lg_u32 %1, 0", 4)
+            line("s_cbranch_scc1 .Lkf_digest%=", 4)
+        line(text(i), 8)
     for d, s in moves:
-        w(f'  "v_mov_b32 v{d}, v{s}\\n" \\\n')
-    w(f'  ::: "v{top - 1}")\n')
+        line(f"v_mov_b32 v{d}, v{s}", 4)
+    line("s_branch .Lkf_end%=", 4)
+    line(".Lkf_digest%=:", 0)
+    for d, s in dmoves:
+        line(f"v_mov_b32 v{d}, v{s}", 4)
+    line("s_branch .Lkf_end%=", 4)
+    if size[0] % 8:
+        line("s_nop 0", 4)
+    line(".Lkf_node%=:", 0)
+    for i in alt:
+        line(text(i), 8)
+    line("s_branch .Lkf_join%=", 4)
+    line(".Lkf_end%=:", 0)
+    w(f'  ::"s"(__builtin_amdgcn_readfirstlane((uint32_t)(NODE))), "s"(__builtin_amdgcn_readfirstlane((uint32_t)(DIGEST))) : "v{top - 1}", "scc")\n')
 
 
 if __name__ == "__main__":
diff --git a/acvm-backend-plonky2_amd/csrc/handle.hip b/acvm-backend-plonky2_amd/csrc/handle.hip
--- a/acvm-backend-plonky2_amd/csrc/handle.hip
+++ b/acvm-backend-plonky2_amd/csrc/handle.hip
@@ -897,6 +897,102 @@
   return P2GPU_OK;
 } P2GPU_CATCH
 
+int p2gpu_keccak_nodes(const uint8_t *left, const uint8_t *right, size_t n, int form, uint8_t *out) try {
+  if (!left || !right || !out || form < 0 || form > 2) return P2GPU_E_ARG;
+  std::vector<dig_t> h(2 * n);
+  memcpy(h.data(), left, 32 * n);
+  memcpy(h.data() + n, right, 32 * n);
+  if (form == 0) {
+    for (size_t i = 0; i < n; i++) {
+      const dig_t o = keccak_two_to_one(h[i], h[n + i]);
+      memcpy(out + 32 * i, o.w, 32);
+    }
+    return P2GPU_OK;
+  }
+  if (n == 0 || n % 256 || n > (1u << 30)) return P2GPU_E_ARG;
+  if (int rc = ensure_device()) return rc;
+  Scratch S;
+  HIP_TRY(hipStreamCreate(&S.st));
+  dig_t *in = S.alloc<dig_t>(2 * n), *o = S.alloc<dig_t>(n);
+  if (!in || !o) { set_err("hipMalloc failed"); return P2GPU_E_DEVICE; }
+  HIP_TRY(hipMemcpyAsync(in, h.data(), sizeof(dig_t) * 2 * n, hipMemcpyHostToDevice, S.st));
+  merkle_level_kf(S.st, in, o, (uint32_t)(2 * n), form == 2);
+  HIP_TRY(hipMemcpyAsync(out, o, sizeof(dig_t) * n, hipMemcpyDeviceToHost, S.st));
+  HIP_TRY(hipStreamSynchronize(S.st));
+  return P2GPU_OK;
+} P2GPU_CATCH
+
+int p2gpu_leaf_digests(const uint64_t *lde, size_t cols, unsigned d, unsigned cosets, const uint32_t *cls, const uint64_t *val,
+                       unsigned first, const uint64_t *basis, int levels, uint8_t *dig_out, uint8_t *lvl1_out, uint8_t *lvl2_out) try {
+  if (!lde || !dig_out || cols == 0 || cols > 4096 || d > 20 || cosets == 0 || cosets > 8 || (levels != 0 && levels != 2)) return P2GPU_E_ARG;
+  if (cls && (!val || !basis)) return P2GPU_E_ARG;
+  if (levels == 2 && (!lvl1_out || !lvl2_out || d < 2)) return P2GPU_E_ARG;
+  if (int rc = ensure_device()) return rc;
+  const size_t n = (size_t)1 << d;
+  Scratch S;
+  HIP_TRY(hipStreamCreate(&S.st));
+  gl_t *a = S.alloc<gl_t>(cosets * cols * n), *dval = S.alloc<gl_t>(cols), *dbasis = S.alloc<gl_t>(cosets * n);
+  uint32_t *dcls = S.alloc<uint32_t>(cols);
+  dig_t *dg = S.alloc<dig_t>(cosets * n), *l1 = S.alloc<dig_t>(cosets * n), *l2 = S.alloc<dig_t>(cosets * n);
+  if (!a || !dval || !dbasis || !dcls || !dg || !l1 || !l2) { set_err("hipMalloc failed"); return P2GPU_E_DEVICE; }
+  HIP_TRY(hipMemcpyAsync(a, lde, 8 * cosets * cols * n, hipMemcpyHostToDevice, S.st));
+  VirtCols v;
+  if (cls) {
+    HIP_TRY(hipMemcpyAsync(dcls, cls, 4 * cols, hipMemcpyHostToDevice, S.st));
+    HIP_TRY(hipMemcpyAsync(dval, val, 8 * cols, hipMemcpyHostToDevice, S.st));
+    HIP_TRY(hipMemcpyAsync(dbasis, basis, 8 * cosets * n, hipMemcpyHostToDevice, S.st));
+    v.cls = dcls; v.val = dval; v.basis = dbasis; v.first = first;
+  }
+  const uint32_t built = hash_lde_leaves(S.st, a, (uint32_t)cols, d, cosets, dg, nullptr, cls ? &v : nullptr, l1, l2, levels);
+  HIP_TRY(hipMemcpyAsync(dig_out, dg, sizeof(dig_t) * cosets * n, hipMemcpyDeviceToHost, S.st));
+  if (built == 2) {
+    HIP_TRY(hipMemcpyAsync(lvl1_out, l1, sizeof(dig_t) * cosets * (n >> 1), hipMemcpyDeviceToHost, S.st));
+    HIP_TRY(hipMemcpyAsync(lvl2_out, l2, sizeof(dig_t) * cosets * (n >> 2), hipMemcpyDeviceToHost, S.st));
+  }
+  HIP_TRY(hipStreamSynchronize(S.st));
+  return (int)built;
+} P2GPU_CATCH
+
+int p2gpu_fri_leaves(const uint64_t *vals, unsigned lg_npc, unsigned cosets, unsigned arity_bits, uint8_t *dig_out) try {
+  if (!vals || !dig_out || lg_npc > 24 || arity_bits > lg_npc || arity_bits > 4 || cosets == 0 || cosets > 8) return P2GPU_E_ARG;
+  if (int rc = ensure_device()) return rc;
+  const size_t npc = (size_t)1 << lg_npc, per = npc >> arity_bits;
+  Scratch S;
+  HIP_TRY(hipStreamCreate(&S.st));
+  gl_t *a = S.alloc<gl_t>(cosets * 2 * npc);
+  dig_t *dg = S.alloc<dig_t>(cosets * per);
+  if (!a || !dg) { set_err("hipMalloc failed"); return P2GPU_E_DEVICE; }
+  HIP_TRY(hipMemcpyAsync(a, vals, 8 * cosets * 2 * npc, hipMemcpyHostToDevice, S.st));
+  hash_fri_leaves(S.st, a, lg_npc, cosets, arity_bits, dg);
+  HIP_TRY(hipMemcpyAsync(dig_out, dg, sizeof(dig_t) * cosets * per, hipMemcpyDeviceToHost, S.st));
+  HIP_TRY(hipStreamSynchronize(S.st));
+  return P2GPU_OK;
+} P2GPU_CATCH
+
+int p2gpu_pow_min(const uint64_t state[12], unsigned pos, unsigned pow_bits, uint64_t count, int on_device, uint64_t *witness_out) try {
+  if (!state || !witness_out || pos >= 12 || pow_bits > 32 || count == 0 || count > (1ull << 24)) return P2GPU_E_ARG;
+  *witness_out = UINT64_MAX;
+  if (!on_device) {
+    for (uint64_t w = 0; w < count; w++) {
+      gl_t st[12];
+      for (int j = 0; j < 12; j++) st[j] = (unsigned)j == pos ? w : state[j];
+      keccak_permutation12<8>(st);
+      if (pow_bits == 0 || (st[7] >> (64 - pow_bits)) == 0) { *witness_out = w; break; }
+    }
+    return P2GPU_OK;
+  }
+  if (int rc = ensure_device()) return rc;
+  Scratch S;
+  HIP_TRY(hipStreamCreate(&S.st));
+  unsigned long long *res = S.alloc<unsigned long long>(1);
+  if (!res) { set_err("hipMalloc failed"); return P2GPU_E_DEVICE; }
+  HIP_TRY(hipMemsetAsync(res, 0xFF, 8, S.st));
+  pow_search(S.st, state, pos, pow_bits, 0, count, res, nullptr);
+  HIP_TRY(hipMemcpyAsync(witness_out, res, 8, hipMemcpyDeviceToHost, S.st));
+  HIP_TRY(hipStreamSynchronize(S.st));
+  return P2GPU_OK;
+} P2GPU_CATCH
+
 int p2gpu_commit_values(const uint64_t *vals, size_t ncols, unsigned d, unsigned rate_bits, unsigned cap_h,
                         uint8_t *cap_out) try {
   if (int rc = ensure_device()) return rc;
diff --git a/acvm-backend-plonky2_amd/csrc/internal.hpp b/acvm-backend-plonky2_amd/csrc/internal.hpp
--- a/acvm-backend-plonky2_amd/csrc/internal.hpp
+++ b/acvm-backend-plonky2_amd/csrc/internal.hpp
@@ -94,7 +94,8 @@
   uint32_t coset_first = 0, coset_stride = 1;
 };
 uint32_t hash_lde_leaves(hipStream_t st, const gl_t *lde, uint32_t cols, uint32_t d, uint32_t cosets, dig_t *dig, const gl_t *prc = nullptr,
-                         const VirtCols *virt = nullptr, dig_t *lvl1 = nullptr, dig_t *lvl2 = nullptr);
+                         const VirtCols *virt = nullptr, dig_t *lvl1 = nullptr, dig_t *lvl2 = nullptr, int levels = -1);
+void merkle_level_kf(hipStream_t st, const dig_t *in, dig_t *out, uint32_t m, bool lone);
 void hash_lde_absorb(hipStream_t st, const gl_t *lde, uint32_t cols, uint32_t d, uint32_t cosets, uint32_t blk0,
                      uint32_t nblk, bool first, bool last, uint64_t *state, dig_t *dig, const VirtCols *virt = nullptr);
 void hash_rows(hipStream_t st, const gl_t *rows, size_t n_rows, uint32_t row_len, dig_t *dig);
diff --git a/acvm-backend-plonky2_amd/csrc/keccak.hpp b/acvm-backend-plonky2_amd/csrc/keccak.hpp
--- a/acvm-backend-plonky2_amd/csrc/keccak.hpp
+++ b/acvm-backend-plonky2_amd/csrc/keccak.hpp
@@ -86,7 +86,7 @@
   }
 
 #if defined(__HIP_DEVICE_COMPILE__)
-#include "keccak_fixed.inc"
+#include "keccak_edges.inc"
 #define P2_KF_SET(i, lo, hi)                                                                                     \
   asm volatile("v_mov_b32 v%c2, %0\n v_mov_b32 v%c3, %1" ::"v"(lo), "v"(hi), "n"(P2_KF_BASE + 2 * (i)), "n"(P2_KF_BASE + 2 * (i) + 1))
 #define P2_KF_XOR(i, lo, hi)                                                                                     \
@@ -99,10 +99,11 @@
 #define P2_KF_SET(i, lo, hi) ((void)(lo), (void)(hi))
 #define P2_KF_XOR(i, lo, hi) ((void)(lo), (void)(hi))
 #define P2_KF_GET(i, lo, hi) ((lo) = 0, (hi) = 0)
-#define P2_KECCAK_FIXED_PERMUTE() ((void)0)
-#define P2_KECCAK_FIXED_PERMUTE_PH(PH) ((void)0)
-#endif
-
+#define P2_KECCAK_FIXED_PERMUTE(NODE, DIGEST) ((void)(NODE), (void)(DIGEST))
+#define P2_KECCAK_FIXED_PERMUTE_PH(PH, NODE, DIGEST) ((void)(NODE), (void)(DIGEST))
+#endif
+
+template <bool NODE = false, bool DIGEST = false>
 P2_HD void keccak_f1600(uint64_t st[25]) {
   const uint64_t RC[24] = {
       0x0000000000000001ULL, 0x0000000000008082ULL, 0x800000000000808aULL, 0x8000000080008000ULL,
@@ -111,18 +112,27 @@
       0x000000008000808bULL, 0x800000000000008bULL, 0x8000000000008089ULL, 0x8000000000008003ULL,
       0x8000000000008002ULL, 0x8000000000000080ULL, 0x000000000000800aULL, 0x800000008000000aULL,
       0x8000000080008081ULL, 0x8000000000008080ULL, 0x0000000080000001ULL, 0x8000000080008008ULL};
-  uint64_t a00 = st[0], a01 = st[1], a02 = st[2], a03 = st[3], a04 = st[4], a05 = st[5], a06 = st[6], a07 = st[7],
-           a08 = st[8], a09 = st[9], a10 = st[10], a11 = st[11], a12 = st[12], a13 = st[13], a14 = st[14],
-           a15 = st[15], a16 = st[16], a17 = st[17], a18 = st[18], a19 = st[19], a20 = st[20], a21 = st[21],
-           a22 = st[22], a23 = st[23], a24 = st[24];
+  uint64_t a00 = st[0], a01 = st[1], a02 = st[2], a03 = st[3], a04 = st[4], a05 = st[5], a06 = st[6];
+#define P2_KECCAK_IN(i) (NODE ? ((i) == 16 ? 0x8000000000000000ULL : 0ULL) : st[NODE ? 0 : (i)])
+  uint64_t a07 = P2_KECCAK_IN(7), a08 = P2_KECCAK_IN(8), a09 = P2_KECCAK_IN(9), a10 = P2_KECCAK_IN(10), a11 = P2_KECCAK_IN(11),
+           a12 = P2_KECCAK_IN(12), a13 = P2_KECCAK_IN(13), a14 = P2_KECCAK_IN(14), a15 = P2_KECCAK_IN(15), a16 = P2_KECCAK_IN(16),
+           a17 = P2_KECCAK_IN(17), a18 = P2_KECCAK_IN(18), a19 = P2_KECCAK_IN(19), a20 = P2_KECCAK_IN(20), a21 = P2_KECCAK_IN(21),
+           a22 = P2_KECCAK_IN(22), a23 = P2_KECCAK_IN(23), a24 = P2_KECCAK_IN(24);
+#undef P2_KECCAK_IN
+  if constexpr (NODE) P2_KECCAK_ROUND(RC[0])
 #if defined(__HIP_DEVICE_COMPILE__)
 #pragma unroll 2
 #endif
-  for (int r = 0; r < 24; r++) P2_KECCAK_ROUND(RC[r])
-  st[0] = a00; st[1] = a01; st[2] = a02; st[3] = a03; st[4] = a04; st[5] = a05; st[6] = a06; st[7] = a07;
-  st[8] = a08; st[9] = a09; st[10] = a10; st[11] = a11; st[12] = a12; st[13] = a13; st[14] = a14; st[15] = a15;
-  st[16] = a16; st[17] = a17; st[18] = a18; st[19] = a19; st[20] = a20; st[21] = a21; st[22] = a22; st[23] = a23;
-  st[24] = a24;
+  for (int r = NODE ? 1 : 0; r < (DIGEST ? 23 : 24); r++) P2_KECCAK_ROUND(RC[r])
+  if constexpr (DIGEST) {
+    P2_KECCAK_ROUND(RC[23])
+    st[0] = a00; st[1] = a01; st[2] = a02; st[3] = a03;
+  } else {
+    st[0] = a00; st[1] = a01; st[2] = a02; st[3] = a03; st[4] = a04; st[5] = a05; st[6] = a06; st[7] = a07;
+    st[8] = a08; st[9] = a09; st[10] = a10; st[11] = a11; st[12] = a12; st[13] = a13; st[14] = a14; st[15] = a15;
+    st[16] = a16; st[17] = a17; st[18] = a18; st[19] = a19; st[20] = a20; st[21] = a21; st[22] = a22; st[23] = a23;
+    st[24] = a24;
+  }
 }
 
 P2_HD void keccak256_words(const uint64_t *in, size_t nwords, uint64_t out[4]) {
@@ -138,7 +148,7 @@
   for (size_t i = 0; i < rem; i++) st[i] ^= in[off + i];
   st[rem] ^= 0x01ULL;
   st[16] ^= 0x8000000000000000ULL;
-  keccak_f1600(st);
+  keccak_f1600<false, true>(st);
   for (int i = 0; i < 4; i++) out[i] = st[i];
 }
 
@@ -153,7 +163,6 @@
 
 P2_HD dig_t keccak_two_to_one(const dig_t &l, const dig_t &r) {
   uint64_t st[25];
-  for (int i = 0; i < 25; i++) st[i] = 0;
   st[0] = l.w[0];
   st[1] = l.w[1];
   st[2] = l.w[2];
@@ -161,8 +170,7 @@
   st[4] = (r.w[0] >> 56) | (r.w[1] << 8);
   st[5] = (r.w[1] >> 56) | (r.w[2] << 8);
   st[6] = (r.w[2] >> 56) | ((r.w[3] & 0xFFULL) << 8) | (0x01ULL << 16);
-  st[16] = 0x8000000000000000ULL;
-  keccak_f1600(st);
+  keccak_f1600<true, true>(st);
   return dig_from_state(st);
 }
 
@@ -191,6 +199,7 @@
   c.m0 = L0 == 0 ? 0xFFFFFFFFu : 0u;
   return c;
 }
+#if defined(__HIPCC__)
 __device__ __forceinline__ void keccak_f1600_coop(uint32_t &lo, uint32_t &hi, const KeccakCoopLane &c) {
 #if defined(__HIP_DEVICE_COMPILE__)
   constexpr uint64_t RC[24] = {
@@ -221,6 +230,7 @@
   (void)lo, (void)hi, (void)c;
 #endif
 }
+#endif
 
 P2_HD void dig_to_elems(const dig_t &d, gl_t out[4]) {
   const uint64_t M56 = 0x00FFFFFFFFFFFFFFULL;
diff --git a/acvm-backend-plonky2_amd/csrc/kf_check.py b/acvm-backend-plonky2_amd/csrc/kf_check.py
--- a/acvm-backend-plonky2_amd/csrc/kf_check.py
+++ b/acvm-backend-plonky2_amd/csrc/kf_check.py
@@ -6,7 +6,7 @@
 import tempfile
 
 here = os.path.dirname(os.path.abspath(__file__))
-inc = open(os.path.join(here, "keccak_fixed.inc")).read()
+inc = open(os.path.join(here, "keccak_edges.inc")).read()
 base = int(re.search(r"#define P2_KF_BASE (\d+)", inc).group(1))
 top = int(re.search(r"#define P2_KF_TOP (\d+)", inc).group(1))
 hipcc = sys.argv[1] if len(sys.argv) > 1 else "hipcc"
diff --git a/acvm-backend-plonky2_amd/csrc/merkle.hip b/acvm-backend-plonky2_amd/csrc/merkle.hip
--- a/acvm-backend-plonky2_amd/csrc/merkle.hip
+++ b/acvm-backend-plonky2_amd/csrc/merkle.hip
@@ -65,7 +65,7 @@
     if ((uint32_t)w == rem) st[w] ^= 0x01ULL;
   }
   st[16] ^= 0x8000000000000000ULL;
-  keccak_f1600(st);
+  keccak_f1600<false, true>(st);
   return dig_from_state(st);
 }
 
@@ -180,10 +180,6 @@
     const uint64_t x = w[i];
     const uint32_t lo = (uint32_t)x, hi = (uint32_t)(x >> 32);
     P2_KF_SET(i, lo, hi);
-  });
-  static_for<7, 25>([&](auto ic) {
-    constexpr int i = decltype(ic)::value;
-    P2_KF_SET(i, 0u, (i == 16 ? 0x80000000u : 0u));
   });
 }
 template <bool V, int LV>
@@ -229,7 +225,7 @@
         off += 17;
       }
     }
-    P2_KECCAK_FIXED_PERMUTE();
+    P2_KECCAK_FIXED_PERMUTE(stage, complete);
     if (!complete) continue;
     const dig_t dg = kf_digest();
     if (stage == 0) dig[(size_t)c * n + k] = dg;
@@ -259,8 +255,8 @@
 template <int PH>
 __device__ __forceinline__ dig_t kf_two_to_one(const dig_t &l, const dig_t &r) {
   kf_set_two_to_one(l, r);
-  if constexpr (PH == 0) P2_KECCAK_FIXED_PERMUTE_PH(0);
-  else P2_KECCAK_FIXED_PERMUTE_PH(1);
+  if constexpr (PH == 0) P2_KECCAK_FIXED_PERMUTE_PH(0, 1u, 1u);
+  else P2_KECCAK_FIXED_PERMUTE_PH(1, 1u, 1u);
   return kf_digest();
 }
 template <int PH>
@@ -271,6 +267,11 @@
   if (k >= half) return;
   const dig_t l = in[(size_t)c * m + k], r = in[(size_t)c * m + k + half];
   out[(size_t)c * half + k] = kf_two_to_one<PH>(l, r);
+}
+void merkle_level_kf(hipStream_t st, const dig_t *in, dig_t *out, uint32_t m, bool lone) {
+  const dim3 grid(m / 2 / 256), block(256);
+  if (lone) hipLaunchKernelGGL(merkle_level_kf_kernel<0>, grid, block, 0, st, in, out, m);
+  else hipLaunchKernelGGL(merkle_level_kf_kernel<1>, grid, block, 0, st, in, out, m);
 }
 __global__ __launch_bounds__(256) P2_KF_KERNEL_ATTR void merkle_levels_kf_kernel(dig_t *lvl, uint32_t cosets, uint32_t m, uint32_t levels) {
   __shared__ dig_t nodes[4][64];
@@ -364,7 +365,7 @@
   for (uint32_t b = 0; b < steps; b++) {
     const uint32_t off = 17 * (blk0 + b);
     kf_absorb<true>(off, b < nblk ? 17u : cols - off, row);
-    P2_KECCAK_FIXED_PERMUTE();
+    P2_KECCAK_FIXED_PERMUTE(0u, b < nblk ? 0u : 1u);
   }
   if (last) {
     dig[(size_t)c * n + k] = kf_digest();
@@ -405,7 +406,7 @@
       if ((uint32_t)w == rem) st[w] ^= 0x01ULL;
     }
     st[16] ^= 0x8000000000000000ULL;
-    keccak_f1600(st);
+    keccak_f1600<false, true>(st);
     dig[(size_t)c * n + k] = dig_from_state(st);
   } else {
 #pragma unroll
@@ -533,12 +534,12 @@
 #define P2_LEAF_PLAIN(...) LeafVariant{#__VA_ARGS__, __VA_ARGS__, nullptr, 0}
 #define P2_LEAF_FIXED(LV, ...) LeafVariant{#__VA_ARGS__, nullptr, __VA_ARGS__, LV}
 uint32_t hash_lde_leaves(hipStream_t st, const gl_t *lde, uint32_t cols, uint32_t d, uint32_t cosets, dig_t *dig, const gl_t *prc,
-                         const VirtCols *virt, dig_t *lvl1, dig_t *lvl2) {
+                         const VirtCols *virt, dig_t *lvl1, dig_t *lvl2, int levels) {
   size_t n = (size_t)1 << d;
   uint32_t threads = n >= 256 ? 256 : 64;
   const bool kf = !prc && cols * 8 > 25 && n >= 256;
   const bool virt_on = has_virtual(virt, cols);
-  const bool lv2 = kf && virt_on && lvl1 != nullptr && lvl2 != nullptr && cols > 3 * 17 && leaf_levels_on();
+  const bool lv2 = kf && virt_on && lvl1 != nullptr && lvl2 != nullptr && (levels < 0 ? cols > 3 * 17 && leaf_levels_on() : levels == 2);
   const LeafVariant k = prc   ? (virt_on ? P2_LEAF_PLAIN(hash_lde_leaves_kernel<1, true>) : P2_LEAF_PLAIN(hash_lde_leaves_kernel<1, false>))
                         : !kf ? (virt_on ? P2_LEAF_PLAIN(hash_lde_leaves_kernel<0, true>) : P2_LEAF_PLAIN(hash_lde_leaves_kernel<0, false>))
                         : !virt_on ? P2_LEAF_FIXED(0, hash_lde_leaves_kf_kernel<false, 0>)
diff --git a/acvm-backend-plonky2_amd/prover.py b/acvm-backend-plonky2_amd/prover.py
--- a/acvm-backend-plonky2_amd/prover.py
+++ b/acvm-backend-plonky2_amd/prover.py
@@ -101,6 +101,10 @@
     lib.p2gpu_lde_batch.argtypes = [vp, sz, ctypes.c_uint, ctypes.c_uint, vp]
     lib.p2gpu_commit_values.argtypes = [vp, sz, ctypes.c_uint, ctypes.c_uint, ctypes.c_uint, u8p]
     lib.p2gpu_hash_rows.argtypes = [vp, sz, sz, u8p]
+    lib.p2gpu_keccak_nodes.argtypes = [vp, vp, sz, ctypes.c_int, vp]
+    lib.p2gpu_leaf_digests.argtypes = [vp, sz, ctypes.c_uint, ctypes.c_uint, vp, vp, ctypes.c_uint, vp, ctypes.c_int, vp, vp, vp]
+    lib.p2gpu_fri_leaves.argtypes = [vp, ctypes.c_uint, ctypes.c_uint, ctypes.c_uint, vp]
+    lib.p2gpu_pow_min.argtypes = [vp, ctypes.c_uint, ctypes.c_uint, ctypes.c_uint64, ctypes.c_int, vp]
     lib.p2gpu_field_selftest.argtypes = [vp, vp, sz, vp]
     lib.p2gpu_field_selftest16.argtypes = [vp, vp, sz, vp]
     lib.p2gpu_device_info.argtypes = [ctypes.c_char_p, sz, ctypes.POINTER(ctypes.c_int), ctypes.POINTER(sz)]
@@ -753,3 +757,53 @@
     out = np.zeros(25 * n_rows, dtype=np.uint8)
     _check(lib.p2gpu_hash_rows(r.ctypes.data, n_rows, row_len, out.ctypes.data))
     return out.reshape(n_rows, 25)
+
+
+def keccak_nodes(left, right, form=1):
+    lib = load_library()
+    l, r = _u64(left), _u64(right)
+    assert l.shape == r.shape and l.ndim == 2 and l.shape[1] == 4
+    out = np.zeros_like(l)
+    _check(lib.p2gpu_keccak_nodes(l.ctypes.data, r.ctypes.data, l.shape[0], form, out.ctypes.data))
+    return out
+
+
+def leaf_digests(lde, virt=None, levels=0):
+    lib = load_library()
+    a = _u64(lde)
+    cosets, cols, n = a.shape
+    d = n.bit_length() - 1
+    dig = np.zeros((cosets, n, 4), dtype=np.uint64)
+    l1 = np.zeros((cosets, n // 2, 4), dtype=np.uint64)
+    l2 = np.zeros((cosets, n // 4, 4), dtype=np.uint64)
+    cls = val = basis = None
+    first = 0
+    if virt is not None:
+        cls = np.ascontiguousarray(virt[0], dtype=np.uint32)
+        val, first, basis = _u64(virt[1]), int(virt[2]), _u64(virt[3])
+        assert cls.shape == (cols,) and val.shape == (cols,) and basis.shape == (cosets, n)
+    built = lib.p2gpu_leaf_digests(a.ctypes.data, cols, d, cosets, cls.ctypes.data if virt is not None else None,
+                                   val.ctypes.data if virt is not None else None, first,
+                                   basis.ctypes.data if virt is not None else None, levels, dig.ctypes.data, l1.ctypes.data, l2.ctypes.data)
+    if built < 0:
+        _check(built)
+    return dig, l1, l2, built
+
+
+def fri_leaves(vals, arity_bits):
+    lib = load_library()
+    a = _u64(vals)
+    cosets, two, npc = a.shape
+    assert two == 2
+    out = np.zeros((cosets, npc >> arity_bits, 4), dtype=np.uint64)
+    _check(lib.p2gpu_fri_leaves(a.ctypes.data, npc.bit_length() - 1, cosets, arity_bits, out.ctypes.data))
+    return out
+
+
+def pow_min(state, pos, pow_bits, count, on_device=True):
+    lib = load_library()
+    s = _u64(state)
+    assert s.shape == (12,)
+    out = np.zeros(1, dtype=np.uint64)
+    _check(lib.p2gpu_pow_min(s.ctypes.data, pos, pow_bits, count, 1 if on_device else 0, out.ctypes.data))
+    return None if int(out[0]) == 0xFFFFFFFFFFFFFFFF else int(out[0])
diff --git a/include/p2gpu.h b/include/p2gpu.h
--- a/include/p2gpu.h
+++ b/include/p2gpu.h
@@ -120,6 +120,11 @@
 int p2gpu_commit_values(const uint64_t *vals, size_t ncols, unsigned d, unsigned rate_bits, unsigned cap_h,
                         uint8_t *cap_out);
 int p2gpu_hash_rows(const uint64_t *rows, size_t n_rows, size_t row_len, uint8_t *digests_out);
+int p2gpu_keccak_nodes(const uint8_t *left, const uint8_t *right, size_t n, int form, uint8_t *out);
+int p2gpu_leaf_digests(const uint64_t *lde, size_t cols, unsigned d, unsigned cosets, const uint32_t *cls, const uint64_t *val,
+                       unsigned first, const uint64_t *basis, int levels, uint8_t *dig_out, uint8_t *lvl1_out, uint8_t *lvl2_out);
+int p2gpu_fri_leaves(const uint64_t *vals, unsigned lg_npc, unsigned cosets, unsigned arity_bits, uint8_t *dig_out);
+int p2gpu_pow_min(const uint64_t state[12], unsigned pos, unsigned pow_bits, uint64_t count, int on_device, uint64_t *witness_out);
 int p2gpu_field_selftest(const uint64_t *a, const uint64_t *b, size_t n, uint64_t bad_out[8]);
 int p2gpu_field_selftest16(const uint64_t *a, const uint64_t *b, size_t n, uint64_t bad_out[16]);
 
```

Result: no change. 234.1 proofs/sec (median of 2 runs) (+0.3%).
